# RunhuiWang/DeltaPQ

Hardware: AMD Instinct MI355X
Metric: queries/sec, SIFT1M-shaped m=8 k=256 topk=100 (higher is better)
Workload: dtype f64 sum of f32 table entries (u8 code decode; the reference's incremental f64 stack); 1 GPU

## Files before the change

deltapq_amd/api.py:

```python
import ctypes

import numpy as np

from . import _lib
from ._lib import DpqError, Info, OpenOpts, Profile, check


def _np_ptr(a):
    return ctypes.c_void_p(a.ctypes.data)


def device_count():
    return _lib.load().dpq_device_count()


def read_codewords(path):
    lib = _lib.load()
    M, K, Ds = _lib.c_i32(), _lib.c_i32(), _lib.c_i32()
    check(lib.dpq_read_codewords(path.encode(), M, K, Ds, None), "dpq_read_codewords")
    out = np.empty((M.value, K.value, Ds.value), dtype=np.float32)
    check(lib.dpq_read_codewords(path.encode(), M, K, Ds, _np_ptr(out)), "dpq_read_codewords")
    return out


def read_vecs(path, ext="fvecs", top_n=-1):
    lib = _lib.load()
    n, D = _lib.c_i64(), _lib.c_i32()
    check(lib.dpq_read_vecs(path.encode(), int(ext == "bvecs"), n, D, None, 0), "dpq_read_vecs")
    keep = n.value if top_n < 0 else min(n.value, top_n)
    out = np.empty((keep, D.value), dtype=np.float32)
    check(lib.dpq_read_vecs(path.encode(), int(ext == "bvecs"), n, D, _np_ptr(out), keep), "dpq_read_vecs")
    return out


def read_dtc_file(path):
    lib = _lib.load()
    n_codes, n_bytes = _lib.c_i64(), _lib.c_i64()
    check(lib.dpq_read_dtc_header(path.encode(), n_codes, n_bytes), "dpq_read_dtc_header")
    payload = np.fromfile(path, dtype=np.uint8, offset=16, count=n_bytes.value)
    return n_codes.value, payload


def dtc_validate(payload, n_codes, M=8):
    lib = _lib.load()
    pl = np.ascontiguousarray(payload, dtype=np.uint8)
    st = _lib.DtcStats()
    check(lib.dpq_dtc_validate(_np_ptr(pl), pl.size, n_codes, M, st), "dpq_dtc_validate")
    return dict(n_codes=st.n_codes, n_bytes=st.n_bytes, n_diffs=st.n_diffs, max_depth=st.max_depth,
                depth_hist=list(st.depth_hist))


def dtc_encode(root, depths, masks, deltas, M=8):
    lib = _lib.load()
    root = np.ascontiguousarray(root, dtype=np.uint8)
    depths = np.ascontiguousarray(depths, dtype=np.uint8)
    masks = np.ascontiguousarray(masks, dtype=np.uint16)
    deltas = np.ascontiguousarray(deltas, dtype=np.uint8)
    nb = _lib.c_i64()
    check(lib.dpq_dtc_encode(_np_ptr(root), _np_ptr(depths), _np_ptr(masks), _np_ptr(deltas), len(depths), M, None,
                             nb), "dpq_dtc_encode")
    out = np.empty(nb.value, dtype=np.uint8)
    check(lib.dpq_dtc_encode(_np_ptr(root), _np_ptr(depths), _np_ptr(masks), _np_ptr(deltas), len(depths), M,
                             _np_ptr(out), nb), "dpq_dtc_encode")
    return out


def dtc_decode(payload, n_codes, M=8, first=0, count=None):
    lib = _lib.load()
    pl = np.ascontiguousarray(payload, dtype=np.uint8)
    if count is None:
        count = n_codes - first
    out = np.empty((max(int(count), 0), M), dtype=np.uint8)
    check(lib.dpq_dtc_decode(_np_ptr(pl), pl.size, n_codes, M, first, count, _np_ptr(out)), "dpq_dtc_decode")
    return out


class HostSoA:

    def __init__(self, payload, n_codes, M=8, shard_rank=0, shard_count=1, chunks_per_segment=0, num_codes=0,
                 multi_index_stride=0):
        lib = _lib.load()
        pl = np.ascontiguousarray(payload, dtype=np.uint8)
        opts = OpenOpts(0, shard_rank, shard_count, chunks_per_segment, 0, num_codes, multi_index_stride)
        h = ctypes.c_void_p()
        check(lib.dpq_soa_build(_np_ptr(pl), pl.size, n_codes, M, opts, h), "dpq_soa_build")
        self._h = h
        info = Info()
        check(lib.dpq_soa_info(h, info), "dpq_soa_info")
        self.info = info.as_dict()
        names = ["nib", "mask", "delta", "seg_delta_off", "seg_ckpt", "mi_cell_start", "mi_code", "mi_id", "par", "carry",
                 "st_ckpt", "st_mask", "st_poff", "st_pbase", "st_delta", "st_depth"]
        views = {"seg_delta_off": np.uint64, "st_ckpt": np.uint64, "st_mask": np.uint32, "st_poff": np.uint16, "st_pbase": np.uint32,
                 "st_depth": np.uint16}
        for which, name in enumerate(names):
            ptr, nb = ctypes.c_void_p(), _lib.c_i64()
            check(lib.dpq_soa_array(h, which, ptr, nb), "dpq_soa_array")
            buf = (ctypes.c_ubyte * nb.value).from_address(ptr.value) if nb.value else b""
            arr = np.frombuffer(buf, dtype=np.uint8).copy()
            if name in views:
                arr = arr.view(views[name])
            if name.startswith("mi_"):
                arr = arr.view(np.uint32)
            setattr(self, name, arr)
        lib.dpq_soa_free(h)
        self._h = None


class DeltaTree:

    _ARRAYS = [("vec_id", np.uint32), ("parent_pos", np.uint32), ("depth", np.uint8), ("mask", np.uint16),
               ("deltas", np.uint8), ("root", np.uint8), ("edges", np.uint32)]

    def __init__(self, codes, K=256, max_height_folds=1, codebook=None, device=None):
        lib = _lib.load()
        self._lib = lib
        c = np.ascontiguousarray(codes, dtype=np.uint8)
        assert c.ndim == 2
        n, M = c.shape
        cb = None if codebook is None else np.ascontiguousarray(codebook, dtype=np.float32)
        h = ctypes.c_void_p()
        cbp, ds = (None, 0) if cb is None else (_np_ptr(cb), cb.shape[2])
        if device is None:
            check(lib.dpq_tree_build(_np_ptr(c), n, M, K, max_height_folds, cbp, ds, h), "dpq_tree_build")
        else:
            check(lib.dpq_tree_build_gpu(_np_ptr(c), n, M, K, max_height_folds, cbp, ds, device, h),
                  "dpq_tree_build_gpu")
        self._h = h
        self.M, self.K, self.n = M, K, n
        st = _lib.DtcStats()
        check(lib.dpq_tree_stats(h, st), "dpq_tree_stats")
        self.stats = dict(n_codes=st.n_codes, n_bytes=st.n_bytes, n_diffs=st.n_diffs, max_depth=st.max_depth,
                          depth_hist=list(st.depth_hist))
        for which, (name, dt) in enumerate(self._ARRAYS):
            ptr, nb = ctypes.c_void_p(), _lib.c_i64()
            check(lib.dpq_tree_array(h, which, ptr, nb), "dpq_tree_array")
            buf = (ctypes.c_ubyte * nb.value).from_address(ptr.value) if nb.value else b""
            setattr(self, name, np.frombuffer(buf, dtype=np.uint8).copy().view(dt))
        self.edges = self.edges.reshape(-1, 2)

    def payload(self):
        nb = _lib.c_i64()
        check(self._lib.dpq_tree_encode(self._h, None, nb), "dpq_tree_encode")
        out = np.empty(nb.value, dtype=np.uint8)
        check(self._lib.dpq_tree_encode(self._h, _np_ptr(out), nb), "dpq_tree_encode")
        return out

    def write_files(self, dataset_dir):
        check(self._lib.dpq_tree_write_files(self._h, dataset_dir.encode()), "dpq_tree_write_files")

    def close(self):
        if self._h is not None:
            self._lib.dpq_tree_free(self._h)
            self._h = None

    def __del__(self):
        try:
            self.close()
        except Exception:
            pass


def encode_pq(vectors, codebook, device=0):
    lib = _lib.load()
    v = np.ascontiguousarray(vectors, dtype=np.float32)
    cb = np.ascontiguousarray(codebook, dtype=np.float32)
    M, K, Ds = cb.shape
    out = np.empty((v.shape[0], M), dtype=np.uint8)
    check(lib.dpq_encode_pq(_np_ptr(v), v.shape[0], v.shape[1], _np_ptr(cb), M, K, Ds, device, _np_ptr(out)),
          "dpq_encode_pq")
    return out


def train_codebook(vectors, M=8, K=256, max_iters=25, seed=0, init=None, device=0):
    lib = _lib.load()
    v = np.ascontiguousarray(vectors, dtype=np.float32)
    assert v.ndim == 2
    n, D = v.shape
    Ds = -(-D // M) if M >= 1 else 1
    opts = _lib.TrainOpts(device=device, max_iters=max_iters, seed=seed, use_initial=int(init is not None))
    if init is None:
        cb = np.zeros((max(M, 1), max(K, 1), Ds), dtype=np.float32)
    else:
        cb = np.array(init, dtype=np.float32, order="C")
        assert cb.shape == (M, K, Ds), "init must be [M][K][ceil(D / M)]"
    st = _lib.TrainStats()
    check(lib.dpq_train_codebook(_np_ptr(v), n, D, M, K, opts, _np_ptr(cb), st), "dpq_train_codebook")
    stats = {k: getattr(st, k) for k, _ in st._fields_ if k != "distortion"}
    stats["distortion"] = [st.distortion[i] for i in range(st.iters_run)]
    return cb, stats


def write_codewords(path, codebook):
    cb = np.ascontiguousarray(codebook, dtype=np.float32)
    M, K, Ds = cb.shape
    check(_lib.load().dpq_write_codewords(path.encode(), _np_ptr(cb), M, K, Ds), "dpq_write_codewords")


def read_codes_plain(path, M):
    lib = _lib.load()
    n = _lib.c_i64()
    check(lib.dpq_read_codes_plain(path.encode(), M, n, None), "dpq_read_codes_plain")
    out = np.empty((n.value, M), dtype=np.uint8)
    check(lib.dpq_read_codes_plain(path.encode(), M, n, _np_ptr(out)), "dpq_read_codes_plain")
    return out


def read_codes_plain_ex(path, M, K=256, with_id=False):
    lib = _lib.load()
    n = _lib.c_i64()
    check(lib.dpq_read_codes_plain_ex(path.encode(), M, K, int(with_id), n, None, None), "dpq_read_codes_plain_ex")
    codes = np.empty((n.value, M), dtype=np.uint16 if K > 256 else np.uint8)
    ids = np.empty(n.value, dtype=np.int32) if with_id else None
    check(lib.dpq_read_codes_plain_ex(path.encode(), M, K, int(with_id), n, _np_ptr(codes), None if ids is None else _np_ptr(ids)),
          "dpq_read_codes_plain_ex")
    return codes, ids


def write_codes_plain(path, codes):
    c = np.ascontiguousarray(codes, dtype=np.uint8)
    check(_lib.load().dpq_write_codes_plain(path.encode(), _np_ptr(c), c.shape[0], c.shape[1]), "dpq_write_codes_plain")


def read_qnode_ids(path, n_codes):
    out = np.empty(n_codes, dtype=np.uint32)
    check(_lib.load().dpq_read_qnode_ids(path.encode(), n_codes, _np_ptr(out)), "dpq_read_qnode_ids")
    return out


def _apply_tuning(opts, tune):
    for name, value in tune.items():
        if name == "plan_ratios":
            vals = list(value) + [0, 0, 0]
            for i in range(3):
                opts.plan_ratios[i] = int(vals[i])
        elif name in ("stream_max_queries", "coarse_below", "boot_cap", "boot_target", "flags", "batch_tile_nodes"):
            v = int(value)
            if name == "stream_max_queries" and v > MAX_STREAM_QUERIES:
                raise ValueError("stream_max_queries above %d: the stream pass answers at most four queries per pass" % MAX_STREAM_QUERIES)
            if name == "boot_cap" and v != 0 and not 2048 <= v <= 16384:
                raise ValueError("boot_cap outside 2048..16384")
            setattr(opts, name, v)
        else:
            raise TypeError("unknown dpq_open_opts field %r" % name)
    return opts


OPT_NO_RELABEL, OPT_NO_FUSE_QUANTISE, OPT_NO_ASYNC_OVERLAP, OPT_BOOT_FULLSORT = 1, 2, 4, 8
OPT_NO_TIGHTEN, OPT_NO_STRANDS, OPT_FORCE_STRANDS, OPT_NO_STRAND1 = 16, 32, 64, 128
MAX_STREAM_QUERIES = 16


class DeltaPQIndex:

    def __init__(self, handle):
        self._h = handle
        self._lib = _lib.load()

    @classmethod
    def open_file(cls, path, M=8, K=256, device=0, shard_rank=0, shard_count=1, chunks_per_segment=0,
                  cand_capacity=0, num_codes=0, bootstrap=0, batch_decode=0, **tune):
        lib = _lib.load()
        opts = _apply_tuning(OpenOpts(device, shard_rank, shard_count, chunks_per_segment, cand_capacity, num_codes, bootstrap,
                                      batch_decode), tune)
        h = ctypes.c_void_p()
        check(lib.dpq_open_file(path.encode(), M, K, opts, h), "dpq_open_file")
        return cls(h)

    @classmethod
    def open_memory(cls, payload, n_codes, M=8, K=256, device=0, shard_rank=0, shard_count=1, chunks_per_segment=0,
                    cand_capacity=0, num_codes=0, bootstrap=0, global_offset=0, global_n_codes=0, batch_decode=0, **tune):
        lib = _lib.load()
        pl = np.ascontiguousarray(payload, dtype=np.uint8)
        opts = _apply_tuning(OpenOpts(device, shard_rank, shard_count, chunks_per_segment, cand_capacity, num_codes, bootstrap,
                                      batch_decode, global_offset, global_n_codes), tune)
        h = ctypes.c_void_p()
        check(lib.dpq_open_memory(_np_ptr(pl), pl.size, n_codes, M, K, opts, h), "dpq_open_memory")
        return cls(h)

    @classmethod
    def open_plain(cls, codes, K=256, device=0, shard_rank=0, shard_count=1, chunks_per_segment=0, cand_capacity=0,
                   num_codes=0, bootstrap=0, **tune):
        lib = _lib.load()
        c = np.ascontiguousarray(codes, dtype=np.uint8)
        opts = _apply_tuning(OpenOpts(device, shard_rank, shard_count, chunks_per_segment, cand_capacity, num_codes, bootstrap), tune)
        h = ctypes.c_void_p()
        check(lib.dpq_open_plain_memory(_np_ptr(c), c.shape[0], c.shape[1], K, opts, h), "dpq_open_plain_memory")
        return cls(h)

    def set_codebook(self, codebook):
        cb = np.ascontiguousarray(codebook, dtype=np.float32)
        assert cb.ndim == 3
        check(self._lib.dpq_set_codebook(self._h, _np_ptr(cb), cb.shape[2]), "dpq_set_codebook")
        return self

    def info(self):
        i = Info()
        check(self._lib.dpq_get_info(self._h, i), "dpq_get_info")
        return i.as_dict()

    def query_batch(self, queries, top_k):
        q = np.ascontiguousarray(queries, dtype=np.float32)
        if q.ndim == 1:
            q = q[None, :]
        nq = q.shape[0]
        ids = np.empty((nq, top_k), dtype=np.int32)
        dists = np.empty((nq, top_k), dtype=np.float32)
        check(self._lib.dpq_query_batch(self._h, _np_ptr(q), nq, top_k, _np_ptr(ids), _np_ptr(dists)),
              "dpq_query_batch")
        return ids, dists

    def range_search(self, queries, radius):
        q = np.ascontiguousarray(queries, dtype=np.float32)
        if q.ndim == 1:
            q = q[None, :]
        nq = q.shape[0]
        r = np.ascontiguousarray(np.broadcast_to(np.asarray(radius, dtype=np.float32), (nq,)))
        res = ctypes.c_void_p()
        check(self._lib.dpq_range_search(self._h, _np_ptr(q), nq, _np_ptr(r), res), "dpq_range_search")
        try:
            n = _lib.c_i32()
            pl, pi, pd = ctypes.c_void_p(), ctypes.c_void_p(), ctypes.c_void_p()
            check(self._lib.dpq_range_result_get(res, n, pl, pi, pd), "dpq_range_result_get")
            lims = np.ctypeslib.as_array(ctypes.cast(pl, ctypes.POINTER(_lib.c_i64)), (n.value + 1,)).copy()
            total = int(lims[-1])
            ids = np.empty(total, dtype=np.int32)
            dists = np.empty(total, dtype=np.float32)
            if total:
                ctypes.memmove(ids.ctypes.data, pi.value, total * 4)
                ctypes.memmove(dists.ctypes.data, pd.value, total * 4)
            return lims, ids, dists
        finally:
# ... 398 lines not shown
```

deltapq_amd/csrc/dpq_capi.cpp:

```cpp
#include <hip/hip_runtime.h>

#include <algorithm>
#include <atomic>
#include <cmath>
#include <cstdio>
#include <cstdlib>
#include <cstring>
#include <memory>
#include <new>
#include <numeric>
#include <stdexcept>
#include <string>
#include <type_traits>
#include <vector>

#include "../../include/deltapq_amd.h"
#include "dpq_build.h"
#include "dpq_flat.h"
#include "dpq_format.h"
#include "dpq_kernels.h"
#include "dpq_lookup.h"
#include "dpq_train.h"

namespace {
// ... 54 lines not shown
        return *this;
    }
    ~DevBuf() { reset(); }
    int alloc(size_t count) {
        reset();
        return dev_alloc(&p_, count);
    }
    void reset() {
        if (p_) hipFree(p_);
        p_ = nullptr;
    }
    T* get() const { return p_; }
    operator T*() const { return p_; }

  private:
    T* p_ = nullptr;
};

struct EventPair {
    int kind;
    hipEvent_t a, b;
};

constexpr int kMaxBatchQueries = 2048;

}

struct dpq_soa {
    dpq::SoA soa;
};

struct dpq_tree {
    dpq::Tree tree;
};

struct dpq_range_result {
    int32_t nq = 0;
    std::vector<int64_t> lims;
    std::vector<int32_t> ids;
    std::vector<float> dists;
};

struct dpq_filter {
    uint64_t owner = 0;
    DevBuf<uint32_t> bits;
    int64_t n_allowed = 0;
    mutable DevBuf<uint32_t> l0_id;
    mutable int l0_n = -1;
};

struct dpq_flat {
    int device = 0;
    int64_t n = 0, id_offset = 0;
    int D = 0, Dp = 0;
    DevBuf<float> base;
    DevBuf<uint32_t> map;
    std::vector<uint32_t> h_map;
    DevBuf<uint64_t> keys;
    DevBuf<dpq::FlatQueryState> state;
    DevBuf<float> d_q, d_dists;
    DevBuf<int32_t> d_ids, d_cand;
    DevBuf<uint32_t> flag;
    size_t keys_n = 0, state_n = 0, q_n = 0, out_n = 0, cand_n = 0;
};

namespace {
uint64_t next_index_serial() {
    static std::atomic<uint64_t> next{1};
    return next++;
}
}

struct Tuning {
    int stream_max = 4;
    int coarse_below = 128;
    int plan_ratios[3] = {0, 0, 0};
    int boot_cap = 0, boot_target = 0;
    int boot_variant = 1;
    int select_threads = 0;
    int select_fast = 1;
    int64_t batch_tile_nodes = (int64_t)16 << 20;
    bool relabel = true, fuse_quantise = true, async_overlap = true, boot_fullsort = false, tighten = true, strands = true,
         force_strands = false;
    bool strand1 = true;
    int s1_debug = 0;
};

struct RangeWs {
    DevBuf<int32_t> slot_query;
    DevBuf<uint64_t> thr_key;
    DevBuf<int64_t> out_off;
    DevBuf<uint32_t> max_count;
    DevBuf<int64_t> lims;
    DevBuf<uint32_t> cand_count;
    DevBuf<uint64_t> cand_key;
    DevBuf<int32_t> out_ids;
    DevBuf<float> out_dists;
    DevBuf<uint64_t> scratch;
    size_t key_n = 0, out_n = 0, scratch_n = 0;
    int64_t last_max_keys = 0;
};

struct LookupWs {
    DevBuf<uint32_t> flag;
    DevBuf<int32_t> ids;
    DevBuf<uint8_t> codes;
    DevBuf<float> vecs;
    DevBuf<uint8_t> tile;
    DevBuf<uint32_t> tile_segs;
    size_t ids_n = 0, codes_n = 0, vecs_n = 0, tile_n = 0, tile_segs_n = 0;
};

struct Workspace {
    int slots = 0, cap = 0;
    DevBuf<float> d_lut32;
    DevBuf<float> d_lut32r;
    DevBuf<float> d_lut_min;
    DevBuf<uint4> d_qtab;
    DevBuf<uint32_t> d_cand_count;
    DevBuf<uint32_t> d_overflow;
    DevBuf<uint32_t> d_tight;
    DevBuf<uint64_t> d_cand_key, d_thr_key;
    DevBuf<uint64_t> d_scratch;
    DevBuf<uint8_t> d_batch_raw;
};

struct dpq_index {
    Tuning tune;
    const uint64_t serial = next_index_serial();
    int device = 0;
    int M = 8, K = 256, Ds = 0;
    int cap = 0;
    bool cap_auto = true;
    dpq_info info{};
    dpq::DeviceImage img;
    DevBuf<uint64_t> d_st_ckpt;
    DevBuf<uint32_t> d_st_mask;
    DevBuf<uint16_t> d_st_depth;
    DevBuf<uint32_t> d_st_pbase, d_strip_order;
    DevBuf<uint32_t> d_strip_segs;
    std::vector<int64_t> strip_seg_off;
    DevBuf<uint8_t> d_st_delta;
    int64_t strand_bytes = 0;
    DevBuf<uint8_t> d_nib, d_par, d_carry, d_mask, d_delta, d_ckpt, d_raw;
    bool plain = false;
    DevBuf<uint64_t> d_seg_off;
    DevBuf<uint32_t> d_mi_cell, d_mi_code, d_mi_id;
    bool boot = false;
    int boot_classes = 0;
    DevBuf<unsigned long long> d_boot_stamps;
    DevBuf<unsigned long long> d_s1_stamps;
    int batch_decode = 0;
    DevBuf<uint8_t> d_relabel;
    DevBuf<uint8_t> d_nbr;
    DevBuf<float> d_codebook;
    DevBuf<unsigned long long> d_counters;
    uint32_t* h_overflow = nullptr;
    static constexpr int kFlagSlots = 64;
    uint32_t* h_any = nullptr;
    uint32_t* d_any = nullptr;
    struct Pending {
        const float* d_queries;
        int nq, top_k;
        int32_t* d_ids;
        float* d_dists;
        hipStream_t stream;
        hipStream_t user_stream;
        int flag_slot;
        int host_slot = -1;
    };
    static constexpr int kHostSlots = 16;
    struct HostSlot {
        DevBuf<float> d_q;
        DevBuf<int32_t> d_ids;
        DevBuf<float> d_d;
        size_t qf = 0, oe = 0;
        int32_t* h_ids = nullptr;
        float* h_d = nullptr;
        size_t n_out = 0;
        bool busy = false, redo = false;
        bool direct = false;
        hipEvent_t kernels_done = nullptr;
    };
    HostSlot host_slots[kHostSlots];
    hipStream_t copy_in = nullptr, copy_out = nullptr;
    uint64_t host_seq = 0;
    Workspace lane[2];
    int active_lane = 0;
    Workspace& ws() { return lane[active_lane]; }
    const Workspace& ws() const { return lane[active_lane]; }
    hipStream_t lane_stream[2] = {nullptr, nullptr};
    hipEvent_t lane_ready[2] = {nullptr, nullptr};
    uint64_t async_seq = 0;
    hipStream_t ordered_stream[2] = {nullptr, nullptr};
    bool ordered_stream_set[2] = {false, false};
    int64_t finish_reruns = 0;
    std::vector<Pending> pending;
    DevBuf<float> d_q_stage;
    DevBuf<int32_t> d_ids_stage;
    DevBuf<float> d_dists_stage;
    size_t q_stage_floats = 0, out_stage_elems = 0;
    int plan_top_k = -1, plan_cap = -1, plan_coarse = -1;
    std::vector<int> level_off, level_cnt;
    RangeWs range;
    LookupWs lookup;
    DevBuf<uint32_t> d_order;
    DevBuf<uint32_t> d_l0_id, d_l0_code;
    int l0_segments = 0;
    bool prof = false;
    bool prof_scan_only = false;
    std::vector<EventPair> events;
    std::vector<hipEvent_t> ev_pool;
    dpq_profile prof_acc{};
    hipEvent_t get_event() {
        if (!ev_pool.empty()) {
            hipEvent_t e = ev_pool.back();
            ev_pool.pop_back();
            return e;
        }
        hipEvent_t e = nullptr;
        if (hipEventCreateWithFlags(&e, hipEventDisableSystemFence) != hipSuccess) {
            prof_failed = true;
            return nullptr;
        }
        return e;
    }
    bool prof_failed = false;
    dpq::BootArgs dbg_ba{};
    dpq::ScanArgs dbg_sa{};
    int dbg_boot_slots = 0, dbg_groups = 0, dbg_splits = 0;
};

namespace {

bool dev_mode() {
    const char* dev = getenv("DPQ_DEV");
    return dev && atoi(dev) != 0;
}
#define DPQ_DEV_ONLY() \
    if (!dev_mode()) return fail(DPQ_ERR_STATE, "developer diagnostics: start the process with DPQ_DEV=1")

Tuning resolve_tuning(const dpq_open_opts& o) {
    Tuning t;
    if (o.stream_max_queries != 0) t.stream_max = std::min(16, std::max(0, o.stream_max_queries));
    if (o.coarse_below > 0) t.coarse_below = o.coarse_below;
    for (int i = 0; i < 3; ++i) t.plan_ratios[i] = o.plan_ratios[i];
    t.boot_cap = std::max(0, o.boot_cap);
    t.boot_target = std::max(0, o.boot_target);
    if (o.batch_tile_nodes > 0) t.batch_tile_nodes = o.batch_tile_nodes;
    t.relabel = !(o.flags & DPQ_OPT_NO_RELABEL);
    t.fuse_quantise = !(o.flags & DPQ_OPT_NO_FUSE_QUANTISE);
    t.async_overlap = !(o.flags & DPQ_OPT_NO_ASYNC_OVERLAP);
    t.boot_fullsort = (o.flags & DPQ_OPT_BOOT_FULLSORT) != 0;
    t.tighten = !(o.flags & DPQ_OPT_NO_TIGHTEN);
    t.strands = !(o.flags & DPQ_OPT_NO_STRANDS);
    t.force_strands = (o.flags & DPQ_OPT_FORCE_STRANDS) != 0;
    t.strand1 = !(o.flags & DPQ_OPT_NO_STRAND1);
    if (dev_mode()) {
        auto geti = [](const char* name, int* v) { if (const char* e = getenv(name)) *v = atoi(e); };
        geti("DPQ_STREAM_MAX_QUERIES", &t.stream_max);
        geti("DPQ_COARSE_BELOW", &t.coarse_below);
        if (const char* e = getenv("DPQ_PLAN_RATIOS")) sscanf(e, "%d,%d,%d", &t.plan_ratios[0], &t.plan_ratios[1], &t.plan_ratios[2]);
        geti("DPQ_BOOT_CAP", &t.boot_cap);
        geti("DPQ_BOOT_TARGET", &t.boot_target);
        geti("DPQ_BOOT_VARIANT", &t.boot_variant);
        if (const char* e = getenv("DPQ_BATCH_TILE_NODES")) t.batch_tile_nodes = std::max<int64_t>(1, atoll(e));
        int v = 1;
        geti("DPQ_RELABEL", &v); t.relabel = t.relabel && v != 0;
        v = 1; geti("DPQ_FUSE_QUANTISE", &v); t.fuse_quantise = t.fuse_quantise && v != 0;
        v = 1; geti("DPQ_ASYNC_OVERLAP", &v); t.async_overlap = t.async_overlap && v != 0;
        v = 0; geti("DPQ_BOOT_FULLSORT", &v); t.boot_fullsort = t.boot_fullsort || v != 0;
        v = 1; geti("DPQ_TIGHTEN", &v); t.tighten = t.tighten && v != 0;
        geti("DPQ_SELECT_THREADS", &t.select_threads);
        geti("DPQ_SELECT_FAST", &t.select_fast);
        v = 1; geti("DPQ_STRANDS", &v); t.strands = t.strands && v != 0;
        t.force_strands = t.force_strands || v == 2;
        v = 1; geti("DPQ_STRAND1", &v); t.strand1 = t.strand1 && v != 0;
        geti("DPQ_S1_DEBUG", &t.s1_debug);
    }
    return t;
}

void use_lane(dpq_index* x, int lane) {
    if (lane == x->active_lane) return;
    x->dbg_groups = x->dbg_boot_slots = 0;
    x->active_lane = lane;
}

int ensure_workspace(dpq_index* x, int slots, int cap) {
    Workspace& w = x->ws();
    if (slots <= w.slots && cap <= w.cap) return DPQ_OK;
    slots = std::max(slots, w.slots);
    cap = std::max(cap, w.cap);
    x->dbg_groups = x->dbg_boot_slots = 0;
    DevBuf<uint8_t> batch_raw = std::move(w.d_batch_raw);
    w = Workspace();
    w.d_batch_raw = std::move(batch_raw);
    int rc;
    if ((rc = w.d_lut32.alloc((size_t)slots * x->M * 256))) return rc;
    if (x->d_relabel && (rc = w.d_lut32r.alloc((size_t)slots * x->M * 256))) return rc;
    if ((rc = w.d_lut_min.alloc((size_t)slots * x->M * 4))) return rc;
    if ((rc = w.d_qtab.alloc((size_t)(slots / dpq::queries_per_group(x->M) + 1) *
                             (dpq::qtab_bytes_per_group(x->M) / sizeof(uint4)))))
        return rc;
    if ((rc = w.d_cand_count.alloc((size_t)slots * dpq::kRegionStride))) return rc;
    if ((rc = w.d_cand_key.alloc((size_t)slots * cap))) return rc;
    if ((rc = w.d_scratch.alloc((size_t)slots * cap))) return rc;
    if ((rc = w.d_overflow.alloc((size_t)slots))) return rc;
    if ((rc = w.d_tight.alloc((size_t)slots * dpq::kTightWords))) return rc;
    if ((rc = w.d_thr_key.alloc((size_t)slots))) return rc;
    if (!x->h_overflow) DPQ_HIP(hipHostMalloc(reinterpret_cast<void**>(&x->h_overflow), sizeof(uint32_t) * 4096));
    if (!x->d_counters) {
        if ((rc = x->d_counters.alloc(2))) return rc;
        DPQ_HIP(hipMemset(x->d_counters, 0, 16));
    }
    if (!x->h_any) {
        DPQ_HIP(hipHostMalloc(reinterpret_cast<void**>(&x->h_any), sizeof(uint32_t) * dpq_index::kFlagSlots,
                              hipHostMallocMapped));
        DPQ_HIP(hipHostGetDevicePointer(reinterpret_cast<void**>(&x->d_any), x->h_any, 0));
    }
    w.slots = slots;
    w.cap = cap;
    return DPQ_OK;
}

std::vector<uint32_t> golden_order(int64_t n) {
    std::vector<uint32_t> order((size_t)n);
    int64_t P = std::max<int64_t>(1, (int64_t)((double)n * 0.6180339887498949));
    auto gcd = [](int64_t a, int64_t b) { while (b) { int64_t t = a % b; a = b; b = t; } return a; };
    while (gcd(P, n) != 1) ++P;
    for (int64_t j = 0; j < n; ++j) order[(size_t)j] = (uint32_t)((j * P) % n);
    return order;
}

int ensure_order(dpq_index* x) {
    const int64_t nseg = x->img.n_segments;
    if (x->d_order || nseg <= 0) return DPQ_OK;
    const std::vector<uint32_t> order = golden_order(nseg);
    int rc = x->d_order.alloc((size_t)nseg);
    if (rc) return rc;
    DPQ_HIP(hipMemcpy(x->d_order, order.data(), (size_t)nseg * sizeof(uint32_t), hipMemcpyHostToDevice));
    return DPQ_OK;
}

int auto_cap(int top_k) { return std::max(4096, 32 * top_k); }

int ensure_plan(dpq_index* x, int top_k, int cap, int shape) {
    if (x->plan_top_k == top_k && x->plan_cap == cap && x->plan_coarse == shape) return DPQ_OK;
    const int coarse = shape & 1;
    const bool tight = (shape & 2) != 0;
    const bool one_level = (shape & 4) != 0;
    const int64_t S = (int64_t)dpq::kChunk * x->img.chunks_per_segment;
    const int64_t nseg = x->img.n_segments;
    const int64_t s0 = std::min<int64_t>(nseg, std::max<int64_t>(1, dpq::kLevel0Nodes / S));
    std::vector<int64_t> bounds;
    if (x->boot) {
        bounds.push_back(nseg);
        std::vector<int> ratios;
        const int* forced = x->tune.plan_ratios;
        if (forced[0] >= 2) {
// ... 102 lines not shown
    return x->ws().d_batch_raw.alloc((size_t)batch_raw_bytes(x));
}

int splits_for(int n_seg_pass, int n_groups) {
    const int want = std::max(1, dpq::kMaxSplits / std::max(1, n_groups));
    return std::max(1, std::min(n_seg_pass, want));
}

struct Regions {
    int splits;
    int region_cap;
    int64_t stride;
};

Regions regions_for(const dpq_index* x, int n_seg_pass, int n_groups, int top_k, int cap) {
    Regions r;
    r.splits = splits_for(n_seg_pass, n_groups);
    r.region_cap = (cap - top_k) / r.splits;
    if (x->cap_auto)
        r.region_cap = std::max(r.region_cap, std::max(std::max(256, 16384 / r.splits), 64 * top_k / r.splits));
    r.region_cap = std::max(r.region_cap, 1);
    r.stride = (int64_t)top_k + (int64_t)r.splits * r.region_cap;
    return r;
}

struct Batch {
    int nq, top_k;
    int nqp, ngroups;
    int cap;
    bool tight_plan;
    bool direct;
    bool strands, strand1, strand1_tight;
    bool scratch;
    int64_t tile_segs;
    bool one_tile;
    bool labelled;
    bool boot_tables;
    int plan_shape;
    int64_t stride;
};

Batch batch_mode(const dpq_index* x, int nq, int top_k, bool filtered = false) {
    Batch b{};
    const int QG = dpq::queries_per_group(x->M);
    b.nq = nq;
    b.top_k = top_k;
    b.nqp = (nq + QG - 1) / QG * QG;
    b.ngroups = b.nqp / QG;
    b.cap = x->cap_auto ? auto_cap(top_k) : std::max(x->cap, top_k);
    b.tight_plan = x->tune.tighten && nq > x->tune.stream_max && b.ngroups * dpq::kTightSplits >= dpq::kMaxSplits &&
                   (x->plain || use_batch_decode(x, b.ngroups));
    b.direct = !x->plain && nq <= x->tune.stream_max && !filtered;
    b.strands = b.direct && x->img.st_ckpt != nullptr && (x->tune.force_strands || x->img.n_local >= dpq::kStrandMinNodes);
    b.strand1 = b.strands && x->tune.strand1 && dpq::stream_queries_per_pass(x->M, nq) == 1;
    b.strand1_tight = b.strand1 && x->tune.tighten && x->tune.plan_ratios[0] == 0;
    b.scratch = !b.direct && use_batch_decode(x, b.ngroups);
    b.tile_segs = b.scratch ? batch_tile_segments(x) : 0;
    b.one_tile = b.scratch && b.tile_segs >= x->img.n_segments;
    b.labelled = b.scratch && x->d_relabel.get() != nullptr;
    b.boot_tables = x->boot && x->tune.fuse_quantise && !b.direct;
    b.plan_shape = (nq <= x->tune.coarse_below ? 1 : 0) | (b.tight_plan ? 2 : 0) | (b.strand1_tight ? 4 : 0);
    return b;
}

int prepare_batch(dpq_index* x, Batch* b) {
    int rc;
    if ((rc = ensure_plan(x, b->top_k, b->cap, b->plan_shape))) return rc;
    int64_t stride = b->top_k;
    for (size_t l = 1; l < x->level_cnt.size(); ++l)
        stride = std::max(stride, regions_for(x, x->level_cnt[l], b->ngroups, b->top_k, b->cap).stride);
    const int s1_region_cap = std::min(std::max(64, b->top_k), 256);
    if (b->strand1) stride = std::max<int64_t>(stride, (int64_t)b->top_k + (int64_t)dpq::kStrand1Regions * s1_region_cap);
    if (stride > INT32_MAX) return fail(DPQ_ERR_NOMEM, "candidate buffer too large");
    if ((rc = ensure_workspace(x, b->nqp, (int)stride))) return rc;
    b->stride = x->ws().cap;
    if (b->scratch && (rc = ensure_batch_raw(x))) return rc;
    return DPQ_OK;
}

int build_tables(dpq_index* x, const Batch& b, const float* d_queries, hipStream_t stream) {
    Workspace& w = x->ws();
    if (b.one_tile) {
        Timer t(x, stream, 4);
        DPQ_HIP(dpq::launch_decode_list(x->img, nullptr, x->img.n_segments, x->d_relabel,
                                        reinterpret_cast<uint32_t*>(w.d_batch_raw.get()), stream));
    }
    {
        Timer t(x, stream, 0);
        DPQ_HIP(dpq::launch_lut_build(x->d_codebook, d_queries, b.nq, b.nqp, x->M, x->K, x->Ds, w.d_lut32, w.d_lut_min,
                                      nullptr, w.d_overflow, b.scratch ? x->d_relabel.get() : nullptr, w.d_lut32r,
                                      x->tune.tighten ? w.d_tight.get() : nullptr, stream));
    }
    if (x->prof) x->prof_acc.lut_launches++;
    return DPQ_OK;
}

dpq::ScanArgs batch_scan_args(const dpq_index* x, const Batch& b) {
    const Workspace& w = x->ws();
    dpq::ScanArgs sa{};
    sa.img = x->img;
    if (b.one_tile) sa.img.raw = w.d_batch_raw;
    sa.fp32_accum = x->plain ? 1 : 0;
    sa.lut32 = b.labelled ? w.d_lut32r.get() : w.d_lut32.get();
    sa.lut_min = w.d_lut_min;
    sa.thr_key = w.d_thr_key;
    sa.slot_query = nullptr;
    sa.n_queries = b.nq;
    sa.cand_count = w.d_cand_count;
    sa.cand_key = w.d_cand_key;
    sa.cand_stride = b.stride;
    sa.region_off = b.top_k;
    sa.counters = x->prof && !x->prof_scan_only ? x->d_counters.get() : nullptr;
    sa.qtab = w.d_qtab;
    sa.tight_hist = x->tune.tighten && (b.top_k <= 512 || x->level_cnt.size() <= 2) ? w.d_tight.get() : nullptr;
    sa.tight_k = b.top_k;
    return sa;
}

dpq::SelectArgs batch_select_args(const dpq_index* x, const Batch& b, int32_t* d_ids, float* d_dists, int flag_slot) {
    const Workspace& w = x->ws();
    dpq::SelectArgs se{};
    se.threads = x->tune.select_threads;
    se.fast_final = x->tune.select_fast;
    se.cand_count = w.d_cand_count;
    se.cand_key = w.d_cand_key;
    se.cand_stride = b.stride;
    se.region_off = b.top_k;
    se.scratch = w.d_scratch;
    se.lut32 = w.d_lut32;
    se.slot_query = nullptr;
    se.top_k = b.top_k;
    se.thr_key = w.d_thr_key;
    se.overflow = w.d_overflow;
    se.any_overflow = x->d_any + flag_slot;
    se.out_ids = d_ids;
    se.out_dists = d_dists;
    se.n_codes_total = x->plain ? -1 : x->img.n_codes_total;
    se.fp32_accum = x->plain ? 1 : 0;
    se.keep_thr = x->boot ? 1 : 0;
    se.stamps = x->d_boot_stamps ? x->d_boot_stamps + (size_t)kMaxBatchQueries * 8 : nullptr;
    return se;
}

int boot_level(dpq_index* x, const Batch& b, const dpq_filter* filt, hipStream_t stream) {
    const Workspace& w = x->ws();
    const int top_k = b.top_k;
    const int cap_env = x->tune.boot_cap;
    dpq::BootArgs ba{};
    ba.cell_start = x->d_mi_cell;
    const bool full_sort = x->tune.boot_fullsort;
    ba.nbr = full_sort ? nullptr : x->d_nbr.get();
    ba.n_classes = x->boot_classes;
    ba.mi_code = x->d_mi_code;
    ba.mi_id = x->d_mi_id;
    ba.lut32 = w.d_lut32;
    ba.slot_query = nullptr;
    ba.top_k = top_k;
    const int cap_auto = top_k <= 256 ? (x->M <= 8 ? 3072 : 6144) : (top_k <= 640 && x->M <= 8) ? 5888 : 12288;
    ba.cap = std::max(std::min(cap_env > 0 ? cap_env : cap_auto, 16384), std::max(top_k, 2048));
    ba.cap = (ba.cap + 63) / 64 * 64;
    const int target_env = x->tune.boot_target;
    const int target_auto = top_k <= 256 ? std::max(top_k, ba.cap * 2 / 3) : ba.cap;
    ba.target = target_env > 0 ? std::min(ba.cap, std::max(target_env, top_k)) : target_auto;
    ba.thr_key = w.d_thr_key;
    ba.cand_count = w.d_cand_count;
    ba.fp32_accum = x->plain ? 1 : 0;
    ba.stamps = x->d_boot_stamps;
    ba.variant = x->tune.boot_variant;
    ba.n_queries = b.nq;
    ba.qtab = b.boot_tables ? w.d_qtab.get() : nullptr;
    ba.relabel = b.scratch ? x->d_relabel.get() : nullptr;
    ba.lut_min = w.d_lut_min;
    if (filt) {
        ba.filter = filt->bits;
        ba.id_base = x->img.id_base;
        ba.eval_cap = 8 * ba.cap;
    }
    const int slots = b.boot_tables ? b.nqp : b.nq;
    {
        Timer t(x, stream, 5);
        DPQ_HIP(dpq::launch_bootstrap(ba, x->M, slots, stream));
    }
    if (x->prof) x->prof_acc.bootstrap_launches++;
    if (filt) return DPQ_OK;
    x->dbg_ba = ba;
    x->dbg_boot_slots = slots;
    return DPQ_OK;
}

int stream_level(dpq_index* x, const Batch& b, size_t l, const dpq::ScanArgs& sa, dpq::SelectArgs& se,
                 hipStream_t stream) {
    const Workspace& w = x->ws();
    const int nq = b.nq, top_k = b.top_k;
    dpq::ScanArgs st = sa;
    st.tight_hist = nullptr;
    st.region_cap = se.region_cap = (int32_t)std::min<int64_t>(b.stride - top_k, INT32_MAX);
    se.n_regions = 2;
    DPQ_HIP(hipMemset2DAsync(w.d_cand_count + 1, sizeof(uint32_t) * dpq::kRegionStride, 0, sizeof(uint32_t), (size_t)nq,
                             stream));
    if (!b.strands) {
        Timer t(x, stream, 1);
        DPQ_HIP(dpq::launch_stream(st, nq, stream));
        if (x->prof) x->prof_acc.stream_launches++;
    } else {
        const bool one_level = x->level_cnt.size() == 2;
        const int64_t nseg = x->img.n_segments, ns = x->img.n_strips;
        const int64_t lo = (int64_t)x->level_off[l] * ns / nseg;
        const int64_t hi = l + 1 == x->level_cnt.size() ? ns : ((int64_t)x->level_off[l] + x->level_cnt[l]) * ns / nseg;
        Timer t(x, stream, 1);
        if (b.strand1) {
            st.seg_list = one_level ? nullptr : x->d_strip_order + lo;
            st.n_seg_pass = (int32_t)(hi - lo);
            st.tight_hist = b.strand1_tight && one_level && nq == 1 ? w.d_tight.get() : nullptr;
            st.debug_pass = x->tune.s1_debug ? 16 + x->tune.s1_debug : 0;
            st.stamps = x->d_s1_stamps;
            st.region_cap = se.region_cap = (int32_t)((b.stride - top_k) / dpq::kStrand1Regions);
            se.n_regions = 1 + dpq::strand1_workgroups(st.n_seg_pass);
            DPQ_HIP(dpq::launch_strand1(st, nq, stream));
            if (x->prof) x->prof_acc.strand1_launches++;
        } else if (hi - lo < 1536 && x->d_strip_segs && !x->tune.force_strands) {
            st.seg_list = x->d_strip_segs + x->strip_seg_off[(size_t)lo];
            st.n_seg_pass = (int32_t)(x->strip_seg_off[(size_t)hi] - x->strip_seg_off[(size_t)lo]);
            DPQ_HIP(dpq::launch_stream(st, nq, stream));
            if (x->prof) x->prof_acc.stream_launches++;
        } else {
            st.seg_list = x->d_strip_order + lo;
            st.n_seg_pass = (int32_t)(hi - lo);
            DPQ_HIP(dpq::launch_strand(st, nq, stream));
            if (x->prof) x->prof_acc.strand_launches++;
        }
    }
    if (x->prof) {
        x->prof_acc.scan_launches++;
        x->prof_acc.scan_stream_bytes +=
            (int64_t)nq * (int64_t)((double)x->info.device_bytes * sa.n_seg_pass / std::max(1, x->img.n_segments));
    }
    return DPQ_OK;
}

int filter_level(dpq_index* x, const Batch& b, size_t l, dpq::ScanArgs sa, dpq::SelectArgs& se, hipStream_t stream) {
    const Workspace& w = x->ws();
    const Regions rg = regions_for(x, sa.n_seg_pass, b.ngroups, b.top_k, b.cap);
    sa.region_cap = se.region_cap = rg.region_cap;
    se.n_regions = 1 + rg.splits;
    if (!(b.boot_tables && l == 1)) {
        Timer t(x, stream, 3);
        DPQ_HIP(dpq::launch_quantise(sa, b.ngroups, stream));
    }
    if (b.scratch && !b.one_tile) {
        for (int t0 = 0; t0 < sa.n_seg_pass; t0 += (int)b.tile_segs) {
            const int cnt = std::min<int>((int)b.tile_segs, sa.n_seg_pass - t0);
            {
                Timer t(x, stream, 4);
                DPQ_HIP(dpq::launch_decode_list(x->img, sa.seg_list + t0, cnt, x->d_relabel,
                                                reinterpret_cast<uint32_t*>(w.d_batch_raw.get()), stream));
            }
            dpq::ScanArgs tile = sa;
            tile.img.raw = w.d_batch_raw;
            tile.raw_by_pos = 1;
            tile.append = t0 > 0 ? 1 : 0;
            tile.seg_list = sa.seg_list + t0;
            tile.n_seg_pass = cnt;
            {
                Timer t(x, stream, 1);
                DPQ_HIP(dpq::launch_scan(tile, b.ngroups, rg.splits, stream));
            }
            if (x->prof && t0 > 0) x->prof_acc.scan_launches++;
        }
    } else {
        Timer t(x, stream, 1);
        DPQ_HIP(dpq::launch_scan(sa, b.ngroups, rg.splits, stream));
        if (l == 1 && !sa.filter) {
            x->dbg_sa = sa;
            x->dbg_groups = b.ngroups;
            x->dbg_splits = rg.splits;
        }
    }
    if (x->prof) {
        x->prof_acc.scan_launches++;
        x->prof_acc.scan_stream_bytes +=
            (int64_t)((double)x->info.device_bytes * sa.n_seg_pass / std::max(1, x->img.n_segments));
    }
    return DPQ_OK;
}

int rerun_overflowed(dpq_index* x, const Batch& b, dpq::ScanArgs sa, dpq::SelectArgs se, hipStream_t stream) {
    const Workspace& w = x->ws();
    const int nq = b.nq, top_k = b.top_k;
    DPQ_HIP(hipStreamSynchronize(stream));
    if (*reinterpret_cast<volatile uint32_t*>(x->h_any) == 0) return DPQ_OK;
    std::vector<int> over;
    for (int base = 0; base < nq; base += 4096) {
        const int n = std::min(4096, nq - base);
        DPQ_HIP(hipMemcpyAsync(x->h_overflow, w.d_overflow.get() + base, sizeof(uint32_t) * n, hipMemcpyDeviceToHost,
                               stream));
        DPQ_HIP(hipStreamSynchronize(stream));
        for (int i = 0; i < n; ++i)
            if (x->h_overflow[i]) over.push_back(base + i);
    }
    if (over.empty()) return DPQ_OK;

    const int QG = dpq::queries_per_group(x->M);
    const int slots2 = ((int)over.size() + QG - 1) / QG * QG;
    const int ng2 = slots2 / QG;
    std::vector<int32_t> slot_query((size_t)slots2, -1);
    std::vector<uint64_t> h_key((size_t)b.nqp), k2((size_t)slots2, ~0ull);
    DPQ_HIP(hipMemcpy(h_key.data(), w.d_thr_key, sizeof(uint64_t) * b.nqp, hipMemcpyDeviceToHost));
    for (size_t i = 0; i < over.size(); ++i) {
        slot_query[i] = over[i];
        k2[i] = h_key[(size_t)over[i]];
    }
    const int splits2 = std::min(16, splits_for(x->img.n_segments, ng2));
    int64_t rcap2 = std::max<int64_t>(2 * (int64_t)top_k, 1024);
    for (int attempt = 0;; ++attempt) {
        const int64_t stride2 = (int64_t)top_k + (int64_t)splits2 * rcap2;
        if (stride2 > INT32_MAX) return fail(DPQ_ERR_NOMEM, "candidate buffer too large");
        DevBuf<int32_t> d_slot_query;
        DevBuf<uint32_t> c_count, c_over;
        DevBuf<uint64_t> c_keys, c_scratch, c_tk;
        DevBuf<uint4> c_qtab;
        int rc = d_slot_query.alloc((size_t)slots2);
        if (!rc) rc = c_count.alloc((size_t)slots2 * dpq::kRegionStride);
        if (!rc) rc = c_over.alloc((size_t)slots2);
        if (!rc) rc = c_keys.alloc((size_t)slots2 * stride2);
        if (!rc) rc = c_scratch.alloc((size_t)slots2 * stride2);
        if (!rc) rc = c_tk.alloc((size_t)slots2);
        if (!rc) rc = c_qtab.alloc((size_t)ng2 * (dpq::qtab_bytes_per_group(x->M) / sizeof(uint4)));
        if (rc) return rc;
        hipError_t e = hipSuccess;
        auto chk = [&](hipError_t r) { if (e == hipSuccess) e = r; };
        chk(hipMemcpy(d_slot_query, slot_query.data(), sizeof(int32_t) * slots2, hipMemcpyHostToDevice));
        chk(hipMemcpy(c_tk, k2.data(), sizeof(uint64_t) * slots2, hipMemcpyHostToDevice));
        chk(hipMemsetAsync(c_count, 0, sizeof(uint32_t) * slots2 * dpq::kRegionStride, stream));
        chk(hipMemsetAsync(c_over, 0, sizeof(uint32_t) * slots2, stream));
        sa.seg_list = nullptr;
        sa.n_seg_pass = x->img.n_segments;
        sa.tight_hist = nullptr;
// ... 57 lines not shown
            DPQ_HIP(dpq::launch_filter_ids(x->d_l0_id, n0, filt->bits, x->img.id_base, filt->l0_id, stream));
            filt->l0_n = n0;
        }
    }
    if ((rc = build_tables(x, b, d_queries, stream))) return rc;
    x->h_any[flag_slot] = 0;
    dpq::ScanArgs sa = batch_scan_args(x, b);
    sa.filter = filt ? filt->bits.get() : nullptr;
    dpq::SelectArgs se = batch_select_args(x, b, d_ids, d_dists, flag_slot);

    const int64_t S = (int64_t)dpq::kChunk * x->img.chunks_per_segment;
    const size_t n_levels = x->img.n_segments > 0 ? x->level_cnt.size() : 0;
    if (n_levels == 0) {
        se.final_pass = 1;
        DPQ_HIP(dpq::launch_select(se, x->M, nq, stream));
        return DPQ_OK;
    }
    for (size_t l = 0; l < n_levels; ++l) {
        if (l == 0 && x->boot) {
            if ((rc = boot_level(x, b, filt, stream))) return rc;
            continue;
        }
        if (l == 0) {
            se.shared_id = filt ? filt->l0_id.get() : x->d_l0_id.get();
            se.shared_code = x->d_l0_code;
            se.shared_n = (int)(x->level_cnt[0] * S);
        } else {
            se.shared_id = nullptr;
            se.shared_code = nullptr;
            se.shared_n = 0;
            sa.seg_list = x->d_order + x->level_off[l];
            sa.n_seg_pass = x->level_cnt[l];
            if ((rc = b.direct ? stream_level(x, b, l, sa, se, stream) : filter_level(x, b, l, sa, se, stream))) return rc;
        }
        if (x->prof) x->prof_acc.scan_node_query_pairs += (int64_t)x->level_cnt[l] * S * nq;
        se.final_pass = l + 1 == n_levels ? 1 : 0;
        {
            Timer t(x, stream, 2);
            DPQ_HIP(dpq::launch_select(se, x->M, nq, stream));
        }
        if (x->prof) x->prof_acc.select_launches++;
    }
    if (flag_slot > 0) return DPQ_OK;
    return rerun_overflowed(x, b, sa, se, stream);
}

constexpr int64_t kRangeChunkKeys = (int64_t)1 << 26;

bool range_thr_key(float r, uint64_t* key) {
    if (!(r > 0.0f)) return false;
    if (std::isinf(r)) {
        *key = ~0ull;
        return true;
    }
    uint32_t bits;
    std::memcpy(&bits, &r, sizeof bits);
    *key = ((uint64_t)bits << 32) - 1ull;
    return true;
}

template <class T>
int grow(DevBuf<T>& buf, size_t* have, size_t want) {
    if (want <= *have && buf) return DPQ_OK;
    *have = 0;
    int rc = buf.alloc(want);
    if (!rc) *have = want;
    return rc;
}

int range_scan(dpq_index* x, const Batch& b, dpq::ScanArgs sa, int n_groups, int splits, hipStream_t stream) {
    const Workspace& w = x->ws();
    DPQ_HIP(hipMemsetAsync(sa.cand_count, 0, sizeof(uint32_t) * (size_t)n_groups * dpq::queries_per_group(x->M) *
                                                 dpq::kRegionStride, stream));
    if (sa.n_seg_pass <= 0) return DPQ_OK;
    {
        Timer t(x, stream, 3);
        DPQ_HIP(dpq::launch_quantise(sa, n_groups, stream));
    }
    if (b.scratch && !b.one_tile) {
        for (int t0 = 0; t0 < sa.n_seg_pass; t0 += (int)b.tile_segs) {
            const int cnt = std::min<int>((int)b.tile_segs, sa.n_seg_pass - t0);
            {
                Timer t(x, stream, 4);
                DPQ_HIP(dpq::launch_decode_list(x->img, sa.seg_list + t0, cnt, x->d_relabel,
                                                reinterpret_cast<uint32_t*>(w.d_batch_raw.get()), stream));
            }
            dpq::ScanArgs tile = sa;
            tile.img.raw = w.d_batch_raw;
            tile.raw_by_pos = 1;
            tile.append = t0 > 0 ? 1 : 0;
            tile.seg_list = sa.seg_list + t0;
            tile.n_seg_pass = cnt;
            Timer t(x, stream, 1);
            DPQ_HIP(dpq::launch_scan(tile, n_groups, splits, stream));
            if (x->prof) x->prof_acc.scan_launches++;
        }
    } else {
        Timer t(x, stream, 1);
        DPQ_HIP(dpq::launch_scan(sa, n_groups, splits, stream));
        if (x->prof) x->prof_acc.scan_launches++;
    }
    return DPQ_OK;
}

int range_emit(dpq_index* x, dpq::RangeEmitArgs ea, int n_slots, const std::vector<int>& emit,
               const std::vector<int32_t>& slot_query, const std::vector<int64_t>& lims, int64_t res_base,
               dpq_range_result* res, hipStream_t stream) {
    RangeWs& R = x->range;
    std::vector<int64_t> off((size_t)n_slots);
    for (size_t i = 0; i < emit.size();) {
        std::fill(off.begin(), off.end(), -1);
        int64_t span = 0, max_n = 0;
        bool contiguous = true;
        size_t j = i;
        for (; j < emit.size(); ++j) {
            const int q = slot_query[(size_t)emit[j]];
            const int64_t n = lims[(size_t)q + 1] - lims[(size_t)q];
            if (j > i && span + n > kRangeChunkKeys) break;
            if (j > i && lims[(size_t)slot_query[(size_t)emit[j - 1]] + 1] != lims[(size_t)q]) contiguous = false;
            off[(size_t)emit[j]] = span;
            span += n;
            max_n = std::max(max_n, n);
        }
        if (span > 0) {
            int rc;
            if ((size_t)span > R.out_n) {
                R.out_n = 0;
                if ((rc = R.out_ids.alloc((size_t)span)) || (rc = R.out_dists.alloc((size_t)span))) return rc;
                R.out_n = (size_t)span;
            }
            if (max_n > dpq::kRangeLdsKeys && (rc = grow(R.scratch, &R.scratch_n, 2 * (size_t)span))) return rc;
            DPQ_HIP(hipMemcpyAsync(R.out_off, off.data(), sizeof(int64_t) * n_slots, hipMemcpyHostToDevice, stream));
            ea.out_off = R.out_off;
            ea.out_ids = R.out_ids;
            ea.out_dists = R.out_dists;
            ea.out_n = span;
            ea.scratch = max_n > dpq::kRangeLdsKeys ? R.scratch.get() : nullptr;
            int lk = 2;
            while (lk < std::min<int64_t>(max_n, dpq::kRangeLdsKeys)) lk <<= 1;
            ea.lds_keys = lk;
            {
                Timer t(x, stream, 2);
                DPQ_HIP(dpq::launch_range_emit(ea, n_slots, stream));
            }
            const int64_t first = res_base + lims[(size_t)slot_query[(size_t)emit[i]]];
            if (contiguous) {
                DPQ_HIP(hipMemcpyAsync(res->ids.data() + first, R.out_ids, sizeof(int32_t) * span, hipMemcpyDeviceToHost, stream));
                DPQ_HIP(hipMemcpyAsync(res->dists.data() + first, R.out_dists, sizeof(float) * span, hipMemcpyDeviceToHost,
                                       stream));
                DPQ_HIP(hipStreamSynchronize(stream));
            } else {
                std::vector<int32_t> h_ids((size_t)span);
                std::vector<float> h_d((size_t)span);
                DPQ_HIP(hipMemcpyAsync(h_ids.data(), R.out_ids, sizeof(int32_t) * span, hipMemcpyDeviceToHost, stream));
                DPQ_HIP(hipMemcpyAsync(h_d.data(), R.out_dists, sizeof(float) * span, hipMemcpyDeviceToHost, stream));
                DPQ_HIP(hipStreamSynchronize(stream));
                for (size_t k = i; k < j; ++k) {
                    const int q = slot_query[(size_t)emit[k]];
                    const int64_t o = off[(size_t)emit[k]], n = lims[(size_t)q + 1] - lims[(size_t)q];
                    std::copy(h_ids.begin() + o, h_ids.begin() + o + n, res->ids.begin() + res_base + lims[(size_t)q]);
                    std::copy(h_d.begin() + o, h_d.begin() + o + n, res->dists.begin() + res_base + lims[(size_t)q]);
                }
            }
        }
        i = j;
    }
    return DPQ_OK;
}

int range_batch(dpq_index* x, const float* d_queries, int nq, const float* radii, int base, dpq_range_result* res,
                hipStream_t stream) {
    RangeWs& R = x->range;
    const int QG = dpq::queries_per_group(x->M);
    Batch b = batch_mode(x, nq, 1);
    std::vector<int32_t> slot_query;
    std::vector<uint64_t> thr;
    for (int q = 0; q < nq; ++q) {
        uint64_t key;
        if (!range_thr_key(radii[q], &key)) continue;
        slot_query.push_back(q);
        thr.push_back(key);
    }
    const int n_active = (int)slot_query.size();
    const int slots = (n_active + QG - 1) / QG * QG, n_groups = slots / QG;
    slot_query.resize((size_t)slots, -1);
    thr.resize((size_t)slots, 0ull);
    const int64_t res_base = res->lims[(size_t)base];
    std::vector<int64_t> lims((size_t)nq + 1, 0);
    if (n_active == 0) {
        for (int q = 0; q <= nq; ++q) res->lims[(size_t)base + q] = res_base;
        return DPQ_OK;
    }
    int rc;
    if (!R.slot_query) {
        if ((rc = R.slot_query.alloc(kMaxBatchQueries))) return rc;
        if ((rc = R.thr_key.alloc(kMaxBatchQueries))) return rc;
        if ((rc = R.out_off.alloc(kMaxBatchQueries))) return rc;
        if ((rc = R.max_count.alloc(kMaxBatchQueries))) return rc;
        if ((rc = R.lims.alloc(kMaxBatchQueries + 1))) return rc;
        if ((rc = R.cand_count.alloc((size_t)kMaxBatchQueries * dpq::kRegionStride))) return rc;
    }
    if ((rc = ensure_workspace(x, b.nqp, std::max(1, x->ws().cap)))) return rc;
    if (b.scratch && (rc = ensure_batch_raw(x))) return rc;
    const bool tiled = b.scratch && !b.one_tile;
    if (tiled && (rc = ensure_order(x))) return rc;
    if ((rc = build_tables(x, b, d_queries, stream))) return rc;

    const int nseg = x->img.n_segments;
    const int splits = splits_for(nseg, n_groups);
    const int region_cap = x->cap_auto ? std::max(256, 16384 / splits) : std::max(1, x->cap / splits);
    const Workspace& w = x->ws();
    dpq::ScanArgs sa{};
    sa.img = x->img;
    if (b.one_tile) sa.img.raw = w.d_batch_raw;
    sa.fp32_accum = x->plain ? 1 : 0;
    sa.lut32 = b.labelled ? w.d_lut32r.get() : w.d_lut32.get();
    sa.lut_min = w.d_lut_min;
    sa.thr_key = R.thr_key;
    sa.slot_query = R.slot_query;
    sa.n_queries = slots;
    sa.seg_list = tiled ? x->d_order.get() : nullptr;
    sa.n_seg_pass = nseg;
    sa.cand_count = R.cand_count;
    sa.region_off = 0;
    sa.counters = x->prof && !x->prof_scan_only ? x->d_counters.get() : nullptr;
    sa.qtab = w.d_qtab;
    sa.tight_hist = nullptr;

    auto scan_and_count = [&](int n_live, int rcap, int64_t* lims_out, std::vector<uint32_t>* max_count) -> int {
        const int n_slots = (n_live + QG - 1) / QG * QG, ng = n_slots / QG;
        const int64_t stride = (int64_t)splits * rcap;
        int rc2 = grow(R.cand_key, &R.key_n, (size_t)n_live * stride);
        if (rc2) return rc2;
        R.last_max_keys = std::max(R.last_max_keys, (int64_t)n_live * stride);
        DPQ_HIP(hipMemcpyAsync(R.slot_query, slot_query.data(), sizeof(int32_t) * n_slots, hipMemcpyHostToDevice, stream));
        DPQ_HIP(hipMemcpyAsync(R.thr_key, thr.data(), sizeof(uint64_t) * n_slots, hipMemcpyHostToDevice, stream));
        sa.cand_key = R.cand_key;
        sa.cand_stride = stride;
        sa.region_cap = rcap;
        if ((rc2 = range_scan(x, b, sa, ng, splits, stream))) return rc2;
        dpq::RangeCountArgs ca{};
        ca.slot_query = R.slot_query;
        ca.cand_count = R.cand_count;
        ca.n_slots = n_slots;
        ca.n_regions = splits;
        ca.n_queries = nq;
        ca.max_count = R.max_count;
        ca.lims = R.lims;
        {
            Timer t(x, stream, 2);
            DPQ_HIP(dpq::launch_range_count(ca, stream));
        }
        max_count->resize((size_t)n_slots);
        DPQ_HIP(hipMemcpyAsync(lims_out, R.lims, sizeof(int64_t) * (nq + 1), hipMemcpyDeviceToHost, stream));
        DPQ_HIP(hipMemcpyAsync(max_count->data(), R.max_count, sizeof(uint32_t) * n_slots, hipMemcpyDeviceToHost, stream));
        DPQ_HIP(hipStreamSynchronize(stream));
        return DPQ_OK;
    };
    std::vector<uint32_t> max_count;
    if ((rc = scan_and_count(n_active, region_cap, lims.data(), &max_count))) return rc;
    for (int q = 0; q <= nq; ++q) res->lims[(size_t)base + q] = res_base + lims[(size_t)q];
    const int64_t total = res_base + lims[(size_t)nq];
    res->ids.resize((size_t)total);
    res->dists.resize((size_t)total);

    dpq::RangeEmitArgs ea{};
    ea.cand_count = R.cand_count;
    ea.cand_key = R.cand_key;
    ea.cand_stride = (int64_t)splits * region_cap;
    ea.region_off = 0;
    ea.region_cap = region_cap;
    ea.n_regions = splits;
    ea.n_codes_total = x->plain ? -1 : x->img.n_codes_total;
    std::vector<int> emit, over;
    for (int s = 0; s < n_active; ++s) (max_count[(size_t)s] > (uint32_t)region_cap ? over : emit).push_back(s);
    if ((rc = range_emit(x, ea, slots, emit, slot_query, lims, res_base, res, stream))) return rc;
    if (over.empty()) return DPQ_OK;

    const std::vector<int32_t> q_of(slot_query.begin(), slot_query.begin() + n_active);
    const std::vector<uint64_t> k_of(thr.begin(), thr.begin() + n_active);
    const std::vector<uint32_t> need(max_count.begin(), max_count.begin() + n_active);
    for (size_t i = 0; i < over.size();) {
        size_t j = i;
        uint32_t rcap = 0;
        for (; j < over.size(); ++j) {
            const uint32_t r2 = std::max(rcap, need[(size_t)over[j]]);
            if (j > i && (int64_t)(j - i + 1) * splits * (int64_t)r2 > kRangeChunkKeys) break;
            rcap = r2;
        }
        if ((int64_t)rcap * splits > INT32_MAX) return fail(DPQ_ERR_NOMEM, "range search: candidate regions too large");
        const int n2 = (int)(j - i), slots2 = (n2 + QG - 1) / QG * QG;
        std::fill(slot_query.begin(), slot_query.end(), -1);
        for (int k = 0; k < n2; ++k) {
            slot_query[(size_t)k] = q_of[(size_t)over[i + k]];
            thr[(size_t)k] = k_of[(size_t)over[i + k]];
        }
        std::vector<int64_t> lims2((size_t)nq + 1);
        if ((rc = scan_and_count(n2, (int)rcap, lims2.data(), &max_count))) return rc;
        for (int k = 0; k < n2; ++k) {
            const int q = slot_query[(size_t)k];
            if (max_count[(size_t)k] > rcap || lims2[(size_t)q + 1] - lims2[(size_t)q] != lims[(size_t)q + 1] - lims[(size_t)q])
                return fail(DPQ_ERR_STATE, "range search: the rerun of an overflowed query found a different count");
        }
        ea.cand_key = R.cand_key;
        ea.cand_stride = (int64_t)splits * rcap;
        ea.region_cap = (int)rcap;
        std::vector<int> emit2((size_t)n2);
        std::iota(emit2.begin(), emit2.end(), 0);
        if ((rc = range_emit(x, ea, slots2, emit2, slot_query, lims, res_base, res, stream))) return rc;
        if (x->prof) x->prof_acc.overflow_reruns += n2;
        i = j;
    }
    return DPQ_OK;
}

void range_trim(dpq_index* x) {
    RangeWs& R = x->range;
    if (R.key_n > ((size_t)40 << 20)) R.cand_key.reset(), R.key_n = 0;
    if (R.out_n > ((size_t)16 << 20)) R.out_ids.reset(), R.out_dists.reset(), R.out_n = 0;
    R.scratch.reset();
    R.scratch_n = 0;
}

dpq::ScanArgs debug_scan_args(const dpq_index* x, int nq, int* splits) {
    const Workspace& w = x->ws();
    const int QG = dpq::queries_per_group(x->M);
    dpq::ScanArgs sa{};
    sa.img = x->img;
    sa.fp32_accum = x->plain ? 1 : 0;
    sa.lut32 = w.d_lut32;
    sa.lut_min = w.d_lut_min;
    sa.thr_key = w.d_thr_key;
    sa.slot_query = nullptr;
    sa.n_queries = nq;
    sa.seg_list = nullptr;
    sa.n_seg_pass = x->img.n_segments;
    if (const char* e = getenv("DPQ_DEBUG_NSEG")) sa.n_seg_pass = std::min(x->img.n_segments, atoi(e));
    if (*splits <= 0) *splits = splits_for(sa.n_seg_pass, (nq + QG - 1) / QG);
    sa.cand_count = w.d_cand_count;
    sa.cand_key = w.d_cand_key;
    sa.cand_stride = w.cap;
    sa.region_off = 0;
    sa.region_cap = std::max(1, w.cap / *splits);
    sa.qtab = w.d_qtab;
    return sa;
}

int open_from_payload(const uint8_t* payload, int64_t n_bytes, int64_t n_codes, int M, int K,
                      const dpq_open_opts* opts, dpq_index** out) {
    if (!out) return fail(DPQ_ERR_ARG, "out is NULL");
    *out = nullptr;
    dpq_open_opts o{};
    if (opts) o = *opts;
    if (M != 8 && M != 16)
        return fail(DPQ_ERR_ARG, "this build has scan kernels for M = 8 (reference format) and M = 16 (own extension)");
    if (K < 1 || K > 256) return fail(DPQ_ERR_ARG, "K must be in 1..256 (one byte per sub-code)");
    if (o.global_offset < 0 || o.global_n_codes < 0 || (o.global_offset != 0 && o.global_n_codes == 0) ||
        (o.global_n_codes > 0 && o.global_offset + n_codes > o.global_n_codes))
        return fail(DPQ_ERR_ARG, "global_offset / global_n_codes do not enclose this payload (a part of a larger index "
                                 "needs global_n_codes > 0)");
    if (n_codes >= (int64_t)INT32_MAX || o.global_n_codes >= (int64_t)INT32_MAX || o.global_offset + n_codes >= (int64_t)INT32_MAX)
        return fail(DPQ_ERR_ARG, "ids beyond 2^31 - 1: results carry int32 DFS positions (h:2979)");
    if (o.chunks_per_segment > dpq::kSortMax / dpq::kChunk)
        return fail(DPQ_ERR_ARG, "chunks_per_segment must be <= 64 (a segment is the cascade's level-0 unit)");
    int ndev = 0;
    if (hipGetDeviceCount(&ndev) != hipSuccess || ndev <= 0)
        return fail(DPQ_ERR_NO_DEVICE, "no HIP device visible; this library has no CPU fallback");
    if (o.device < 0 || o.device >= ndev) return fail(DPQ_ERR_NO_DEVICE, "device ordinal out of range");

    dpq::SoA soa;
    std::string err;
    const int64_t n_scan = o.num_codes > 0 ? std::min<int64_t>(o.num_codes, n_codes) : n_codes;
    const int64_t per_shard = n_scan / std::max(1, o.shard_count);
    int mi_stride = o.bootstrap < 0 ? 0 : dpq::bootstrap_stride_for(per_shard);
    if (o.bootstrap > 0 && mi_stride == 0 && per_shard >= 16384) mi_stride = 1;
    const Tuning tune0 = resolve_tuning(o);
    const bool want_strands = tune0.strands && (tune0.force_strands || per_shard >= dpq::kStrandMinNodes / 4 * 3);
    int rc = dpq::transcode(payload, n_bytes, n_codes, M, o.shard_rank, o.shard_count, o.chunks_per_segment, &soa,
                            &err, o.num_codes, mi_stride, 0, want_strands ? 1 : 0);
    if (rc) return fail(rc, err);

    DPQ_HIP(hipSetDevice(o.device));
    dpq_index* x = new dpq_index();
    x->device = o.device;
    x->M = M;
    x->K = K;
    x->cap_auto = o.cand_capacity <= 0;
    x->cap = o.cand_capacity;
    x->batch_decode = o.batch_decode;
    x->tune = tune0;
    auto up = [&](auto& buf, const void* src, size_t bytes) -> int {
        using T = typename std::remove_reference_t<decltype(buf)>::value_type;
        int r = buf.alloc((bytes + sizeof(T) - 1) / sizeof(T) + 64 / sizeof(T));
        if (r) return r;
        if (bytes) {
            hipError_t e = hipMemcpy(buf, src, bytes, hipMemcpyHostToDevice);
            if (e != hipSuccess) return fail(DPQ_ERR_HIP, std::string("upload: ") + hipGetErrorString(e));
        }
        return DPQ_OK;
    };
    rc = up(x->d_nib, soa.nib.data(), soa.nib.size());
    if (!rc) rc = up(x->d_par, soa.par.data(), soa.par.size());
    if (!rc) rc = up(x->d_carry, soa.carry.data(), soa.carry.size());
    if (!rc) rc = up(x->d_mask, soa.mask.data(), soa.mask.size());
    if (!rc) rc = up(x->d_delta, soa.delta.data(), soa.delta.size());
    if (!rc) rc = up(x->d_seg_off, soa.seg_delta_off.data(), soa.seg_delta_off.size() * 8);
    if (!rc) rc = up(x->d_ckpt, soa.seg_ckpt.data(), soa.seg_ckpt.size());
    if (o.global_offset != 0)
        for (uint32_t& id : soa.mi_id) id += (uint32_t)o.global_offset;
    if (!rc && soa.mi_stride > 0 && (int64_t)soa.mi_id.size() >= 16384) {
        rc = up(x->d_mi_cell, soa.mi_cell_start.data(), soa.mi_cell_start.size() * 4);
        if (!rc) rc = up(x->d_mi_code, soa.mi_code.data(), soa.mi_code.size() * 4);
        if (!rc) rc = up(x->d_mi_id, soa.mi_id.data(), soa.mi_id.size() * 4);
        x->boot = !rc;
        x->boot_classes = soa.mi_classes;
    }
    if (!rc && x->tune.relabel && soa.relabel.size() == (size_t)M * 256) {
        rc = up(x->d_relabel, soa.relabel.data(), soa.relabel.size());
    }
    if (!rc && x->boot && x->tune.strands && soa.n_strips > 0 && soa.n_strips < INT32_MAX) {
        rc = up(x->d_st_ckpt, soa.st_ckpt.data(), soa.st_ckpt.size() * 8);
        if (!rc) rc = up(x->d_st_mask, soa.st_mask.data(), soa.st_mask.size() * 4);
        if (!rc) rc = up(x->d_st_depth, soa.st_depth.data(), soa.st_depth.size() * 2);
        if (!rc) rc = up(x->d_st_pbase, soa.st_pbase.data(), soa.st_pbase.size() * 4);
        if (!rc) rc = up(x->d_st_delta, soa.st_delta.data(), soa.st_delta.size());
        if (!rc) {
            const int64_t ns = soa.n_strips;
            const std::vector<uint32_t> order = golden_order(ns);
            rc = up(x->d_strip_order, order.data(), order.size() * 4);
            const int64_t S = soa.nodes_per_segment();
            if (!rc && dpq::kStripNodes % S == 0) {
                std::vector<uint32_t> segs;
                x->strip_seg_off.assign((size_t)ns + 1, 0);
                for (int64_t j = 0; j < ns; ++j) {
                    const int64_t s0 = (int64_t)order[(size_t)j] * (dpq::kStripNodes / S);
                    for (int64_t t = s0; t < std::min(s0 + dpq::kStripNodes / S, soa.n_segments); ++t) segs.push_back((uint32_t)t);
                    x->strip_seg_off[(size_t)j + 1] = (int64_t)segs.size();
                }
                rc = up(x->d_strip_segs, segs.data(), segs.size() * 4);
            }
        }
        if (!rc) {
            x->img.st_ckpt = x->d_st_ckpt;
            x->img.st_mask = x->d_st_mask;
            x->img.st_depth = x->d_st_depth;
            x->img.st_pbase = x->d_st_pbase;
            x->img.st_delta = x->d_st_delta;
            x->img.n_strips = (int32_t)soa.n_strips;
            x->strand_bytes = soa.strand_bytes();
        }
    }
    if (rc) {
        dpq_close(x);
        return rc;
    }
    x->img.nib = x->d_nib;
    x->img.par = x->d_par;
    x->img.carry = x->d_carry;
    x->img.mask = x->d_mask;
    x->img.delta = x->d_delta;
    x->img.seg_delta_off = x->d_seg_off;
    x->img.seg_ckpt = x->d_ckpt;
    x->img.n_local = soa.node_hi - soa.node_lo;
    x->img.n_codes_total = o.global_n_codes > 0 ? o.global_n_codes : soa.n_codes_total;
    x->img.id_base = (uint32_t)(o.global_offset + soa.node_lo);
    x->img.n_segments = (int32_t)soa.n_segments;
    x->img.chunks_per_segment = soa.chunks_per_segment;
    x->img.M = M;
    x->img.K = K;

    dpq_info& inf = x->info;
    inf.n_codes_total = x->img.n_codes_total;
    inf.n_bytes_total = soa.n_bytes_total;
    inf.node_lo = o.global_offset + soa.node_lo;
    inf.node_hi = o.global_offset + soa.node_hi;
    inf.algorithmic_bytes = soa.algorithmic_bytes;
    inf.device_bytes = soa.device_bytes();
    inf.bootstrap_bytes = x->boot ? soa.bootstrap_bytes() : 0;
    inf.bootstrap_stride = x->boot ? soa.mi_stride : 0;
    inf.batch_decode_mb = batch_decode_possible(x) ? (int32_t)((batch_raw_bytes(x) + (1 << 20) - 1) >> 20) : 0;
    inf.strand_bytes = x->strand_bytes;
    inf.n_diffs = soa.n_diffs;
    inf.M = M;
    inf.K = K;
    inf.Ds = 0;
    inf.n_segments = (int32_t)soa.n_segments;
    inf.chunks_per_segment = soa.chunks_per_segment;
    inf.max_depth = soa.max_depth;
    inf.device = o.device;
    inf.cand_capacity = x->cap;
    *out = x;
    return DPQ_OK;
}

int open_plain(const uint8_t* codes, int64_t n_codes, int M, int K, const dpq_open_opts* opts, dpq_index** out) {
    if (!out) return fail(DPQ_ERR_ARG, "out is NULL");
    *out = nullptr;
    dpq_open_opts o{};
    if (opts) o = *opts;
    if (!codes || n_codes < 1 || n_codes >= (int64_t)INT32_MAX) return fail(DPQ_ERR_ARG, "bad codes / n_codes");
    if (M != 8 && M != 16) return fail(DPQ_ERR_ARG, "M must be 8 or 16");
    if (K < 1 || K > 256) return fail(DPQ_ERR_ARG, "K must be in 1..256 (one byte per sub-code)");
    int ndev = 0;
    if (hipGetDeviceCount(&ndev) != hipSuccess || ndev <= 0)
        return fail(DPQ_ERR_NO_DEVICE, "no HIP device visible; this library has no CPU fallback");
    if (o.device < 0 || o.device >= ndev) return fail(DPQ_ERR_NO_DEVICE, "device ordinal out of range");
    int cps = o.chunks_per_segment <= 0 ? dpq::kDefaultChunksPerSegment : o.chunks_per_segment;
    if (cps > dpq::kSortMax / dpq::kChunk) return fail(DPQ_ERR_ARG, "chunks_per_segment must be <= 64");
    int count = o.shard_count <= 0 ? 1 : o.shard_count;
    if (o.shard_rank < 0 || o.shard_rank >= count) return fail(DPQ_ERR_ARG, "bad shard_rank / shard_count");
    if (o.num_codes < 0 || (int64_t)o.num_codes > n_codes) return fail(DPQ_ERR_ARG, "num_codes outside 0..n_codes");
    if (o.num_codes > 0) n_codes = o.num_codes;
    const int64_t S = (int64_t)dpq::kChunk * cps;
    const int64_t nseg_total = (n_codes + S - 1) / S;
    const int64_t seg_lo = nseg_total * o.shard_rank / count, seg_hi = nseg_total * (o.shard_rank + 1) / count;
    const int64_t lo = std::min(seg_lo * S, n_codes), hi = std::min(seg_hi * S, n_codes);
    DPQ_HIP(hipSetDevice(o.device));
    dpq_index* x = new dpq_index();
    x->device = o.device;
    x->M = M;
    x->K = K;
    x->plain = true;
    x->tune = resolve_tuning(o);
    x->cap_auto = o.cand_capacity <= 0;
    x->cap = o.cand_capacity;
    const size_t padded = (size_t)(seg_hi - seg_lo) * S * M;
    int rc = x->d_raw.alloc(padded + 64);
    if (!rc) {
        hipError_t e = hipMemset(x->d_raw, 0, padded + 64);
        if (e == hipSuccess && hi > lo)
            e = hipMemcpy(x->d_raw, codes + (size_t)lo * M, (size_t)(hi - lo) * M, hipMemcpyHostToDevice);
        if (e != hipSuccess) rc = fail(DPQ_ERR_HIP, std::string("upload: ") + hipGetErrorString(e));
    }
    if (rc) {
        dpq_close(x);
        return rc;
    }
    {
        int mi_stride = o.bootstrap < 0 ? 0 : dpq::bootstrap_stride_for(hi - lo);
        if (o.bootstrap > 0 && mi_stride == 0 && hi - lo >= 16384) mi_stride = 1;
        if (mi_stride > 0) {
            dpq::SoA mi;
            std::vector<uint32_t> ids;
            std::vector<uint8_t> cds;
            for (int64_t i = lo; i < hi; i += mi_stride) {
                ids.push_back((uint32_t)i);
                cds.insert(cds.end(), codes + (size_t)i * M, codes + (size_t)(i + 1) * M);
            }
            dpq::build_multi_index(ids, cds, M, mi_stride, dpq::bootstrap_classes_for((int64_t)ids.size()), &mi);
            auto upl = [&](DevBuf<uint32_t>& d, const std::vector<uint32_t>& v) -> int {
                int r = d.alloc(v.size() + 16);
                if (r) return r;
                if (!v.empty() && hipMemcpy(d, v.data(), v.size() * 4, hipMemcpyHostToDevice) != hipSuccess)
                    return fail(DPQ_ERR_HIP, "upload of the bootstrap multi-index failed");
                return DPQ_OK;
            };
            rc = upl(x->d_mi_cell, mi.mi_cell_start);
            if (!rc) rc = upl(x->d_mi_code, mi.mi_code);
            if (!rc) rc = upl(x->d_mi_id, mi.mi_id);
            if (rc) {
// ... 65 lines not shown
        case DPQ_ERR_NO_DEVICE: return "no usable GPU";
        case DPQ_ERR_HIP: return "HIP runtime error";
        case DPQ_ERR_NOMEM: return "out of memory";
        case DPQ_ERR_STATE: return "call out of order";
        case DPQ_ERR_TOPK: return "top_k exceeds the number of codes";
        default: return "unknown status";
    }
}

const char* dpq_last_error(void) { return g_last_error.c_str(); }

int dpq_device_count(void) {
    int n = 0;
    if (hipGetDeviceCount(&n) != hipSuccess) return 0;
    return n < 0 ? 0 : n;
}

int dpq_read_dtc_header(const char* path, int64_t* n_codes, int64_t* n_bytes) {
    return guarded([&]() -> int {
    if (!path || !n_codes || !n_bytes) return fail(DPQ_ERR_ARG, "NULL argument");
    std::string err;
    int rc = dpq::read_dtc_header(path, n_codes, n_bytes, &err);
    return rc ? fail(rc, err) : DPQ_OK;
    });
}

int dpq_read_codewords(const char* path, int32_t* M, int32_t* K, int32_t* Ds, float* out) {
    return guarded([&]() -> int {
    if (!path || !M || !K || !Ds) return fail(DPQ_ERR_ARG, "NULL argument");
    std::string err;
    std::vector<float> v;
    int m, k, ds;
    int rc = dpq::read_codewords(path, &m, &k, &ds, out ? &v : nullptr, &err);
    if (rc) return fail(rc, err);
    *M = m;
    *K = k;
    *Ds = ds;
    if (out) memcpy(out, v.data(), v.size() * sizeof(float));
    return DPQ_OK;
    });
}

int dpq_read_vecs(const char* path, int is_bvecs, int64_t* n, int32_t* D, float* out, int64_t cap) {
    return guarded([&]() -> int {
    if (!path || !n || !D) return fail(DPQ_ERR_ARG, "NULL argument");
    std::string err;
    std::vector<float> v;
    int d = 0;
    int rc = dpq::read_vecs(path, is_bvecs != 0, n, &d, out ? &v : nullptr, cap, &err);
    if (rc) return fail(rc, err);
    *D = d;
    if (out) memcpy(out, v.data(), v.size() * sizeof(float));
    return DPQ_OK;
    });
}

int dpq_dtc_file_name(const char* dataset_dir, int M, int K, int64_t N, char* out, int64_t out_len) {
    return guarded([&]() -> int {
    if (!dataset_dir || !out) return fail(DPQ_ERR_ARG, "NULL argument");
    std::string s = dpq::dtc_file_name(dataset_dir, M, K, N);
    if ((int64_t)s.size() + 1 > out_len) return fail(DPQ_ERR_ARG, "output buffer too small");
    memcpy(out, s.c_str(), s.size() + 1);
    return DPQ_OK;
    });
}

int dpq_dtc_validate(const uint8_t* payload, int64_t n_bytes, int64_t n_codes, int M, dpq_dtc_stats* stats) {
    return guarded([&]() -> int {
    std::string err;
    int rc = dpq::validate(payload, n_bytes, n_codes, M, stats, &err);
    return rc ? fail(rc, err) : DPQ_OK;
    });
}

int dpq_soa_build(const uint8_t* payload, int64_t n_bytes, int64_t n_codes, int M, const dpq_open_opts* opts,
                  dpq_soa** out) {
    return guarded([&]() -> int {
    if (!out) return fail(DPQ_ERR_ARG, "out is NULL");
    dpq_open_opts o{};
    if (opts) o = *opts;
    dpq_soa* s = new dpq_soa();
    std::string err;
    int rc = dpq::transcode(payload, n_bytes, n_codes, M, o.shard_rank, o.shard_count, o.chunks_per_segment, &s->soa,
                            &err, o.num_codes, o.bootstrap > 0 && M % 4 == 0 ? o.bootstrap : 0);
    if (rc) {
        delete s;
        *out = nullptr;
        return fail(rc, err);
    }
    *out = s;
    return DPQ_OK;
    });
}

int dpq_soa_info(const dpq_soa* soa, dpq_info* info) {
    return guarded([&]() -> int {
    if (!soa || !info) return fail(DPQ_ERR_ARG, "NULL argument");
    fill_info_from_soa(soa->soa, info);
    return DPQ_OK;
    });
}

int dpq_soa_array(const dpq_soa* soa, int which, const void** ptr, int64_t* n_bytes) {
    return guarded([&]() -> int {
    if (!soa || !ptr || !n_bytes) return fail(DPQ_ERR_ARG, "NULL argument");
    const dpq::SoA& s = soa->soa;
    switch (which) {
        case 0: *ptr = s.nib.data(); *n_bytes = (int64_t)s.nib.size(); break;
        case 1: *ptr = s.mask.data(); *n_bytes = (int64_t)s.mask.size(); break;
        case 2: *ptr = s.delta.data(); *n_bytes = (int64_t)s.delta.size(); break;
        case 3: *ptr = s.seg_delta_off.data(); *n_bytes = (int64_t)s.seg_delta_off.size() * 8; break;
        case 4: *ptr = s.seg_ckpt.data(); *n_bytes = (int64_t)s.seg_ckpt.size(); break;
        case 5: *ptr = s.mi_cell_start.data(); *n_bytes = (int64_t)s.mi_cell_start.size() * 4; break;
        case 6: *ptr = s.mi_code.data(); *n_bytes = (int64_t)s.mi_code.size() * 4; break;
        case 7: *ptr = s.mi_id.data(); *n_bytes = (int64_t)s.mi_id.size() * 4; break;
        case 8: *ptr = s.par.data(); *n_bytes = (int64_t)s.par.size(); break;
        case 9: *ptr = s.carry.data(); *n_bytes = (int64_t)s.carry.size(); break;
        case 10: *ptr = s.st_ckpt.data(); *n_bytes = (int64_t)s.st_ckpt.size() * 8; break;
        case 11: *ptr = s.st_mask.data(); *n_bytes = (int64_t)s.st_mask.size() * 4; break;
        case 12: *ptr = s.st_poff.data(); *n_bytes = (int64_t)s.st_poff.size() * 2; break;
        case 13: *ptr = s.st_pbase.data(); *n_bytes = (int64_t)s.st_pbase.size() * 4; break;
        case 14: *ptr = s.st_delta.data(); *n_bytes = (int64_t)s.st_delta.size(); break;
        case 15: *ptr = s.st_depth.data(); *n_bytes = (int64_t)s.st_depth.size() * 2; break;
        default: return fail(DPQ_ERR_ARG, "which must be 0..15");
    }
    return DPQ_OK;
    });
}

void dpq_soa_free(dpq_soa* soa) { delete soa; }

int dpq_dtc_encode(const uint8_t* root_code, const uint8_t* depths, const uint16_t* masks, const uint8_t* deltas,
                   int64_t n_codes, int M, uint8_t* out, int64_t* n_bytes) {
    return guarded([&]() -> int {
    std::string err;
    int rc = dpq::encode(root_code, depths, masks, deltas, n_codes, M, out, n_bytes, &err);
    return rc ? fail(rc, err) : DPQ_OK;
    });
}

int dpq_tree_build(const uint8_t* codes, int64_t n_codes, int M, int K, int max_height_folds, const float* codewords,
                   int Ds, dpq_tree** out) {
    return guarded([&]() -> int {
    if (!out) return fail(DPQ_ERR_ARG, "out is NULL");
    *out = nullptr;
    dpq_tree* t = new dpq_tree();
    std::string err;
    int rc = dpq::build_tree(codes, n_codes, M, K, max_height_folds, codewords, Ds, &t->tree, &err);
    if (rc) {
        delete t;
        return fail(rc, err);
    }
    *out = t;
    return DPQ_OK;
    });
}

int dpq_tree_build_gpu(const uint8_t* codes, int64_t n_codes, int M, int K, int max_height_folds,
                       const float* codewords, int Ds, int device, dpq_tree** out) {
    return guarded([&]() -> int {
    if (!out) return fail(DPQ_ERR_ARG, "out is NULL");
    *out = nullptr;
    if (!codes || n_codes < 1 || n_codes >= (int64_t)INT32_MAX || M < 1 || M > 16 || K < 1 || K > 256 ||
        max_height_folds < 1)
        return fail(DPQ_ERR_ARG, "bad argument to dpq_tree_build_gpu");
    std::string err;
    std::vector<uint32_t> finalists;
    std::vector<std::pair<uint32_t, uint32_t>> edges;
    const bool prefilter = !(dev_mode() && getenv("DPQ_BUILD_PREFILTER") && atoi(getenv("DPQ_BUILD_PREFILTER")) == 0);
    int rc = dpq::find_edges_gpu(codes, n_codes, M, max_height_folds, device, &finalists, &edges, &err, prefilter);
    if (rc) return fail(rc, err);
    dpq_tree* t = new dpq_tree();
    static const bool host_layout = dev_mode() && getenv("DPQ_BUILD_LAYOUT") &&
                                    std::string(getenv("DPQ_BUILD_LAYOUT")) == "host";
    rc = host_layout ? dpq::layout_tree(codes, n_codes, M, K, max_height_folds, codewords, Ds, finalists, &edges, &t->tree, &err)
                     : dpq::layout_tree_gpu(codes, n_codes, M, K, max_height_folds, codewords, Ds, finalists, &edges, device,
                                            &t->tree, &err);
    if (rc) {
        delete t;
        return fail(rc, err);
    }
    *out = t;
    return DPQ_OK;
    });
}

int dpq_tree_stats(const dpq_tree* t, dpq_dtc_stats* stats) {
    return guarded([&]() -> int {
    if (!t || !stats) return fail(DPQ_ERR_ARG, "NULL argument");
    const dpq::Tree& tr = t->tree;
    memset(stats, 0, sizeof *stats);
    stats->n_codes = tr.n;
    stats->n_diffs = tr.n_diffs;
    stats->n_bytes = tr.M + tr.n_diffs + (tr.n - 1) * dpq::mask_bytes_for(tr.M) + tr.n / 2;
    for (int d = 0; d < 16; ++d) stats->depth_hist[d] = tr.depth_hist[d];
    stats->max_depth = tr.max_depth;
    stats->M = tr.M;
    return DPQ_OK;
    });
}

int dpq_tree_array(const dpq_tree* t, int which, const void** ptr, int64_t* n_bytes) {
    return guarded([&]() -> int {
    if (!t || !ptr || !n_bytes) return fail(DPQ_ERR_ARG, "NULL argument");
    const dpq::Tree& tr = t->tree;
    switch (which) {
        case 0: *ptr = tr.vec_id.data(); *n_bytes = (int64_t)tr.vec_id.size() * 4; break;
// ... 883 lines not shown
    int64_t allowed = 0;
    for (int64_t w = 0; w < n_words && 32 * w < n_local; ++w) {
        const int64_t g0 = base + 32 * w;
        if (g0 >= n_bits) break;
        const int64_t lo = g0 >> 5;
        const int sh = (int)(g0 & 31);
        uint32_t v = words[lo] >> sh;
        if (sh && lo + 1 < user_words) v |= words[lo + 1] << (32 - sh);
        const int64_t valid = std::min<int64_t>(32, std::min(n_bits - g0, n_local - 32 * w));
        if (valid < 32) v &= (1u << valid) - 1u;
        h[(size_t)w] = v;
    }
    const int64_t N = x->img.n_codes_total;
    if (!x->plain && (N & 1) == 0 && N - 1 >= base && N - 1 < base + n_local) {
        const int64_t l = N - 1 - base;
        h[(size_t)(l >> 5)] = (h[(size_t)(l >> 5)] & ~(1u << (l & 31))) | (user_bit(N) << (l & 31));
    }
    for (uint32_t v : h) allowed += __builtin_popcount(v);
    std::unique_ptr<dpq_filter> f(new dpq_filter());
    f->owner = x->serial;
    f->n_allowed = allowed;
    int rc = f->bits.alloc((size_t)n_words);
    if (rc) return rc;
    DPQ_HIP(hipMemcpy(f->bits, h.data(), (size_t)n_words * sizeof(uint32_t), hipMemcpyHostToDevice));
    *out = f.release();
    return DPQ_OK;
    });
}

void dpq_filter_free(dpq_filter* f) { delete f; }

int dpq_filter_count(const dpq_filter* f, int64_t* n_allowed) {
    if (!f || !n_allowed) return fail(DPQ_ERR_ARG, "NULL argument");
    *n_allowed = f->n_allowed;
    return DPQ_OK;
}

int dpq_query_batch_filtered(dpq_index* x, const dpq_filter* f, const float* queries, int nq, int top_k, int32_t* ids,
                             float* dists) {
    return guarded([&]() -> int {
    int rc = check_filter(x, f);
    if (rc) return rc;
    return query_host(x, f, queries, nq, top_k, ids, dists);
    });
}

int dpq_query_batch_device_filtered(dpq_index* x, const dpq_filter* f, const float* d_queries, int nq, int top_k,
                                    int32_t* d_ids, float* d_dists, void* hip_stream) {
    return guarded([&]() -> int {
    int rc = check_filter(x, f);
    if (rc) return rc;
    return query_device(x, f, d_queries, nq, top_k, d_ids, d_dists, hip_stream);
    });
}

namespace {

constexpr size_t kLookupVecBytes = (size_t)64 << 20;
constexpr int64_t kLookupTileNodes = (int64_t)4 << 20;

bool lookup_id_ok(const dpq_index* x, int64_t id) {
    const int64_t N = x->img.n_codes_total;
    int64_t pos = id;
    if (!x->plain && (N & 1) == 0) {
        if (id == N)
            pos = N - 1;
        else if (id == N - 1)
            return false;
    }
    const int64_t l = pos - (int64_t)x->img.id_base;
    return l >= 0 && l < x->img.n_local;
}

int lookup_begin(dpq_index* x, int64_t n, hipStream_t stream, dpq::DeviceImage* img) {
    LookupWs& lw = x->lookup;
    *img = x->img;
    const int64_t image_bytes = (int64_t)x->img.n_segments * dpq::kChunk * x->img.chunks_per_segment * x->M;
    const bool possible = !x->plain && x->img.n_segments > 0 && image_bytes <= dpq::kLookupGroupedMaxBytes;
    bool grouped = possible && n >= dpq::kLookupGroupedPerSegment * (int64_t)x->img.n_segments;
    if (possible && dev_mode())
        if (const char* e = getenv("DPQ_LOOKUP_GROUPED")) grouped = atoi(e) != 0;
    if (!grouped) return DPQ_OK;
    if (int rc = grow(lw.tile, &lw.tile_n, (size_t)image_bytes)) return rc;
    DPQ_HIP(dpq::launch_decode_list(x->img, nullptr, x->img.n_segments, nullptr, reinterpret_cast<uint32_t*>(lw.tile.get()),
                                    stream));
    img->raw = lw.tile;
    return DPQ_OK;
}

void lookup_end(dpq_index* x) {
    LookupWs& lw = x->lookup;
    if (lw.tile_n > (size_t)(kLookupTileNodes + 1024 * dpq::kChunk) * x->M) {
        lw.tile.reset();
        lw.tile_n = 0;
    }
}

int lookup_run(dpq_index* x, const dpq::DeviceImage& img, const int32_t* d_ids, int64_t n, uint8_t* d_codes, float* d_vecs,
               hipStream_t stream, const char* who) {
    LookupWs& lw = x->lookup;
    int rc;
    if (!lw.flag.get() && (rc = lw.flag.alloc(1))) return rc;
    DPQ_HIP(hipMemsetAsync(lw.flag, 0, sizeof(uint32_t), stream));
    const size_t D = (size_t)x->M * x->Ds;
    for (int64_t i0 = 0; i0 < n; i0 += dpq::kLookupSlice) {
        dpq::LookupArgs a{};
        a.img = img;
        a.ids = d_ids + i0;
        a.n = std::min(dpq::kLookupSlice, n - i0);
        a.even_rule = x->plain ? 0 : 1;
        if (d_vecs) {
            a.out_vecs = d_vecs + (size_t)i0 * D;
            a.codebook = x->d_codebook;
            a.Ds = x->Ds;
        } else {
            a.out_codes = d_codes + (size_t)i0 * x->M;
        }
        a.flag = lw.flag;
        DPQ_HIP(dpq::launch_lookup(a, stream));
    }
    uint32_t bad = 0;
    DPQ_HIP(hipMemcpyAsync(&bad, lw.flag, sizeof bad, hipMemcpyDeviceToHost, stream));
    DPQ_HIP(hipStreamSynchronize(stream));
    if (bad) return fail(DPQ_ERR_ARG, std::string(who) + ": an id names no node of this handle");
    return DPQ_OK;
}

int lookup_on_device(dpq_index* x, const int32_t* d_ids, int64_t n, uint8_t* d_codes, float* d_vecs, hipStream_t stream,
                     const char* who) {
    dpq::DeviceImage img;
    int rc = lookup_begin(x, n, stream, &img);
    if (!rc) rc = lookup_run(x, img, d_ids, n, d_codes, d_vecs, stream, who);
    if (rc) hipStreamSynchronize(stream);
    lookup_end(x);
    return rc;
}

int lookup_args(dpq_index* x, const void* ids, int64_t n, const void* out, bool recon, const char* who) {
    if (!x || n < 0 || (n > 0 && (!ids || !out))) return fail(DPQ_ERR_ARG, std::string(who) + ": NULL argument or n < 0");
    if (recon && !x->d_codebook) return fail(DPQ_ERR_STATE, "dpq_set_codebook has not been called");
    if (!x->pending.empty())
        if (int rc = dpq_finish(x)) return rc;
    return DPQ_OK;
}

int lookup_host(dpq_index* x, const int32_t* ids, int64_t n, uint8_t* codes_out, float* vecs_out, const char* who) {
    int rc = lookup_args(x, ids, n, codes_out ? (const void*)codes_out : (const void*)vecs_out, vecs_out != nullptr, who);
    if (rc || n == 0) return rc;
    for (int64_t i = 0; i < n; ++i)
        if (ids[i] >= 0 && !lookup_id_ok(x, ids[i])) {
            char msg[160];
            snprintf(msg, sizeof msg, "%s: ids[%lld] = %d names no node of this handle", who, (long long)i, (int)ids[i]);
            return fail(DPQ_ERR_ARG, msg);
        }
    DPQ_HIP(hipSetDevice(x->device));
    LookupWs& lw = x->lookup;
    const size_t D = (size_t)x->M * x->Ds;
    int64_t slice = dpq::kLookupSlice;
    if (vecs_out) slice = std::max<int64_t>(1, std::min<int64_t>(slice, (int64_t)(kLookupVecBytes / (D * sizeof(float)))));
    slice = std::min(slice, n);
    rc = grow(lw.ids, &lw.ids_n, (size_t)slice);
    if (!rc && vecs_out) rc = grow(lw.vecs, &lw.vecs_n, (size_t)slice * D);
    if (!rc && codes_out) rc = grow(lw.codes, &lw.codes_n, (size_t)slice * x->M);
    if (rc) return rc;
    dpq::DeviceImage img;
    rc = lookup_begin(x, n, nullptr, &img);
    for (int64_t i0 = 0; !rc && i0 < n; i0 += slice) {
        const int64_t m = std::min(slice, n - i0);
        hipError_t e = hipMemcpy(lw.ids, ids + i0, (size_t)m * sizeof(int32_t), hipMemcpyHostToDevice);
        if (e == hipSuccess)
            rc = lookup_run(x, img, lw.ids, m, codes_out ? lw.codes.get() : nullptr, vecs_out ? lw.vecs.get() : nullptr, nullptr,
                            who);
        if (e == hipSuccess && !rc)
            e = vecs_out ? hipMemcpy(vecs_out + (size_t)i0 * D, lw.vecs, (size_t)m * D * sizeof(float), hipMemcpyDeviceToHost)
                         : hipMemcpy(codes_out + (size_t)i0 * x->M, lw.codes, (size_t)m * x->M, hipMemcpyDeviceToHost);
        if (e != hipSuccess) rc = fail(DPQ_ERR_HIP, std::string(who) + ": " + hipGetErrorString(e));
    }
    hipDeviceSynchronize();
    lookup_end(x);
    return rc;
}

}

int dpq_get_codes(dpq_index* x, const int32_t* ids, int64_t n, uint8_t* codes_out) {
    return guarded([&]() -> int { return lookup_host(x, ids, n, codes_out, nullptr, "dpq_get_codes"); });
}

int dpq_reconstruct(dpq_index* x, const int32_t* ids, int64_t n, float* vectors_out) {
    return guarded([&]() -> int {
    if (!vectors_out && n != 0) return fail(DPQ_ERR_ARG, "dpq_reconstruct: NULL argument or n < 0");
    return lookup_host(x, ids, n, nullptr, vectors_out, "dpq_reconstruct");
    });
}

int dpq_get_codes_device(dpq_index* x, const int32_t* d_ids, int64_t n, uint8_t* d_codes, void* hip_stream) {
    return guarded([&]() -> int {
    int rc = lookup_args(x, d_ids, n, d_codes, false, "dpq_get_codes_device");
    if (rc || n == 0) return rc;
    DPQ_HIP(hipSetDevice(x->device));
    return lookup_on_device(x, d_ids, n, d_codes, nullptr, (hipStream_t)hip_stream, "dpq_get_codes_device");
    });
}

int dpq_reconstruct_device(dpq_index* x, const int32_t* d_ids, int64_t n, float* d_vectors, void* hip_stream) {
    return guarded([&]() -> int {
    int rc = lookup_args(x, d_ids, n, d_vectors, true, "dpq_reconstruct_device");
    if (rc || n == 0) return rc;
    DPQ_HIP(hipSetDevice(x->device));
    return lookup_on_device(x, d_ids, n, nullptr, d_vectors, (hipStream_t)hip_stream, "dpq_reconstruct_device");
    });
}

int dpq_decode_range(dpq_index* x, int64_t first, int64_t count, uint8_t* codes_out) {
    return guarded([&]() -> int {
    if (!x || !codes_out) return fail(DPQ_ERR_ARG, "dpq_decode_range: NULL argument");
    if (first < 0 || count < 0 || first < x->info.node_lo || first > x->info.node_hi || count > x->info.node_hi - first)
        return fail(DPQ_ERR_ARG, "dpq_decode_range: [first, first + count) is not inside the handle's [node_lo, node_hi)");
    if (!x->pending.empty())
        if (int rc = dpq_finish(x)) return rc;
    if (count == 0) return DPQ_OK;
    DPQ_HIP(hipSetDevice(x->device));
    const int M = x->M;
    const int64_t l0 = first - x->info.node_lo, l1 = l0 + count;
    if (x->plain) {
        DPQ_HIP(hipMemcpy(codes_out, x->d_raw.get() + (size_t)l0 * M, (size_t)count * M, hipMemcpyDeviceToHost));
        return DPQ_OK;
    }
    LookupWs& lw = x->lookup;
    const int64_t S = (int64_t)dpq::kChunk * x->img.chunks_per_segment;
    const int64_t seg0 = l0 / S, seg1 = (l1 + S - 1) / S;
    const int64_t tile = std::min(std::max<int64_t>(1, kLookupTileNodes / S), seg1 - seg0);
    int rc = grow(lw.tile, &lw.tile_n, (size_t)(tile * S * M));
    if (!rc) rc = grow(lw.tile_segs, &lw.tile_segs_n, (size_t)tile);
    if (rc) return rc;
    std::vector<uint32_t> segs((size_t)tile);
    for (int64_t t0 = seg0; t0 < seg1; t0 += tile) {
        const int64_t nt = std::min(tile, seg1 - t0);
        for (int64_t j = 0; j < nt; ++j) segs[(size_t)j] = (uint32_t)(t0 + j);
        DPQ_HIP(hipMemcpy(lw.tile_segs, segs.data(), (size_t)nt * sizeof(uint32_t), hipMemcpyHostToDevice));
        DPQ_HIP(dpq::launch_decode_list(x->img, lw.tile_segs, (int)nt, nullptr, reinterpret_cast<uint32_t*>(lw.tile.get()),
                                        nullptr));
        const int64_t a = std::max(l0, t0 * S), b = std::min(l1, (t0 + nt) * S);
        DPQ_HIP(hipMemcpy(codes_out + (size_t)(a - l0) * M, lw.tile.get() + (size_t)(a - t0 * S) * M, (size_t)(b - a) * M,
                          hipMemcpyDeviceToHost));
    }
    return DPQ_OK;
    });
}

int dpq_dtc_decode(const uint8_t* payload, int64_t n_bytes, int64_t n_codes, int M, int64_t first, int64_t count,
                   uint8_t* codes_out) {
    return guarded([&]() -> int {
    std::string err;
    int rc = dpq::decode_codes(payload, n_bytes, n_codes, M, first, count, codes_out, &err);
    return rc ? fail(rc, err) : DPQ_OK;
    });
}

int dpq_range_search(dpq_index* x, const float* queries, int nq, const float* radii, dpq_range_result** out) {
    return guarded([&]() -> int {
    if (!out) return fail(DPQ_ERR_ARG, "out is NULL");
    *out = nullptr;
    if (!x || nq < 0 || (nq > 0 && (!queries || !radii))) return fail(DPQ_ERR_ARG, "NULL argument or nq < 0");
    if (!x->d_codebook) return fail(DPQ_ERR_STATE, "dpq_set_codebook has not been called");
    for (int q = 0; q < nq; ++q)
        if (std::isnan(radii[q])) return fail(DPQ_ERR_ARG, "radius of query " + std::to_string(q) + " is NaN");
    if (!x->pending.empty()) {
        int rc = dpq_finish(x);
        if (rc) return rc;
    }
    x->range.last_max_keys = 0;
    std::unique_ptr<dpq_range_result> res(new dpq_range_result());
    res->nq = nq;
    res->lims.assign((size_t)nq + 1, 0);
    if (nq > 0) {
        DPQ_HIP(hipSetDevice(x->device));
        const size_t qf = (size_t)nq * x->M * x->Ds;
        if (qf > x->q_stage_floats) {
            x->q_stage_floats = 0;
            int rc = x->d_q_stage.alloc(qf);
            if (rc) return rc;
            x->q_stage_floats = qf;
        }
        DPQ_HIP(hipMemcpy(x->d_q_stage, queries, qf * sizeof(float), hipMemcpyHostToDevice));
        const int D = x->M * x->Ds;
        int rc = DPQ_OK;
        for (int base = 0; base < nq && !rc; base += kMaxBatchQueries) {
            const int n = std::min(kMaxBatchQueries, nq - base);
            rc = range_batch(x, x->d_q_stage + (size_t)base * D, n, radii + base, base, res.get(), nullptr);
        }
        range_trim(x);
        if (rc) return rc;
        if (x->prof) x->prof_acc.queries += nq;
    }
    *out = res.release();
    return DPQ_OK;
    });
}

int dpq_range_result_get(const dpq_range_result* r, int32_t* nq, const int64_t** lims, const int32_t** ids,
                         const float** dists) {
    if (!r || !nq || !lims || !ids || !dists) return fail(DPQ_ERR_ARG, "NULL argument");
    *nq = r->nq;
    *lims = r->lims.data();
    *ids = r->ids.data();
    *dists = r->dists.data();
    return DPQ_OK;
}

void dpq_range_result_free(dpq_range_result* r) { delete r; }

int dpq_query_batch_host_async(dpq_index* x, const float* queries, int nq, int top_k, int32_t* ids, float* dists) {
    return guarded([&]() -> int {
    int rc = check_batch_args(x, queries, nq, top_k, ids, dists);
    if (rc || nq == 0) return rc;
    DPQ_HIP(hipSetDevice(x->device));
    if (!x->copy_in) {
        DPQ_HIP(hipStreamCreateWithFlags(&x->copy_in, hipStreamNonBlocking));
        DPQ_HIP(hipStreamCreateWithFlags(&x->copy_out, hipStreamNonBlocking));
    }
    int slot = (int)(x->host_seq % dpq_index::kHostSlots);
    if (x->host_slots[slot].busy) {
        if ((rc = dpq_finish(x))) return rc;
// ... 74 lines not shown
                uint32_t bits;
                memcpy(&bits, &dists[o], 4);
                keys.push_back(((uint64_t)bits << 32) | (uint32_t)ids[o]);
            }
        const size_t kk = std::min((size_t)top_k, keys.size());
        std::partial_sort(keys.begin(), keys.begin() + kk, keys.end());
        for (int r = 0; r < top_k; ++r) {
            const size_t o = (size_t)q * top_k + r;
            if ((size_t)r < kk) {
                out_ids[o] = (int32_t)(keys[r] & 0xffffffffu);
                uint32_t bits = (uint32_t)(keys[r] >> 32);
                memcpy(&out_dists[o], &bits, 4);
            } else {
                out_ids[o] = -1;
                out_dists[o] = INFINITY;
            }
        }
    }
    return DPQ_OK;
    });
}

int dpq_merge_topk_device(const int32_t* d_ids, const float* d_dists, int n_lists, int nq, int top_k,
                          int32_t* d_out_ids, float* d_out_dists, int device, void* hip_stream) {
    return guarded([&]() -> int {
    if (!d_ids || !d_dists || !d_out_ids || !d_out_dists || n_lists < 1 || nq < 0 || top_k < 1)
        return fail(DPQ_ERR_ARG, "bad merge argument");
    if ((int64_t)n_lists * top_k > 16384) return fail(DPQ_ERR_ARG, "n_lists * top_k exceeds 16384");
    DPQ_HIP(hipSetDevice(device));
    DPQ_HIP(dpq::launch_merge(d_ids, d_dists, n_lists, nq, top_k, top_k, d_out_ids, d_out_dists,
                              reinterpret_cast<hipStream_t>(hip_stream)));
    return DPQ_OK;
    });
}

int dpq_merge_topk_device_packed(const int32_t* d_packed, int n_lists, int nq, int top_k, int32_t* d_out_ids,
                                 float* d_out_dists, int device, void* hip_stream) {
    return guarded([&]() -> int {
    if (!d_packed || !d_out_ids || !d_out_dists || n_lists < 1 || nq < 0 || top_k < 1)
        return fail(DPQ_ERR_ARG, "bad merge argument");
    if ((int64_t)n_lists * top_k > 16384) return fail(DPQ_ERR_ARG, "n_lists * top_k exceeds 16384");
    DPQ_HIP(hipSetDevice(device));
    DPQ_HIP(dpq::launch_merge(d_packed, reinterpret_cast<const float*>(d_packed + top_k), n_lists, nq, top_k, 2 * top_k,
                              d_out_ids, d_out_dists, reinterpret_cast<hipStream_t>(hip_stream)));
    return DPQ_OK;
    });
}

int dpq_debug_scan_time(dpq_index* x, int nq, int pass_all, int reps, int splits, float* ms_out) {
    return guarded([&]() -> int {
    DPQ_DEV_ONLY();
    if (!x || !ms_out || !x->ws().d_lut32) return fail(DPQ_ERR_STATE, "run a query batch first");
    DPQ_HIP(hipSetDevice(x->device));
    if (pass_all == 3) {
        if (x->dbg_groups <= 0 || x->dbg_boot_slots <= 0) return fail(DPQ_ERR_STATE, "the last batch ran no bootstrap + scan");
        hipEvent_t a, b;
        DPQ_HIP(hipEventCreate(&a));
        DPQ_HIP(hipEventCreate(&b));
        DPQ_HIP(dpq::launch_bootstrap(x->dbg_ba, x->M, x->dbg_boot_slots, nullptr));
        DPQ_HIP(dpq::launch_scan(x->dbg_sa, x->dbg_groups, x->dbg_splits, nullptr));
        DPQ_HIP(hipEventRecord(a, nullptr));
        for (int r = 0; r < reps; ++r) {
            if (x->dbg_sa.tight_hist)
                DPQ_HIP(hipMemsetAsync(x->dbg_sa.tight_hist, 0, sizeof(uint32_t) * dpq::kTightWords * (size_t)x->dbg_boot_slots, nullptr));
            DPQ_HIP(dpq::launch_scan(x->dbg_sa, x->dbg_groups, x->dbg_splits, nullptr));
        }
        DPQ_HIP(hipEventRecord(b, nullptr));
        DPQ_HIP(hipEventSynchronize(b));
        float ms = 0;
        DPQ_HIP(hipEventElapsedTime(&ms, a, b));
        *ms_out = ms / reps;
        hipEventDestroy(a);
        hipEventDestroy(b);
        return DPQ_OK;
    }
    const int QG = dpq::queries_per_group(x->M);
    const int nqp = (nq + QG - 1) / QG * QG;
    const Workspace& w = x->ws();
    if (nqp > w.slots) return fail(DPQ_ERR_ARG, "nq exceeds the workspace");
    dpq::ScanArgs sa = debug_scan_args(x, nq, &splits);
    sa.debug_pass = pass_all == 2 ? 0 : (pass_all ? 2 : 1);
    if (!x->plain && w.d_batch_raw && batch_tile_segments(x) >= x->img.n_segments && !getenv("DPQ_DEBUG_FUSED")) {
        sa.img.raw = w.d_batch_raw;
        if (x->d_relabel) sa.lut32 = w.d_lut32r;
    }
    hipEvent_t a, b;
    DPQ_HIP(hipEventCreate(&a));
    DPQ_HIP(hipEventCreate(&b));
    DPQ_HIP(dpq::launch_quantise(sa, nqp / QG, nullptr));
    DPQ_HIP(dpq::launch_scan(sa, nqp / QG, splits, nullptr));
    DPQ_HIP(hipEventRecord(a, nullptr));
    for (int r = 0; r < reps; ++r) DPQ_HIP(dpq::launch_scan(sa, nqp / QG, splits, nullptr));
    DPQ_HIP(hipEventRecord(b, nullptr));
    DPQ_HIP(hipEventSynchronize(b));
    float ms = 0;
    DPQ_HIP(hipEventElapsedTime(&ms, a, b));
    *ms_out = ms / reps;
    hipEventDestroy(a);
    hipEventDestroy(b);
    if (getenv("DPQ_DEBUG_WG_TIMES")) {
        const int nwg = splits * (nqp / QG);
        DevBuf<unsigned long long> d_t;
        int rc = d_t.alloc((size_t)nwg * 2);
        if (rc) return rc;
        sa.wg_times = d_t;
        DPQ_HIP(dpq::launch_scan(sa, nqp / QG, splits, nullptr));
        DPQ_HIP(hipDeviceSynchronize());
        std::vector<unsigned long long> h((size_t)nwg * 2);
        DPQ_HIP(hipMemcpy(h.data(), d_t, h.size() * 8, hipMemcpyDeviceToHost));
        unsigned long long t0 = ~0ull, t1 = 0;
        for (int i = 0; i < nwg; ++i) t0 = std::min(t0, h[2 * (size_t)i]), t1 = std::max(t1, h[2 * (size_t)i + 1]);
        std::vector<double> st, en, life;
        for (int i = 0; i < nwg; ++i) {
            st.push_back((double)(h[2 * (size_t)i] - t0) / 100.0);
            en.push_back((double)(h[2 * (size_t)i + 1] - t0) / 100.0);
            life.push_back(en.back() - st.back());
        }
        std::sort(st.begin(), st.end()); std::sort(en.begin(), en.end()); std::sort(life.begin(), life.end());
        auto pct = [&](const std::vector<double>& v, double p) { return v[(size_t)(p * (v.size() - 1))]; };
        fprintf(stderr, "scan workgroups (%d, %s codes): span %.1f us; start p50 %.1f max %.1f; end min %.1f p10 %.1f p50 %.1f p90 %.1f max %.1f; "
                        "lifetime min %.1f p50 %.1f max %.1f us; busy %.1f %%\n", nwg, sa.img.raw ? "plain" : "compressed",
                (double)(t1 - t0) / 100.0, pct(st, 0.5), st.back(), en.front(), pct(en, 0.1), pct(en, 0.5), pct(en, 0.9), en.back(),
                life.front(), pct(life, 0.5), life.back(),
                100.0 * std::accumulate(life.begin(), life.end(), 0.0) / (nwg * (double)(t1 - t0) / 100.0));
    }
    return DPQ_OK;
    });
}

int dpq_debug_scan_stamps(dpq_index* x, int nq, int splits, unsigned long long* out, int n_out, float* ms_out) {
    return guarded([&]() -> int {
    DPQ_DEV_ONLY();
    if (!x || !out || !x->ws().d_lut32) return fail(DPQ_ERR_STATE, "run a query batch first");
    if (x->M != 8) return fail(DPQ_ERR_ARG, "the STAMPS build exists for M = 8");
    DPQ_HIP(hipSetDevice(x->device));
    const int QG = dpq::queries_per_group(x->M);
    const int nqp = (nq + QG - 1) / QG * QG;
    if (nqp > x->ws().slots) return fail(DPQ_ERR_ARG, "nq exceeds the workspace");
    const int n = std::min(n_out, dpq::scan_stamp_count());
    DevBuf<unsigned long long> d_st;
    int rc = d_st.alloc((size_t)dpq::scan_stamp_count());
    if (rc) return rc;
    DPQ_HIP(hipMemset(d_st, 0, sizeof(unsigned long long) * dpq::scan_stamp_count()));
    dpq::ScanArgs sa = debug_scan_args(x, nq, &splits);
    sa.stamps = d_st;
    hipEvent_t a, b;
    DPQ_HIP(hipEventCreate(&a));
    DPQ_HIP(hipEventCreate(&b));
    DPQ_HIP(dpq::launch_quantise(sa, nqp / QG, nullptr));
    DPQ_HIP(hipEventRecord(a, nullptr));
    DPQ_HIP(dpq::launch_scan(sa, nqp / QG, splits, nullptr));
    DPQ_HIP(hipEventRecord(b, nullptr));
    DPQ_HIP(hipEventSynchronize(b));
    float ms = 0;
    DPQ_HIP(hipEventElapsedTime(&ms, a, b));
    if (ms_out) *ms_out = ms;
    DPQ_HIP(hipMemcpy(out, d_st, sizeof(unsigned long long) * n, hipMemcpyDeviceToHost));
    hipEventDestroy(a);
    hipEventDestroy(b);
    return DPQ_OK;
    });
}

int dpq_debug_strand1_stamps(dpq_index* x, unsigned long long* out, int n_words) {
    return guarded([&]() -> int {
    DPQ_DEV_ONLY();
// ... 179 lines not shown
```

deltapq_amd/csrc/dpq_format.cpp:

```cpp
#include "dpq_format.h"

#include <algorithm>
#include <cstdio>
#include <cstring>
#include <fstream>

namespace dpq {

static inline int popcnt(unsigned x) { return __builtin_popcount(x); }

DtcWalker::DtcWalker(const uint8_t* payload, int64_t n_bytes, int64_t n_codes, int M)
    : p_(payload), nb_(n_bytes), n_(n_codes), M_(M), mb_(mask_bytes_for(M)), dmask_(depth_field_mask(M)) {}

int DtcWalker::next(NodeRec* rec) {
    char msg[160];
    if (i_ >= n_) {
        err_ = "walk past the last node";
        return DPQ_ERR_FORMAT;
    }
    if (i_ == 0) {
        if (nb_ < M_) {
            err_ = "payload shorter than the root code";
            return DPQ_ERR_FORMAT;
        }
        rec->depth = 0;
        rec->mask = (1u << M_) - 1u;
        rec->deltas = p_;
        rec->n_diff = M_;
        rec->payload_begin = 0;
        rec->payload_end = M_;
        off_ = M_;
        i_ = 1;
        return DPQ_OK;
    }
    int64_t begin = off_;
    int depth;
    if (pending_depth_ >= 0) {
        depth = pending_depth_;
        pending_depth_ = -1;
    } else {
        if (off_ >= nb_) {
            snprintf(msg, sizeof msg, "payload ends before the depth byte of node %lld", (long long)i_);
            err_ = msg;
            return DPQ_ERR_FORMAT;
        }
        int b = p_[off_++];
        if (i_ + 1 < n_) {
            depth = b & dmask_;
            pending_depth_ = (b >> 4) & dmask_;
        } else {
            depth = b;
        }
    }
    if (depth < 1 || depth >= M_ || depth > max_depth_seen_ + 1) {
        snprintf(msg, sizeof msg, "node %lld: depth %d invalid (deepest so far %d, M %d)", (long long)i_, depth,
                 max_depth_seen_, M_);
        err_ = msg;
        return DPQ_ERR_FORMAT;
    }
    if (depth > max_depth_seen_) max_depth_seen_ = depth;
    if (off_ + mb_ > nb_) {
        snprintf(msg, sizeof msg, "payload ends before the mask of node %lld", (long long)i_);
        err_ = msg;
        return DPQ_ERR_FORMAT;
    }
    unsigned mask = p_[off_];
    if (mb_ == 2) mask |= (unsigned)p_[off_ + 1] << 8;
    off_ += mb_;
    if (M_ < 16 && (mask >> M_) != 0) {
        snprintf(msg, sizeof msg, "node %lld: mask 0x%x has bits beyond M=%d", (long long)i_, mask, M_);
        err_ = msg;
        return DPQ_ERR_FORMAT;
    }
    int nd = popcnt(mask);
    if (off_ + nd > nb_) {
        snprintf(msg, sizeof msg, "payload ends inside the changed bytes of node %lld", (long long)i_);
        err_ = msg;
        return DPQ_ERR_FORMAT;
    }
    rec->depth = depth;
    rec->mask = mask;
    rec->deltas = p_ + off_;
    rec->n_diff = nd;
    rec->payload_begin = begin;
    off_ += nd;
    rec->payload_end = off_;
    i_++;
    return DPQ_OK;
}

static int check_args(const uint8_t* payload, int64_t n_bytes, int64_t n_codes, int M, std::string* err) {
    if (!payload || n_bytes < 0 || n_codes < 1 || M < 1 || M > 16) {
        if (err) *err = "bad argument (payload NULL, n_codes < 1 or M outside 1..16)";
        return DPQ_ERR_ARG;
    }
    if (n_codes >= (int64_t)INT32_MAX) {
        if (err) *err = "number of codes does not fit a 32-bit id";
        return DPQ_ERR_ARG;
    }
    const int64_t least = (int64_t)M + (n_codes - 1) * mask_bytes_for(M) + n_codes / 2;
    if (n_bytes < least) {
        if (err) *err = "n_codes in the header needs more payload bytes than n_bytes";
        return DPQ_ERR_FORMAT;
    }
    return DPQ_OK;
}

int validate(const uint8_t* payload, int64_t n_bytes, int64_t n_codes, int M, dpq_dtc_stats* stats,
             std::string* err) {
    int rc = check_args(payload, n_bytes, n_codes, M, err);
    if (rc) return rc;
    dpq_dtc_stats st;
    memset(&st, 0, sizeof st);
    st.n_codes = n_codes;
    st.n_bytes = n_bytes;
    st.M = M;
    DtcWalker w(payload, n_bytes, n_codes, M);
    NodeRec r;
    while (!w.done()) {
        rc = w.next(&r);
        if (rc) {
            if (err) *err = w.error();
            return rc;
        }
        st.depth_hist[r.depth]++;
        if (r.depth > st.max_depth) st.max_depth = r.depth;
        if (w.pos() > 1) st.n_diffs += r.n_diff;
    }
    if (w.offset() != n_bytes) {
        if (err) {
            char msg[160];
            snprintf(msg, sizeof msg, "stream consumed %lld bytes but n_bytes is %lld", (long long)w.offset(),
                     (long long)n_bytes);
            *err = msg;
        }
        return DPQ_ERR_FORMAT;
    }
    if (stats) *stats = st;
    return DPQ_OK;
}

int transcode(const uint8_t* payload, int64_t n_bytes, int64_t n_codes, int M, int shard_rank, int shard_count,
              int chunks_per_segment, SoA* out, std::string* err, int64_t scan_codes, int multi_index_stride,
              int multi_index_classes, int strands) {
    int rc = check_args(payload, n_bytes, n_codes, M, err);
    if (rc) return rc;
    if (scan_codes < 0 || scan_codes > n_codes) {
        if (err) *err = "num_codes (prefix to scan) outside 0..n_codes";
        return DPQ_ERR_ARG;
    }
    const int64_t n_scan = scan_codes > 0 ? scan_codes : n_codes;
    const bool prefix = n_scan < n_codes;
    if (shard_count <= 0) shard_count = 1;
    if (chunks_per_segment <= 0) chunks_per_segment = kDefaultChunksPerSegment;
    if (shard_rank < 0 || shard_rank >= shard_count || chunks_per_segment > 1024) {
        if (err) *err = "bad shard_rank / shard_count / chunks_per_segment";
        return DPQ_ERR_ARG;
    }
    const int64_t S = (int64_t)kChunk * chunks_per_segment;
    const int64_t nseg_total = (n_scan + S - 1) / S;
    const int levels = levels_for(M);
    const int mb = mask_bytes_for(M);

    int64_t seg_lo = 0, seg_hi = nseg_total;
    if (shard_count > 1) {
        std::vector<int64_t> seg_bytes((size_t)nseg_total, 0);
        DtcWalker w(payload, n_bytes, n_codes, M);
        NodeRec r;
        int64_t bytes_scanned = 0;
        while (!w.done() && w.pos() < n_scan) {
            int64_t i = w.pos();
            rc = w.next(&r);
            if (rc) {
                if (err) *err = w.error();
                return rc;
            }
            seg_bytes[(size_t)(i / S)] += r.payload_end - r.payload_begin;
            bytes_scanned += r.payload_end - r.payload_begin;
        }
        if (!prefix && w.offset() != n_bytes) {
            if (err) *err = "stream length does not match n_bytes";
            return DPQ_ERR_FORMAT;
        }
        auto boundary = [&](int r_) -> int64_t {
            if (r_ <= 0) return 0;
            if (r_ >= shard_count) return nseg_total;
            long double target = (long double)bytes_scanned * r_ / shard_count;
            int64_t acc = 0;
            for (int64_t s = 0; s < nseg_total; s++) {
                if ((long double)acc >= target) return s;
                acc += seg_bytes[(size_t)s];
            }
            return nseg_total;
        };
        seg_lo = boundary(shard_rank);
        seg_hi = boundary(shard_rank + 1);
        if (seg_hi < seg_lo) seg_hi = seg_lo;
    }

    SoA& o = *out;
    o = SoA();
    o.M = M;
    o.levels = levels;
    o.mask_bytes = mb;
    o.chunks_per_segment = chunks_per_segment;
    o.n_codes_total = n_scan;
    o.n_bytes_total = n_bytes;
    o.node_lo = std::min(seg_lo * S, n_scan);
    o.node_hi = std::min(seg_hi * S, n_scan);
    o.n_segments = seg_hi - seg_lo;
    const int64_t n_pad = o.n_segments * S;
    o.nib.assign((size_t)(n_pad / 2), 0x00);
    o.par.assign((size_t)n_pad, 0xFF);
    o.carry.assign((size_t)(n_pad / kChunk) * levels, 0xFF);
    o.mask.assign((size_t)(n_pad * mb), 0);
    o.seg_delta_off.assign((size_t)o.n_segments + 1, 0);
    o.seg_ckpt.assign((size_t)(o.n_segments * levels * M), 0);
    o.delta.reserve((size_t)std::min<int64_t>(n_bytes, (o.node_hi - o.node_lo) * (int64_t)M / 2 + 64));

    std::vector<uint8_t> stack((size_t)levels * M, 0);
    int last_lane[16], top_level[64];
    const bool want_relabel = multi_index_stride > 0 && M % 4 == 0;
    const int64_t group_step = std::max<int64_t>(1, (o.node_hi - o.node_lo) / (16 * 65536));
    std::vector<uint32_t> cooc(want_relabel ? (size_t)M * 65536 : 0, 0);
    uint8_t grp[16][16];
    int grp_n = 0;
    std::vector<uint32_t> mi_ids;
    std::vector<uint8_t> mi_codes;
    if (multi_index_stride > 0) {
        mi_ids.reserve((size_t)((o.node_hi - o.node_lo) / multi_index_stride + 1));
        mi_codes.reserve((size_t)((o.node_hi - o.node_lo) / multi_index_stride + 1) * M);
    }
    const bool want_strands = multi_index_stride > 0 && M == 8 && strands != 0;
    constexpr int kPhases = kRunLen / kPhaseLen;
    std::vector<uint8_t> strip_bytes;
    std::vector<uint8_t> strip_cnt;
    if (want_strands) {
        o.n_strips = (o.node_hi - o.node_lo + kStripNodes - 1) / kStripNodes;
        o.st_ckpt.assign((size_t)o.n_strips * levels * 64, 0);
        o.st_mask.assign((size_t)o.n_strips * (kRunLen / 4) * 64, 0u);
        o.st_depth.assign((size_t)o.n_strips * (kRunLen / 4) * 64, 0x1111u);
        o.st_poff.assign((size_t)o.n_strips * kPhases * 64, 0);
        o.st_pbase.assign((size_t)o.n_strips * kPhases + 1, 0);
        strip_bytes.assign((size_t)kStripNodes * 8, 0);
        strip_cnt.assign((size_t)kStripNodes, 0);
    }
    auto flush_strip = [&](int64_t strip) {
        for (int ph = 0; ph < kPhases; ++ph) {
            o.st_pbase[(size_t)(strip * kPhases + ph)] = (uint32_t)(o.st_delta.size() / 16);
            size_t used = 0;
            for (int lane = 0; lane < 64; ++lane) {
                o.st_poff[(size_t)((strip * kPhases + ph) * 64 + lane)] = (uint16_t)used;
                for (int st = ph * kPhaseLen; st < (ph + 1) * kPhaseLen; ++st) {
                    const size_t node = (size_t)lane * kRunLen + st;
                    o.st_delta.insert(o.st_delta.end(), &strip_bytes[node * 8], &strip_bytes[node * 8] + strip_cnt[node]);
                    used += strip_cnt[node];
                }
            }
            o.st_delta.resize((o.st_delta.size() + 15) / 16 * 16, 0);
        }
        std::fill(strip_cnt.begin(), strip_cnt.end(), 0);
    };
    DtcWalker w(payload, n_bytes, n_codes, M);
    NodeRec r;
    while (!w.done()) {
        const int64_t i = w.pos();
        if ((shard_count > 1 || prefix) && i >= o.node_hi) break;
        if (want_strands && i >= o.node_lo && i < o.node_hi && (i - o.node_lo) % kRunLen == 0) {
            const int64_t l = i - o.node_lo, strip = l / kStripNodes;
            const int lane = (int)((l % kStripNodes) / kRunLen);
            for (int lv = 0; lv < levels; ++lv) memcpy(&o.st_ckpt[(size_t)((strip * levels + lv) * 64 + lane)], &stack[(size_t)lv * M], 8);
        }
        if (i >= o.node_lo && i < o.node_hi && (i - o.node_lo) % S == 0) {
            const int64_t t = (i - o.node_lo) / S;
            memcpy(&o.seg_ckpt[(size_t)(t * levels * M)], stack.data(), (size_t)levels * M);
            o.seg_delta_off[(size_t)t] = o.delta.size();
        }
        rc = w.next(&r);
        if (rc) {
            if (err) *err = w.error();
            return rc;
        }
        uint8_t* cur = &stack[(size_t)r.depth * M];
        if (r.depth > 0) memcpy(cur, &stack[(size_t)(r.depth - 1) * M], (size_t)M);
        int j = 0;
        for (int m = 0; m < M; m++)
            if (r.mask & (1u << m)) cur[m] = r.deltas[j++];
        if (i >= o.node_lo && i < o.node_hi) {
            const int64_t l = i - o.node_lo;
            const int lane = (int)(l % kChunk);
            if (lane == 0)
                for (int d = 0; d < 16; ++d) last_lane[d] = -1;
            const int pl = r.depth > 0 ? last_lane[r.depth - 1] : -1;
            const int level = pl >= 0 ? top_level[pl] : (r.depth > 0 ? r.depth - 1 : 0);
            top_level[lane] = level;
            last_lane[r.depth] = lane;
            o.par[(size_t)l] = pl >= 0 ? (uint8_t)pl : 0xFF;
            o.carry[(size_t)(l / kChunk) * levels + r.depth] = (uint8_t)lane;
            uint8_t& nb = o.nib[(size_t)(l >> 1)];
            if (l & 1)
                nb = (uint8_t)((nb & 0x0F) | (level << 4));
            else
                nb = (uint8_t)((nb & 0xF0) | level);
            o.mask[(size_t)(l * mb)] = (uint8_t)(r.mask & 0xFF);
            if (mb == 2) o.mask[(size_t)(l * mb + 1)] = (uint8_t)(r.mask >> 8);
            o.delta.insert(o.delta.end(), r.deltas, r.deltas + r.n_diff);
            if (want_strands) {
                const int64_t strip = l / kStripNodes, in_strip = l % kStripNodes;
                const int s_lane = (int)(in_strip / kRunLen), step = (int)(in_strip % kRunLen);
                const size_t hw = (size_t)((strip * (kRunLen / 4) + step / 4) * 64 + s_lane);
                o.st_mask[hw] |= (uint32_t)(r.mask & 0xFFu) << (8 * (step % 4));
                o.st_depth[hw] = (uint16_t)((o.st_depth[hw] & ~(0xFu << (4 * (step % 4)))) | ((unsigned)r.depth << (4 * (step % 4))));
                memcpy(&strip_bytes[(size_t)in_strip * 8], r.deltas, (size_t)r.n_diff);
                strip_cnt[(size_t)in_strip] = (uint8_t)r.n_diff;
                if (in_strip + 1 == kStripNodes || i + 1 == o.node_hi) flush_strip(strip);
            }
            o.algorithmic_bytes += r.payload_end - r.payload_begin;
            if (i > 0) o.n_diffs += r.n_diff;
            if (r.depth > o.max_depth) o.max_depth = r.depth;
            if (multi_index_stride > 0 && l % multi_index_stride == 0) {
                mi_ids.push_back((uint32_t)i);
                mi_codes.insert(mi_codes.end(), cur, cur + M);
            }
            if (want_relabel && (l / 16) % group_step == 0) {
                for (int m = 0; m < M; ++m) grp[m][grp_n] = cur[m];
                if (++grp_n == 16 || i + 1 == o.node_hi) {
                    for (int m = 0; m < M; ++m) {
                        uint8_t* v = grp[m];
                        std::sort(v, v + grp_n);
                        const int nd = (int)(std::unique(v, v + grp_n) - v);
                        uint32_t* Wm = &cooc[(size_t)m * 65536];
                        for (int x = 0; x < nd; ++x)
                            for (int y = x + 1; y < nd; ++y) {
                                Wm[(size_t)v[x] * 256 + v[y]]++;
                                Wm[(size_t)v[y] * 256 + v[x]]++;
                            }
                    }
                    grp_n = 0;
                }
            }
        }
    }
    if (want_relabel) {
        o.relabel.assign((size_t)M * 256, 0);
        for (int m = 0; m < M; ++m) {
            const uint32_t* Wm = &cooc[(size_t)m * 65536];
            std::vector<uint64_t> weight(256, 0);
            for (int a = 0; a < 256; ++a)
                for (int b = 0; b < 256; ++b) weight[(size_t)a] += Wm[(size_t)a * 256 + b];
            std::vector<int> order(256);
            for (int a = 0; a < 256; ++a) order[(size_t)a] = a;
            std::stable_sort(order.begin(), order.end(), [&](int a, int b) { return weight[(size_t)a] > weight[(size_t)b]; });
            int load[16] = {0};
            std::vector<uint64_t> cost(256 * 16, 0);
            int colour[256];
            for (int a : order) {
                int best = -1;
                for (int c = 0; c < 16; ++c)
                    if (load[c] < 16 && (best < 0 || cost[(size_t)a * 16 + c] < cost[(size_t)a * 16 + best] ||
                                         (cost[(size_t)a * 16 + c] == cost[(size_t)a * 16 + best] && load[c] < load[best])))
                        best = c;
                colour[a] = best;
                load[best]++;
                for (int b = 0; b < 256; ++b) cost[(size_t)b * 16 + best] += Wm[(size_t)b * 256 + a];
            }
            int seen[16] = {0};
            for (int a = 0; a < 256; ++a) o.relabel[(size_t)m * 256 + a] = (uint8_t)(colour[a] + 16 * seen[colour[a]]++);
        }
    }
    if (multi_index_stride > 0)
        build_multi_index(mi_ids, mi_codes, M, multi_index_stride,
                          multi_index_classes > 0 ? multi_index_classes : bootstrap_classes_for((int64_t)mi_ids.size()), &o);
    if (w.done() && w.offset() != n_bytes) {
        if (err) {
            char msg[160];
            snprintf(msg, sizeof msg, "stream consumed %lld bytes but n_bytes is %lld", (long long)w.offset(),
                     (long long)n_bytes);
            *err = msg;
        }
        return DPQ_ERR_FORMAT;
    }
    o.seg_delta_off[(size_t)o.n_segments] = o.delta.size();
    o.delta.resize(o.delta.size() + 32, 0);
    if (want_strands) {
        o.st_pbase[(size_t)o.n_strips * kPhases] = (uint32_t)(o.st_delta.size() / 16);
        o.st_delta.resize(o.st_delta.size() + 48, 0);
        if (o.st_delta.size() / 16 > 0xffffffffull) {
            if (err) *err = "strand image beyond 64 GB of changed bytes";
            return DPQ_ERR_NOMEM;
        }
    }
    return DPQ_OK;
}

void build_multi_index(const std::vector<uint32_t>& ids, const std::vector<uint8_t>& codes, int M, int stride, int classes,
                       SoA* out) {
    const size_t n = ids.size(), W = (size_t)M / 4;
    const size_t P = (size_t)std::min(std::max(classes, 1), kBootPairs);
    out->mi_stride = stride;
    out->mi_classes = (int)P;
    out->mi_cell_start.assign(P * 65537, 0);
    out->mi_code.assign(n * W, 0);
    out->mi_id.assign(n, 0);
    auto cls = [&](size_t e) { return e % P; };
    auto cell_of = [&](size_t e) {
        const int s = bootstrap_pair_subspace(M, (int)cls(e));
        return (size_t)codes[e * M + s] | ((size_t)codes[e * M + s + 1] << 8);
    };
    for (size_t e = 0; e < n; ++e) out->mi_cell_start[cls(e) * 65537 + cell_of(e) + 1]++;
    uint32_t run = 0;
    for (size_t p = 0; p < P; ++p) {
        uint32_t* cs = &out->mi_cell_start[p * 65537];
        cs[0] = run;
        for (size_t c = 0; c < 65536; ++c) cs[c + 1] += cs[c];
        run = cs[65536];
    }
    std::vector<uint32_t> fill(P * 65536);
    for (size_t p = 0; p < P; ++p)
        for (size_t c = 0; c < 65536; ++c) fill[p * 65536 + c] = out->mi_cell_start[p * 65537 + c];
    for (size_t e = 0; e < n; ++e) {
        const size_t pos = fill[cls(e) * 65536 + cell_of(e)]++;
        out->mi_id[pos] = ids[e];
        memcpy(&out->mi_code[pos * W], &codes[e * M], (size_t)M);
    }
}

int encode(const uint8_t* root_code, const uint8_t* depths, const uint16_t* masks, const uint8_t* deltas,
           int64_t n_codes, int M, uint8_t* out, int64_t* n_bytes, std::string* err) {
    if (!root_code || !depths || !masks || n_codes < 1 || M < 1 || M > 16 || !n_bytes) {
        if (err) *err = "bad argument";
        return DPQ_ERR_ARG;
    }
    const int mb = mask_bytes_for(M);
    int64_t nd = 0;
    for (int64_t i = 1; i < n_codes; i++) nd += popcnt(masks[i]);
    const int64_t total = M + nd + (n_codes - 1) * mb + (n_codes - 1 + 1) / 2;
    *n_bytes = total;
    if (!out) return DPQ_OK;
    int64_t off = 0, doff = 0;
    for (int m = 0; m < M; m++) out[off++] = root_code[m];
    auto put_node = [&](int64_t i) {
        out[off++] = (uint8_t)(masks[i] & 0xFF);
        if (mb == 2) out[off++] = (uint8_t)(masks[i] >> 8);
        int c = popcnt(masks[i]);
        for (int j = 0; j < c; j++) out[off++] = deltas[doff++];
    };
    int64_t i = 1;
    for (; i + 1 < n_codes; i += 2) {
        if (depths[i] < 1 || depths[i] >= M || depths[i + 1] < 1 || depths[i + 1] >= M) {
            if (err) *err = "depth outside 1..M-1";
            return DPQ_ERR_ARG;
        }
        out[off++] = (uint8_t)(depths[i] | (depths[i + 1] << 4));
        put_node(i);
        put_node(i + 1);
    }
    if (i == n_codes - 1) {
        if (depths[i] < 1 || depths[i] >= M) {
            if (err) *err = "depth outside 1..M-1";
            return DPQ_ERR_ARG;
        }
        out[off++] = depths[i];
        put_node(i);
    }
    if (off != total) {
        if (err) *err = "internal: encoded size mismatch";
        return DPQ_ERR_FORMAT;
    }
    return DPQ_OK;
}

int decode_codes(const uint8_t* payload, int64_t n_bytes, int64_t n_codes, int M, int64_t first, int64_t count,
                 uint8_t* codes_out, std::string* err) {
    int rc = validate(payload, n_bytes, n_codes, M, nullptr, err);
    if (rc) return rc;
// ... 150 lines not shown
```

deltapq_amd/csrc/dpq_format.h:

```cpp
#pragma once
#include <cstdint>
#include <string>
#include <vector>

#include "../../include/deltapq_amd.h"

namespace dpq {

constexpr int kChunk = 64;
constexpr int kBootPairs = 4;
constexpr int kRunLen = 64;
constexpr int kStripNodes = 64 * kRunLen;
constexpr int kPhaseLen = 4;
constexpr int kDefaultChunksPerSegment = 2;

inline int mask_bytes_for(int M) { return M > 8 ? 2 : 1; }
inline int depth_field_mask(int M) { return M > 8 ? 15 : 7; }
inline int levels_for(int M) { return M > 8 ? 16 : 8; }

struct NodeRec {
    int depth;
    unsigned mask;
    const uint8_t* deltas;
    int n_diff;
    int64_t payload_begin;
    int64_t payload_end;
};

class DtcWalker {
public:
    DtcWalker(const uint8_t* payload, int64_t n_bytes, int64_t n_codes, int M);
    int next(NodeRec* rec);
    int64_t pos() const { return i_; }
    bool done() const { return i_ >= n_; }
    int64_t offset() const { return off_; }
    const std::string& error() const { return err_; }

private:
    const uint8_t* p_;
    int64_t nb_, n_;
    int M_, mb_, dmask_;
    int64_t i_ = 0, off_ = 0;
    int pending_depth_ = -1;
    int max_depth_seen_ = 0;
    std::string err_;
};

struct SoA {
    int M = 8;
    int levels = 8;
    int mask_bytes = 1;
    int chunks_per_segment = kDefaultChunksPerSegment;
    int64_t n_codes_total = 0, n_bytes_total = 0;
    int64_t node_lo = 0, node_hi = 0;
    int64_t n_segments = 0;
    int64_t algorithmic_bytes = 0;
    int64_t n_diffs = 0;
    int max_depth = 0;
    std::vector<uint8_t> nib;
    std::vector<uint8_t> par;
    std::vector<uint8_t> carry;
    std::vector<uint8_t> mask;
    std::vector<uint8_t> delta;
    std::vector<uint64_t> seg_delta_off;
    std::vector<uint8_t> seg_ckpt;
    int mi_stride = 0;
    int mi_classes = 0;
    std::vector<uint32_t> mi_cell_start;
    std::vector<uint32_t> mi_code;
    std::vector<uint32_t> mi_id;
    std::vector<uint8_t> relabel;
    int64_t n_strips = 0;
    std::vector<uint64_t> st_ckpt;
    std::vector<uint32_t> st_mask;
    std::vector<uint16_t> st_depth;
    std::vector<uint16_t> st_poff;
    std::vector<uint32_t> st_pbase;
    std::vector<uint8_t> st_delta;
    int64_t strand_bytes() const {
        return (int64_t)(st_ckpt.size() * 8 + st_mask.size() * 4 + st_depth.size() * 2 + st_pbase.size() * 4 + st_delta.size());
    }
    int64_t nodes_per_segment() const { return (int64_t)kChunk * chunks_per_segment; }
    int64_t device_bytes() const {
        return (int64_t)(nib.size() + par.size() + carry.size() + mask.size() + delta.size() + seg_delta_off.size() * 8 +
                         seg_ckpt.size());
    }
    int64_t bootstrap_bytes() const { return (int64_t)((mi_cell_start.size() + mi_code.size() + mi_id.size()) * 4); }
};

int validate(const uint8_t* payload, int64_t n_bytes, int64_t n_codes, int M, dpq_dtc_stats* stats, std::string* err);
int transcode(const uint8_t* payload, int64_t n_bytes, int64_t n_codes, int M, int shard_rank, int shard_count,
              int chunks_per_segment, SoA* out, std::string* err, int64_t scan_codes = 0, int multi_index_stride = 0,
              int multi_index_classes = 0, int strands = -1);
constexpr int64_t kStrandMinNodes = (int64_t)8 << 20;
void build_multi_index(const std::vector<uint32_t>& ids, const std::vector<uint8_t>& codes, int M, int stride, int classes,
                       SoA* out);
inline int bootstrap_pair_subspace(int M, int p) { return 2 * p * (M / 8); }
constexpr int64_t kBootstrapMinNodes = 65536;
inline int bootstrap_stride_for(int64_t n_local) {
    if (n_local < kBootstrapMinNodes) return 0;
    return (int)((n_local + (1 << 22) - 1) >> 22);
}
inline int bootstrap_classes_for(int64_t n_sampled) { return n_sampled >= 4 * 65536 ? kBootPairs : 1; }
int encode(const uint8_t* root_code, const uint8_t* depths, const uint16_t* masks, const uint8_t* deltas,
           int64_t n_codes, int M, uint8_t* out, int64_t* n_bytes, std::string* err);
int decode_codes(const uint8_t* payload, int64_t n_bytes, int64_t n_codes, int M, int64_t first, int64_t count,
                 uint8_t* codes_out, std::string* err);

int read_file(const std::string& path, std::vector<uint8_t>* out, std::string* err);
int read_dtc_header(const std::string& path, int64_t* n_codes, int64_t* n_bytes, std::string* err);
int read_codewords(const std::string& path, int* M, int* K, int* Ds, std::vector<float>* out, std::string* err);
int read_vecs(const std::string& path, bool is_bvecs, int64_t* n, int* D, std::vector<float>* out, int64_t cap,
              std::string* err);
std::string dtc_file_name(const std::string& dir, int M, int K, int64_t N);

}
```

deltapq_amd/csrc/dpq_kernels.h:

```cpp
#pragma once
#include <hip/hip_runtime.h>

#include <cstdint>

#include "dpq_format.h"

namespace dpq {

constexpr int kScanThreads = 1024;
constexpr int kScanWaves = kScanThreads / 64;
constexpr int kMaxTopK = 2048;
constexpr int kSelectThreads = 512;
constexpr int kMaxSplits = 256;
constexpr int kRegionStride = 1 + kMaxSplits;
constexpr int kLevel0Nodes = 3840;
constexpr int kSortMax = 4096;
constexpr int queries_per_group(int M) { return M <= 8 ? 64 : 32; }
constexpr int kTightBuckets = 8;
constexpr int kTightSplits = 32;
constexpr int kTightWords = kTightSplits * kTightBuckets / 4;
constexpr int kS1Replicas = 8, kS1ReplicaWords = 512;
constexpr int kS1HistWords = kS1Replicas * kS1ReplicaWords;
static_assert(queries_per_group(8) * kTightWords >= kS1HistWords, "strand1's histogram exceeds what one query group clears");

struct DeviceImage {
    const uint8_t* nib = nullptr;
    const uint8_t* par = nullptr;
    const uint8_t* carry = nullptr;
    const uint8_t* mask = nullptr;
    const uint8_t* delta = nullptr;
    const uint64_t* seg_delta_off = nullptr;
    const uint8_t* seg_ckpt = nullptr;
    const uint8_t* raw = nullptr;
    const uint64_t* st_ckpt = nullptr;
    const uint32_t* st_mask = nullptr;
    const uint16_t* st_depth = nullptr;
    const uint32_t* st_pbase = nullptr;
    const uint8_t* st_delta = nullptr;
    int32_t n_strips = 0;
    int64_t n_local = 0;
    int64_t n_codes_total = 0;
    uint32_t id_base = 0;
    int32_t n_segments = 0;
    int32_t chunks_per_segment = 4;
    int32_t M = 8, K = 256;
};

struct ScanArgs {
    DeviceImage img;
    const uint32_t* seg_list;
    int32_t n_seg_pass;
    const float* lut32;
    const float* lut_min;
    const uint64_t* thr_key;
    const int32_t* slot_query;
    int32_t n_queries;
    int32_t debug_pass;
    unsigned long long* wg_times;
    int32_t raw_by_pos;
    int32_t append;
    int32_t fp32_accum;
    uint32_t* cand_count;
    uint64_t* cand_key;
    int64_t cand_stride;
    int32_t region_off, region_cap;
    unsigned long long* counters;
    uint4* qtab;
    unsigned long long* stamps;
    uint32_t* tight_hist;
    int32_t tight_k;
    const uint32_t* filter;
};

struct SelectArgs {
    const uint32_t* shared_id;
    const uint32_t* shared_code;
    int32_t shared_n;
    uint32_t* cand_count;
    uint64_t* cand_key;
    int64_t cand_stride;
    int32_t region_off, region_cap;
    int32_t n_regions;
    uint64_t* scratch;
    const float* lut32;
    const int32_t* slot_query;
    int32_t top_k;
    int32_t final_pass;
    uint64_t* thr_key;
    uint32_t* overflow;
    uint32_t* any_overflow;
    int32_t* out_ids;
    float* out_dists;
    int64_t n_codes_total;
    int32_t fp32_accum;
    int32_t keep_thr;
    unsigned long long* stamps;
    int32_t threads;
    int32_t fast_final;
};

struct BootArgs {
    const uint8_t* relabel;
    const uint8_t* nbr;
    const uint32_t* cell_start;
    int32_t n_classes;
    const uint32_t* mi_code;
    const uint32_t* mi_id;
    const float* lut32;
    const int32_t* slot_query;
    int32_t top_k;
    int32_t target;
    int32_t cap;
    uint64_t* thr_key;
    uint32_t* cand_count;
    int32_t fp32_accum;
    int32_t n_queries;
    uint4* qtab;
    const float* lut_min;
    unsigned long long* stamps;
    int32_t variant;
    const uint32_t* filter;
    uint32_t id_base;
    int32_t eval_cap;
};

hipError_t launch_filter_ids(const uint32_t* ids, int n, const uint32_t* filter, uint32_t id_base, uint32_t* out,
                             hipStream_t stream);

constexpr int kRangeMaxQueries = 2048;
constexpr int kRangeCountThreads = 1024;
constexpr int kRangeEmitThreads = 256;
constexpr int kRangeLdsKeys = 8192;

struct RangeCountArgs {
    const int32_t* slot_query;
    const uint32_t* cand_count;
    int32_t n_slots, n_regions, n_queries;
    uint32_t* max_count;
    int64_t* lims;
};

struct RangeEmitArgs {
    const int64_t* out_off;
    const uint32_t* cand_count;
    const uint64_t* cand_key;
    int64_t cand_stride;
    int32_t region_off, region_cap, n_regions;
    int32_t lds_keys;
    int32_t* out_ids;
    float* out_dists;
    int64_t out_n;
    uint64_t* scratch;
    int64_t n_codes_total;
};

hipError_t launch_lut_build(const float* d_codebook, const float* d_queries, int nq, int n_slots, int M, int K, int Ds,
                            float* d_lut32, float* d_lut_min, uint32_t* d_cand_count, uint32_t* d_overflow,
                            const uint8_t* d_relabel, float* d_lut_labels, uint32_t* d_tight_hist,
                            hipStream_t stream);
hipError_t launch_decode_list(const DeviceImage& img, const uint32_t* seg_list, int n_seg, const uint8_t* relabel,
                              uint32_t* out_code, hipStream_t stream);
hipError_t launch_decode_segments(const DeviceImage& img, const uint32_t* seg_list, int n_seg, uint32_t* out_id,
                                  uint32_t* out_code, hipStream_t stream);
hipError_t launch_stream(const ScanArgs& a, int n_slots, hipStream_t stream);
hipError_t launch_strand(const ScanArgs& a, int n_slots, hipStream_t stream);
int stream_queries_per_pass(int M, int n_slots);
hipError_t launch_strand1(const ScanArgs& a, int n_slots, hipStream_t stream);
int strand1_workgroups(int n_strips);
constexpr int kStrand1Regions = 256;
hipError_t launch_quantise(const ScanArgs& a, int n_slot_groups, hipStream_t stream);
hipError_t launch_scan(const ScanArgs& a, int n_slot_groups, int splits, hipStream_t stream);
size_t qtab_bytes_per_group(int M);
int scan_stamp_count();
hipError_t launch_select(const SelectArgs& a, int M, int n_slots, hipStream_t stream);
hipError_t launch_bootstrap(const BootArgs& a, int M, int n_slots, hipStream_t stream);
hipError_t launch_range_count(const RangeCountArgs& a, hipStream_t stream);
hipError_t launch_range_emit(const RangeEmitArgs& a, int n_slots, hipStream_t stream);
hipError_t launch_merge(const int32_t* d_ids, const float* d_dists, int n_lists, int nq, int top_k, int row_stride,
                        int32_t* d_out_ids, float* d_out_dists, hipStream_t stream);
hipError_t launch_encode_pq(const float* d_vectors, int64_t n, int D, const float* d_codebook, int M, int K, int Ds,
                            uint8_t* d_codes, hipStream_t stream);
size_t scan_lds_bytes(int M);
size_t select_lds_bytes(int M, int top_k, int n_shared);

}
```

deltapq_amd/csrc/dpq_kernels.hip:

```cpp
#include "dpq_kernels.h"
#include "dpq_wave_decoder.h"

#include <atomic>
#include <type_traits>
#include <cfloat>
#include <cmath>

namespace dpq {

static hipError_t ensure_dynamic_lds(const void* fn, size_t bytes, std::atomic<bool>* done);


__device__ __forceinline__ uint32_t and_or(uint32_t a, uint32_t mask, uint32_t c) {
    uint32_t r;
    asm("v_and_or_b32 %0, %1, %2, %3" : "=v"(r) : "v"(a), "s"(mask), "v"(c));
    return r;
}

__device__ __forceinline__ uint64_t make_key(float d, uint32_t id) {
    return ((uint64_t)__float_as_uint(d) << 32) | (uint64_t)id;
}

constexpr int kLutQueries = 8;
constexpr int kLutMinParts = 4;
// ... 19 lines not shown
        if (overflow) overflow[q0 + k] = 0;
    }
    if (m == 0 && tight_hist)
        for (int i = k; i < kLutQueries * kTightWords; i += 256)
            if (q0 * kTightWords + i < n_slots * kTightWords) tight_hist[(size_t)q0 * kTightWords + i] = 0;
    if (q0 >= nq) return;
    float acc[kLutQueries];
#pragma unroll
    for (int j = 0; j < kLutQueries; ++j) acc[j] = 0.0f;
    if (k < K) {
        const float* c = codebook + ((size_t)m * K + k) * Ds;
        const float* qv = queries + (size_t)q0 * M * Ds + (size_t)m * Ds;
        const size_t qstride = (size_t)M * Ds;
        auto step = [&](float& a, float cv, float qd) {
            const float diff = __fsub_rn(cv, qd);
            const double sq = __dmul_rn((double)diff, (double)diff);
            a = (float)__dadd_rn((double)a, sq);
        };
        if ((Ds & 3) == 0) {
            const float4* c4 = reinterpret_cast<const float4*>(c);
            for (int d = 0; d < Ds; d += 4) {
                const float4 v = c4[d >> 2];
#pragma unroll
                for (int j = 0; j < kLutQueries; ++j) {
                    const float* qj = qv + (size_t)min(j, nq - 1 - q0) * qstride + d;
                    step(acc[j], v.x, qj[0]);
                    step(acc[j], v.y, qj[1]);
                    step(acc[j], v.z, qj[2]);
                    step(acc[j], v.w, qj[3]);
                }
            }
        } else {
            for (int d = 0; d < Ds; ++d) {
                const float cv = c[d];
#pragma unroll
                for (int j = 0; j < kLutQueries; ++j) step(acc[j], cv, qv[(size_t)min(j, nq - 1 - q0) * qstride + d]);
            }
        }
    } else {
#pragma unroll
        for (int j = 0; j < kLutQueries; ++j) acc[j] = INFINITY;
    }
#pragma unroll
    for (int j = 0; j < kLutQueries; ++j) {
        if (q0 + j < nq) lut[((size_t)(q0 + j) * M + m) * 256 + k] = acc[j];
        if (lut_labels && q0 + j < nq) lut_labels[((size_t)(q0 + j) * M + m) * 256 + relabel[m * 256 + k]] = acc[j];
        uint32_t v = __float_as_uint(acc[j]);
#pragma unroll
        for (int o = 32; o > 0; o >>= 1) v = min(v, (uint32_t)__shfl_xor((int)v, o));
        if ((k & 63) == 0 && q0 + j < nq) lut_min[((size_t)(q0 + j) * M + m) * kLutMinParts + (k >> 6)] = __uint_as_float(v);
    }
}

template <int M>
__global__ __launch_bounds__(64) void decode_segments_kernel(const DeviceImage img,
                                                              const uint32_t* __restrict__ seg_list,
                                                              uint32_t* __restrict__ out_id,
                                                              uint32_t* __restrict__ out_code) {
    constexpr int W = Cfg<M>::W;
    const int lane = threadIdx.x;
    const uint32_t seg = seg_list ? seg_list[blockIdx.x] : blockIdx.x;
    const int cps = img.chunks_per_segment;
    WaveDecoder<M> dec;
    if (!img.raw) dec.begin_segment(img, seg, lane);
    for (int c = 0; c < cps; ++c) {
        const int64_t node = ((int64_t)seg * cps + c) * 64 + lane;
        uint32_t code[W];
        if (img.raw) {
#pragma unroll
            for (int w = 0; w < W; ++w) code[w] = reinterpret_cast<const uint32_t*>(img.raw)[(size_t)node * W + w];
        } else {
            dec.step(img, node, lane, c + 1 < cps, code);
        }
        const size_t o = ((size_t)blockIdx.x * cps + c) * 64 + lane;
        out_id[o] = node < img.n_local ? img.id_base + (uint32_t)node : 0xffffffffu;
#pragma unroll
        for (int w = 0; w < W; ++w) out_code[W * o + w] = code[w];
    }
}

template <int M>
__global__ __launch_bounds__(256) void decode_list_kernel(const DeviceImage img, const uint32_t* __restrict__ seg_list,
                                                           int n_seg, const uint8_t* __restrict__ relabel,
                                                           uint32_t* __restrict__ out_code) {
    constexpr int W = Cfg<M>::W;
    __builtin_amdgcn_s_setprio(DPQ_UNDER_SCAN_PRIO);
    const int lane = threadIdx.x & 63;
    const int64_t j = (int64_t)blockIdx.x * 4 + (threadIdx.x >> 6);
    if (j >= n_seg) return;
    const int64_t seg = seg_list ? (int64_t)seg_list[j] : j;
    const int cps = img.chunks_per_segment;
    WaveDecoder<M> dec;
    dec.begin_segment(img, (uint32_t)seg, lane);
    for (int c = 0; c < cps; ++c) {
        const int64_t node = (seg * cps + c) * 64 + lane;
        const int64_t out = (j * cps + c) * 64 + lane;
        uint32_t code[W];
        dec.step(img, node, lane, c + 1 < cps, code);
        if (relabel) {
#pragma unroll
            for (int w = 0; w < W; ++w) {
                uint32_t r = 0;
#pragma unroll
                for (int b = 0; b < 4; ++b) r |= (uint32_t)relabel[(4 * w + b) * 256 + ((code[w] >> (8 * b)) & 0xffu)] << (8 * b);
                code[w] = r;
            }
        }
        if constexpr (W == 2)
            reinterpret_cast<uint2*>(out_code)[out] = make_uint2(code[0], code[1]);
        else
            reinterpret_cast<uint4*>(out_code)[out] = make_uint4(code[0], code[1], code[2], code[3]);
    }
}

template <int M>
__device__ __forceinline__ float exact_dist(const float* __restrict__ T, const uint32_t* __restrict__ c, bool fp32_accum) {
    if (fp32_accum) {
        float fsum = 0.0f;
#pragma unroll
        for (int m = 0; m < M; ++m) fsum = __fadd_rn(fsum, T[m * 256 + ((c[m >> 2] >> (8 * (m & 3))) & 0xffu)]);
        return fsum;
    }
    double dsum = 0.0;
#pragma unroll
    for (int m = 0; m < M; ++m) {
        const uint32_t byte = (c[m >> 2] >> (8 * (m & 3))) & 0xffu;
        dsum = __dadd_rn(dsum, (double)T[m * 256 + byte]);
    }
    return (float)dsum;
}

struct FilterScale {
    float s32;
    uint32_t bias;
    double B;
};

template <int M>
__device__ __forceinline__ FilterScale filter_scale(uint64_t key, const float* __restrict__ lut_min, size_t q) {
    using C = Cfg<M>;
    FilterScale r{0.0f, 0u, 0.0};
    double B = 0.0;
#pragma unroll
    for (int mm = 0; mm < M; ++mm) B += (double)lut_min_of(lut_min, q, M, mm);
    const double taup = (double)__uint_as_float((uint32_t)(key >> 32)) * (1.0 + 0x1p-20);
    const double R = taup - B;
    r.B = B;
    if (key != ~0ull && R > 0.0 && R < 1e300) {
        r.s32 = (float)((double)C::QT / R * (1.0 - 0x1p-20));
        r.bias = C::R == 1 ? (uint32_t)C::BIAS : 0u;
    }
    return r;
}

template <int M>
__device__ __forceinline__ float filter_offset(const FilterScale& fs, float min_m, int m) {
    const float mn = fs.s32 != 0.0f ? min_m : 0.0f;
    const double od = (double)mn * (double)fs.s32;
    float of = (float)od;
    if ((double)of < od) of = __uint_as_float(__float_as_uint(of) + 1u);
    const double sd = (m == 0 ? (double)fs.bias : 0.0) - 0.5 - (double)of;
    float sf = (float)sd;
    if ((double)sf > sd) sf = __uint_as_float(__float_as_uint(sf) + (sf > 0.0f ? -1 : 1));
    return sf;
}

template <int M>
__device__ __forceinline__ uint32_t filter_field(float tv, float sc, float of, uint32_t bias_m) {
    using C = Cfg<M>;
    const float fv = fminf(__fmaf_rn(tv, sc, of), (float)C::SAT + (float)bias_m);
    return __builtin_amdgcn_cvt_pk_u8_f32(fv, 0u, 0u);
}

template <int M>
__device__ __forceinline__ void write_filter_fields(uint4* qtab, int slot, const float* T, float sc, const float* of_m,
                                                    uint32_t bias, const uint8_t* __restrict__ relabel, int tid, int nthreads) {
    using C = Cfg<M>;
    constexpr int F = C::F, AB = C::AB, R = C::R, QG = C::QG, NG = C::NG, J = C::J;
    const int group = slot / QG, ls = slot % QG;
    const int f = (ls % (J * F)) / J, acc = (ls / (J * F)) * AB + ls % J;
    const int d = acc / R, tb = f * R + acc % R;
    const int g = d >> 2, c = d & 3;
    unsigned char* base = reinterpret_cast<unsigned char*>(qtab + ((size_t)group * NG + g) * M * 256) + c * 4 + tb;
    for (int e = tid; e < M * 256; e += nthreads) {
        const int m = e >> 8;
        const uint32_t v = T ? filter_field<M>(T[e], sc, of_m[m], m == 0 ? bias : 0u) : C::reject_entry(m);
        const int row = relabel ? (m << 8) + relabel[e] : e;
        base[(size_t)row * 16] = (unsigned char)v;
    }
// ... 266 lines not shown
            if (!frozen) h[(size_t)split * QG] = mine;
            uint32_t cnt[kTightBuckets];
#pragma unroll
            for (int e = 0; e < kTightBuckets; ++e) cnt[e] = 0;
            const int n_rows = (int)gridDim.x;
            for (int r0 = 0; r0 < n_rows; r0 += 4) {
                uint32_t w[8];
#pragma unroll
                for (int j = 0; j < 4; ++j) {
                    const uint64_t g = r0 + j < n_rows ? __hip_atomic_load(reinterpret_cast<const uint64_t*>(h + (size_t)(r0 + j) * QG),
                                                                            __ATOMIC_RELAXED, __HIP_MEMORY_SCOPE_WORKGROUP) : 0ull;
                    w[2 * j] = (uint32_t)g, w[2 * j + 1] = (uint32_t)(g >> 32);
                }
#pragma unroll
                for (int j = 0; j < 4; ++j) {
                    const uint32_t lo = r0 + j == split ? mine.x : w[2 * j], hi = r0 + j == split ? mine.y : w[2 * j + 1];
#pragma unroll
                    for (int e = 0; e < 4; ++e) cnt[e] += (lo >> (8 * e)) & 0xffu, cnt[4 + e] += (hi >> (8 * e)) & 0xffu;
                }
            }
            uint32_t c = 0;
            int best = 0;
#pragma unroll
            for (int e = C::XMAX; e >= 1; --e) {
                c += cnt[e];
                if (best == 0 && c >= (uint32_t)a.tight_k) best = e;
            }
            if (best > my_steps) {
                raise = (uint32_t)((best - my_steps) * C::XU);
                my_steps = best;
                const double t2 = ((double)s_bdn[ls] + (double)(C::QT - best * C::XU) / (double)s_scale[ls]) / (1.0 + 0x1p-20);
                const uint64_t key = ((uint64_t)__float_as_uint(__double2float_ru(t2)) << 32) | 0xffffffffull;
                if (key < s_thr[ls]) s_thr[ls] = key;
                const int f = (ls % (C::J * F)) / C::J, acc = (ls / (C::J * F)) * EB + ls % C::J;
                field = C::R == 1 ? acc * 4 + f : acc * 2 + f;
            }
        }
        if constexpr (C::R == 1) {
            if (__ballot(raise != 0)) {
                if (raise != 0) reinterpret_cast<volatile uint8_t*>(s_extra)[field] = (uint8_t)raise;
                __builtin_amdgcn_wave_barrier();
                asm volatile("" ::: "memory");
#pragma unroll
                for (int g = 0; g < NG; ++g) {
                    const uint4 d = reinterpret_cast<const uint4*>(s_extra)[g];
                    if ((d.x | d.y | d.z | d.w) == 0) continue;
#pragma unroll
                    for (int i = 0; i < 4; ++i) {
                        uint4 v = lut[(g * M) * 256 + lane + 64 * i];
                        v.x += d.x, v.y += d.y, v.z += d.z, v.w += d.w;
                        lut[(g * M) * 256 + lane + 64 * i] = v;
                    }
                }
                __builtin_amdgcn_wave_barrier();
                if (lane < NA) s_extra[lane] = 0;
                __builtin_amdgcn_wave_barrier();
            }
        } else {
            if (raise != 0) reinterpret_cast<volatile uint16_t*>(s_extra)[field] = (uint16_t)(C::BIAS + my_steps * C::XU);
        }
    };
    const bool helper = TIGHT && __builtin_amdgcn_readfirstlane(tid) >= kScanThreads - 64;
    uint32_t* wg_done = wg_checks + 2;

    int entry_pos = 0;
    auto next_entry = [&]() -> int {
        int j = 0;
        if (lane == 0) j = (int)atomicAdd(wg_next, 1u);
        j = __builtin_amdgcn_readfirstlane(j);
        const int s = split + (int)gridDim.x * j;
        if (s >= a.n_seg_pass) return -1;
        entry_pos = s;
        return __builtin_amdgcn_readfirstlane(a.seg_list ? (int)a.seg_list[s] : s);
    };
    struct Chunk {
        int seg, c;
        int pos;
        typename WaveDecoder<M>::In in;
        uint32_t carry_lane;
        uint64_t h_doff;
        uint32_t h_stk[W];
        typename WaveDecoder<M>::Ld ld;
        uint32_t raw[W];
    };
    int nlane = lane;
    if constexpr (PLAIN) {
        const int h = lane & 31;
        const int g = (h >= 4 && h < 12) || (h >= 16 && h < 20) || h >= 28;
        const int pos = h < 4 ? h : h < 12 ? h - 4 : h < 16 ? h - 8 : h < 20 ? h - 8 : h < 28 ? h - 12 : h - 16;
        nlane = (lane & 32) + 16 * g + pos;
    }
    auto node_of = [&](const Chunk& k) { return ((int64_t)k.seg * cps + k.c) * 64 + nlane; };
    auto stage1 = [&](Chunk& k) {
        if (k.seg < 0) return;
        const int64_t node = node_of(k);
        if (PLAIN) {
#pragma unroll
            for (int w = 0; w < W; ++w) {
                const int64_t at = a.raw_by_pos ? ((int64_t)k.pos * cps + k.c) * 64 + nlane : node;
                k.raw[w] = reinterpret_cast<const uint32_t*>(a.img.raw)[(size_t)at * W + w];
            }
        } else {
            k.in = WaveDecoder<M>::load_in(a.img, node);
            k.carry_lane = 0xffu;
            if (k.c + 1 < cps && lane < C::LEVELS) k.carry_lane = a.img.carry[(size_t)(node >> 6) * C::LEVELS + lane];
            if (k.c == 0) {
                k.h_doff = a.img.seg_delta_off[k.seg];
#pragma unroll
                for (int w = 0; w < W; ++w) k.h_stk[w] = 0;
                if (lane < C::LEVELS) {
                    const uint32_t* ck = reinterpret_cast<const uint32_t*>(a.img.seg_ckpt) + ((size_t)k.seg * C::LEVELS + lane) * W;
#pragma unroll
                    for (int w = 0; w < W; ++w) k.h_stk[w] = ck[w];
                }
            }
        }
    };
    uint64_t at = 0;
    auto stage2 = [&](Chunk& k) {
        if (k.seg < 0 || PLAIN) return;
        if (k.c == 0) at = k.h_doff;
        k.ld = WaveDecoder<M>::load_delta(a.img, k.in, node_of(k), at);
    };
    auto successor = [&](const Chunk& k) {
        Chunk n;
        n.seg = k.seg;
        n.pos = k.pos;
        n.c = k.c + 1;
        if (k.seg >= 0 && n.c == cps) {
            n.seg = next_entry();
            n.pos = entry_pos;
            n.c = 0;
        }
        return n;
    };
    Chunk A, B, Cn;
    uint32_t fwA = 0, fwB = 0, fwC = 0;
    auto filter_word = [&](const Chunk& k) -> uint32_t { return k.seg < 0 ? 0u : a.filter[(size_t)node_of(k) >> 5]; };
    A.seg = helper ? -1 : next_entry();
    A.pos = entry_pos;
    A.c = 0;
    stage1(A);
    if constexpr (FILT) fwA = filter_word(A);
    B = successor(A);
    stage1(B);
    if constexpr (FILT) fwB = filter_word(B);
    stage2(A);
    stamp(kStSegment);
    while (A.seg >= 0) {
        if constexpr (PLAIN) {
#pragma unroll
            for (int w = 0; w < W; ++w) asm volatile("" ::"v"(A.raw[w]), "v"(B.raw[w]));
        } else {
            asm volatile("" ::"v"(A.ld.level), "v"(A.ld.mk), "v"(A.ld.par), "v"(A.carry_lane), "v"(B.in.nb), "v"(B.in.mk),
                         "v"(B.in.par), "v"(B.carry_lane));
#pragma unroll
            for (int h = 0; h < W / 2; ++h)
                asm volatile("" ::"v"(A.ld.w[h][0]), "v"(A.ld.w[h][1]), "v"(A.ld.w[h][2]), "v"(A.ld.t[h].x), "v"(A.ld.t[h].y));
#pragma unroll
            for (int w = 0; w < W; ++w) asm volatile("" ::"v"(A.h_stk[w]), "v"(B.h_stk[w]));
        }
        if constexpr (FILT) asm volatile("" ::"v"(fwA), "v"(fwB));
        Cn = successor(B);
        stage2(B);
        stage1(Cn);
        if constexpr (FILT) fwC = filter_word(Cn);
        {
            const int64_t node = node_of(A);
            uint32_t code[W];
            if (PLAIN) {
#pragma unroll
                for (int w = 0; w < W; ++w) code[w] = A.raw[w];
            } else {
                if (A.c == 0) {
#pragma unroll
                    for (int w = 0; w < W; ++w) dec.stk[w] = A.h_stk[w];
                }
                dec.finish(A.ld, lane, A.carry_lane, code);
            }
            if constexpr (STAMPS) {
                st[kStSteps] += 1;
                asm volatile("" ::"v"(code[0]), "v"(code[W - 1]));
            }
            stamp(kStDecode);

            uint32_t acc[NA];
            uint32_t fold_h[MD] = {};
            if constexpr (C::R == 1 && DPQ_GATHER_PIPE > 0) {
                static_assert(NG * 8 == 32 && (DPQ_GATHER_PIPE % 2) == 0 && DPQ_GATHER_PIPE >= 2 && DPQ_GATHER_PIPE <= 14, "window of read pairs");
                uint32_t off[8];
#pragma unroll
                for (int m = 0; m < 8; ++m) off[m] = (code[m >> 2] >> (8 * (m & 3))) & 0xffu;
                uint4 gv[32];
#define DPQ_RD(r) gv[r] = lut[(((r) >> 3) * M + ((r) & 7)) * 256 + off[(r) & 7]]
#pragma unroll
                for (int r = 0; r < DPQ_GATHER_PIPE; r += 2) {
                    DPQ_RD(r);
                    DPQ_RD(r + 1);
                    __builtin_amdgcn_sched_barrier(0);
                }
#pragma unroll
                for (int p = 0; p < 16; ++p) {
                    if (2 * p + DPQ_GATHER_PIPE < 32) {
                        DPQ_RD(2 * p + DPQ_GATHER_PIPE);
                        DPQ_RD(2 * p + DPQ_GATHER_PIPE + 1);
                    }
                    __builtin_amdgcn_sched_barrier(0);
                    const int g = p >> 2;
                    const uint4 x = gv[2 * p], y = gv[2 * p + 1];
                    if ((p & 3) == 0) {
                        acc[4 * g + 0] = x.x + y.x;
                        acc[4 * g + 1] = x.y + y.y;
                        acc[4 * g + 2] = x.z + y.z;
                        acc[4 * g + 3] = x.w + y.w;
                    } else {
                        acc[4 * g + 0] += x.x + y.x;
                        acc[4 * g + 1] += x.y + y.y;
                        acc[4 * g + 2] += x.z + y.z;
                        acc[4 * g + 3] += x.w + y.w;
                    }
                    if ((p & 3) == 3) {
#pragma unroll
                        for (int j = 4 * g; j < 4 * g + 4; ++j)
                            fold_h[j / EB] = and_or(acc[j], C::LOW << (EB - 1), fold_h[j / EB] >> 1);
                    }
                    __builtin_amdgcn_sched_barrier(0);
                }
#undef DPQ_RD
            } else
#pragma unroll
            for (int g = 0; g < NG; ++g) {
                if constexpr (C::R == 1) {
                    uint4 v[8];
#pragma unroll
                    for (int m = 0; m < 8; ++m) {
                        const uint32_t byte = (code[m >> 2] >> (8 * (m & 3))) & 0xffu;
                        v[m] = lut[(g * M + m) * 256 + byte];
                    }
                    acc[4 * g + 0] = ((v[0].x + v[1].x + v[2].x) + v[3].x + v[4].x) + (v[5].x + v[6].x + v[7].x);
                    acc[4 * g + 1] = ((v[0].y + v[1].y + v[2].y) + v[3].y + v[4].y) + (v[5].y + v[6].y + v[7].y);
                    acc[4 * g + 2] = ((v[0].z + v[1].z + v[2].z) + v[3].z + v[4].z) + (v[5].z + v[6].z + v[7].z);
                    acc[4 * g + 3] = ((v[0].w + v[1].w + v[2].w) + v[3].w + v[4].w) + (v[5].w + v[6].w + v[7].w);
                } else {
                    uint32_t lo[4], hi[4];
                    if constexpr (TIGHT) {
                        asm volatile("" ::: "memory");
                        const uint4 e0 = reinterpret_cast<const uint4*>(s_extra)[2 * g], e1 = reinterpret_cast<const uint4*>(s_extra)[2 * g + 1];
                        lo[0] = e0.x, hi[0] = e0.y, lo[1] = e0.z, hi[1] = e0.w, lo[2] = e1.x, hi[2] = e1.y, lo[3] = e1.z, hi[3] = e1.w;
                    } else {
#pragma unroll
                        for (int c = 0; c < 4; ++c) lo[c] = hi[c] = (uint32_t)C::BIAS * C::LOW;
                    }
#pragma unroll
                    for (int m0 = 0; m0 < M; m0 += C::PRE) {
                        uint32_t p[4] = {0, 0, 0, 0};
#pragma unroll
                        for (int mm = 0; mm < C::PRE; ++mm) {
                            const int m = m0 + mm;
                            const uint32_t byte = (code[m >> 2] >> (8 * (m & 3))) & 0xffu;
                            const uint4 v = lut[(g * M + m) * 256 + byte];
                            p[0] += v.x, p[1] += v.y, p[2] += v.z, p[3] += v.w;
                        }
#pragma unroll
                        for (int c = 0; c < 4; ++c) {
                            lo[c] += __builtin_amdgcn_perm(0u, p[c], 0x0c020c00u);
                            hi[c] += __builtin_amdgcn_perm(0u, p[c], 0x0c030c01u);
                        }
                    }
#pragma unroll
                    for (int c = 0; c < 4; ++c) {
                        acc[(4 * g + c) * 2 + 0] = lo[c];
                        acc[(4 * g + c) * 2 + 1] = hi[c];
                    }
                }
            }
            if constexpr (STAMPS) {
#pragma unroll
                for (int i = 0; i < NA; ++i) asm volatile("" ::"v"(acc[i]));
            }
            stamp(kStGather);
            bool valid = node < a.img.n_local;
            if constexpr (FILT) valid = valid && ((fwA >> ((uint32_t)node & 31u)) & 1u) != 0u;
            uint64_t pend = 0;
#pragma unroll
            for (int h = 0; h < MD; ++h) {
                uint32_t fail = 0;
                if constexpr (C::R == 1 && DPQ_GATHER_PIPE > 0) {
                    fail = fold_h[h];
                } else {
#pragma unroll
                    for (int j = 0; j < C::J; ++j) fail = and_or(acc[EB * h + j], C::LOW << (EB - 1), fail >> 1);
                }
                fail >>= EB - C::J;
                pend |= (uint64_t)(valid ? (~fail & live) : 0u) << (32 * h);
            }
            const uint64_t pushing = __ballot(pend != 0);
            stamp(kStFold);
            if (pushing) {
                const int cnt = (int)__popcll(pushing);
                while (rq_n + cnt > QCAP) {
                    refine(min(rq_n, 64));
                    stamp(kStRefine);
                }
                if (pend != 0) {
                    int pos = rq_head + rq_n + (int)mbcnt64(pushing, 0);
                    pos = pos >= QCAP ? pos - QCAP : pos;
#pragma unroll
                    for (int w = 0; w < W; ++w) rq_code[pos * W + w] = code[w];
                    rq_id[pos] = a.img.id_base + (uint32_t)node;
                    rq_mask[pos * MD] = (uint32_t)pend;
                    if constexpr (MD == 2) rq_mask[pos * MD + 1] = (uint32_t)(pend >> 32);
                }
                rq_n += cnt;
                stamp(kStPush);
            }
        }
        A = B;
        B = Cn;
        if constexpr (FILT) fwA = fwB, fwB = fwC;
    }
    while (rq_n > 0) refine(min(rq_n, 64));
    stamp(kStRefine);
    if constexpr (TIGHT) {
        if (helper) {
            for (;;) {
                tighten();
                if (__builtin_amdgcn_readfirstlane((int)*reinterpret_cast<volatile uint32_t*>(wg_done)) >= kScanWaves - 1) break;
                __builtin_amdgcn_s_sleep(DPQ_TIGHT_SLEEP);
            }
        } else if (lane == 0) {
            atomicAdd(wg_done, 1u);
        }
    }
    if (a.counters || STAMPS) {
#pragma unroll
        for (int off = 32; off > 0; off >>= 1) my_pairs += (uint32_t)__shfl_xor((int)my_pairs, off, 64);
        if (a.counters && lane == 0) atomicAdd(wg_checks, my_pairs);
        if constexpr (STAMPS) st[kStEntries] += my_pairs;
    }

    __syncthreads();
    if (a.counters && tid < 64) {
        uint32_t c = 0;
        for (int q = tid; q < QG; q += 64)
            c += wg_count[q] - (a.append ? a.cand_count[(size_t)(slot0 + q) * kRegionStride + 1 + split] : 0u);
#pragma unroll
        for (int off = 32; off > 0; off >>= 1) c += (uint32_t)__shfl_xor((int)c, off, 64);
        if (tid == 0) {
            atomicAdd(&a.counters[0], (unsigned long long)*wg_checks);
            atomicAdd(&a.counters[1], (unsigned long long)c);
        }
    }
    __syncthreads();
    if (tid < QG) a.cand_count[(size_t)(slot0 + tid) * kRegionStride + 1 + split] = wg_count[tid];
    if (a.wg_times && tid == 0) a.wg_times[2 * (blockIdx.y * gridDim.x + blockIdx.x) + 1] = __builtin_amdgcn_s_memrealtime();
    if constexpr (STAMPS) {
        st[kStTotal] = __builtin_amdgcn_s_memtime() - t_start;
        st[kStWaves] = 1;
        if (a.stamps && lane == 0)
            for (int i = 0; i < kStCount; ++i) atomicAdd(&a.stamps[i], (unsigned long long)st[i]);
    }
}

template <int Q>
constexpr int stream_threads() { return Q >= 4 ? 512 : 256; }
// ... 1851 lines not shown
        sv[d * 256 + tid] = (v < n && col < D) ? vectors[(size_t)v * D + col] : 0.0f;
    }
    __syncthreads();
    if (v >= n) return;
    float best = FLT_MAX;
    int best_k = 0;
    for (int k = 0; k < K; ++k) {
        float dist = 0.0f;
        for (int d = 0; d < Ds; ++d) {
            const float diff = __fsub_rn(sv[d * 256 + tid], cw[k * Ds + d]);
            dist = __fadd_rn(dist, __fmul_rn(diff, diff));
        }
        if (dist < best) {
            best = dist;
            best_k = k;
        }
    }
    codes[(size_t)v * M + m] = (uint8_t)best_k;
}


static hipError_t ensure_dynamic_lds(const void* fn, size_t bytes, std::atomic<bool>* done) {
    int dev = 0;
    hipError_t e = hipGetDevice(&dev);
    if (e != hipSuccess) return e;
    if (dev < 0 || dev >= 64 || !done[dev].load(std::memory_order_acquire)) {
        e = hipFuncSetAttribute(fn, hipFuncAttributeMaxDynamicSharedMemorySize, (int)bytes);
        if (e != hipSuccess) return e;
        if (dev >= 0 && dev < 64) done[dev].store(true, std::memory_order_release);
    }
    return hipSuccess;
}

hipError_t launch_encode_pq(const float* d_vectors, int64_t n, int D, const float* d_codebook, int M, int K, int Ds,
                            uint8_t* d_codes, hipStream_t stream) {
    if (n <= 0) return hipSuccess;
    const size_t lds = ((size_t)K * Ds + (size_t)Ds * 256) * sizeof(float);
    if (lds > 160 * 1024) return hipErrorInvalidValue;
    static std::atomic<bool> done[64] = {};
    hipError_t e = ensure_dynamic_lds(reinterpret_cast<const void*>(&encode_pq_kernel), 160 * 1024, done);
    if (e != hipSuccess) return e;
    hipLaunchKernelGGL(encode_pq_kernel, dim3((unsigned)((n + 255) / 256), (unsigned)M), dim3(256), lds, stream,
                       d_vectors, n, D, d_codebook, M, K, Ds, d_codes);
    return hipGetLastError();
}

size_t scan_lds_bytes(int M) { return M <= 8 ? ScanLds<8>::kBytes : ScanLds<16>::kBytes; }

size_t select_lds_bytes(int M, int top_k, int n_shared) {
    size_t kp = 1;
    while (kp < (size_t)top_k) kp <<= 1;
    const size_t n_keys = n_shared > 0 ? (size_t)std::min(n_shared, kSortMax) : (size_t)select_list_keys(top_k);
    const size_t area = n_shared > 0 ? kp : (size_t)select_area_keys(top_k);
    const size_t select_bytes = area * 8 + 266 * 4, table_bytes = n_shared > 0 ? (size_t)M * 256 * 4 : 0;
    return n_keys * 8 + std::max(select_bytes, table_bytes) + 16;
}

hipError_t launch_lut_build(const float* d_codebook, const float* d_queries, int nq, int n_slots, int M, int K, int Ds,
                            float* d_lut32, float* d_lut_min, uint32_t* d_cand_count, uint32_t* d_overflow,
                            const uint8_t* d_relabel, float* d_lut_labels, uint32_t* d_tight_hist, hipStream_t stream) {
    if (nq <= 0) return hipSuccess;
    n_slots = std::max(n_slots, nq);
    hipLaunchKernelGGL(lut_build_kernel, dim3((unsigned)((n_slots + kLutQueries - 1) / kLutQueries), (unsigned)M),
                       dim3(256), 0, stream, d_codebook, d_queries, nq, n_slots, M, K, Ds, d_lut32, d_lut_min,
                       d_cand_count, d_overflow, d_relabel, d_relabel ? d_lut_labels : nullptr, d_tight_hist);
    return hipGetLastError();
}

hipError_t launch_decode_segments(const DeviceImage& img, const uint32_t* seg_list, int n_seg, uint32_t* out_id,
                                  uint32_t* out_code, hipStream_t stream) {
    if (n_seg <= 0) return hipSuccess;
    if (img.M == 8)
        hipLaunchKernelGGL(decode_segments_kernel<8>, dim3((unsigned)n_seg), dim3(64), 0, stream, img, seg_list,
                           out_id, out_code);
    else if (img.M == 16)
        hipLaunchKernelGGL(decode_segments_kernel<16>, dim3((unsigned)n_seg), dim3(64), 0, stream, img, seg_list,
                           out_id, out_code);
    else
        return hipErrorInvalidValue;
    return hipGetLastError();
}

hipError_t launch_decode_list(const DeviceImage& img, const uint32_t* seg_list, int n_seg, const uint8_t* relabel,
                              uint32_t* out_code, hipStream_t stream) {
    if (n_seg <= 0) return hipSuccess;
    const unsigned grid = (unsigned)((n_seg + 3) / 4);
    if (img.M == 8)
        hipLaunchKernelGGL(decode_list_kernel<8>, dim3(grid), dim3(256), 0, stream, img, seg_list, n_seg, relabel, out_code);
    else if (img.M == 16)
        hipLaunchKernelGGL(decode_list_kernel<16>, dim3(grid), dim3(256), 0, stream, img, seg_list, n_seg, relabel, out_code);
    else
        return hipErrorInvalidValue;
    return hipGetLastError();
}

template <int M, bool PLAIN, bool STAMPS, bool TIGHT = false>
static hipError_t launch_scan_m(const ScanArgs& a, int n_slot_groups, int splits, hipStream_t stream) {
    static std::atomic<bool> done[64] = {};
    hipError_t e = ensure_dynamic_lds(reinterpret_cast<const void*>(&scan_kernel<M, PLAIN, STAMPS, TIGHT>), scan_lds_bytes(M), done);
    if (e != hipSuccess) return e;
    hipLaunchKernelGGL((scan_kernel<M, PLAIN, STAMPS, TIGHT>), dim3((unsigned)splits, (unsigned)n_slot_groups),
                       dim3(kScanThreads), scan_lds_bytes(M), stream, a);
    return hipGetLastError();
}

template <int M, bool PLAIN, bool TIGHT>
static hipError_t launch_scan_filtered_m(const ScanArgs& a, int n_slot_groups, int splits, hipStream_t stream) {
    static std::atomic<bool> done[64] = {};
    hipError_t e = ensure_dynamic_lds(reinterpret_cast<const void*>(&scan_kernel<M | kFiltered, PLAIN, false, TIGHT>),
                                      scan_lds_bytes(M), done);
    if (e != hipSuccess) return e;
    hipLaunchKernelGGL((scan_kernel<M | kFiltered, PLAIN, false, TIGHT>), dim3((unsigned)splits, (unsigned)n_slot_groups),
                       dim3(kScanThreads), scan_lds_bytes(M), stream, a);
    return hipGetLastError();
}

template <int M, int Q>
static hipError_t launch_stream_mq(const ScanArgs& a, int n_slots, hipStream_t stream) {
    const size_t lds = (size_t)Q * M * 256 * sizeof(float);
    static std::atomic<bool> done[64] = {};
    hipError_t e = ensure_dynamic_lds(reinterpret_cast<const void*>(&stream_kernel<M, Q>), lds, done);
    if (e != hipSuccess) return e;
    const int passes = (n_slots + Q - 1) / Q;
    constexpr int threads = stream_threads<Q>(), waves = threads / 64;
    const int per_cu = std::max(1, std::min(32 / waves, (int)(160 * 1024 / lds)));
    const int wgs = std::max(1, std::min(256 * per_cu / std::max(1, std::min(passes, 8)), (a.n_seg_pass + waves - 1) / waves));
    hipLaunchKernelGGL((stream_kernel<M, Q>), dim3((unsigned)wgs, (unsigned)passes), dim3(threads), lds, stream, a);
    return hipGetLastError();
}

int stream_queries_per_pass(int M, int n_slots) {
    (void)M;
    return n_slots <= 1 ? 1 : n_slots <= 2 ? 2 : 4;
}

hipError_t launch_stream(const ScanArgs& a, int n_slots, hipStream_t stream) {
    if (a.n_seg_pass <= 0 || n_slots <= 0) return hipSuccess;
    const int q = stream_queries_per_pass(a.img.M, n_slots);
    if (a.img.M == 8) {
        switch (q) {
            case 1: return launch_stream_mq<8, 1>(a, n_slots, stream);
            case 2: return launch_stream_mq<8, 2>(a, n_slots, stream);
            default: return launch_stream_mq<8, 4>(a, n_slots, stream);
        }
    }
    if (a.img.M == 16) {
        switch (q) {
            case 1: return launch_stream_mq<16, 1>(a, n_slots, stream);
            case 2: return launch_stream_mq<16, 2>(a, n_slots, stream);
            default: return launch_stream_mq<16, 4>(a, n_slots, stream);
        }
    }
    return hipErrorInvalidValue;
}

template <int Q>
static hipError_t launch_strand_q(const ScanArgs& a, int n_slots, hipStream_t stream) {
    const size_t lds = StrandLds<Q>::kBytes;
    static std::atomic<bool> done[64] = {};
    hipError_t e = ensure_dynamic_lds(reinterpret_cast<const void*>(&strand_kernel<Q>), lds, done);
    if (e != hipSuccess) return e;
    const int passes = (n_slots + Q - 1) / Q;
    const int per_cu = std::max(1, std::min(8, (int)(160 * 1024 / lds)));
    const int wgs = std::max(1, std::min(256 * per_cu / std::max(1, std::min(passes, 8)), (a.n_seg_pass + 3) / 4));
    hipLaunchKernelGGL((strand_kernel<Q>), dim3((unsigned)wgs, (unsigned)passes), dim3(kStrandThreads), lds, stream, a);
    return hipGetLastError();
}

#ifndef DPQ_S1_MAX_WGS
#define DPQ_S1_MAX_WGS 256
#endif
int strand1_workgroups(int n_strips) { return std::max(1, std::min(DPQ_S1_MAX_WGS, n_strips)); }

// ... 121 lines not shown
```

include/deltapq_amd.h:

```cpp
#ifndef DELTAPQ_AMD_H
#define DELTAPQ_AMD_H

#include <stdint.h>

#ifdef __cplusplus
extern "C" {
#endif

#define DPQ_VERSION 100

typedef enum dpq_status {
    DPQ_OK = 0,
    DPQ_ERR_ARG = -1,
    DPQ_ERR_IO = -2,
    DPQ_ERR_FORMAT = -3,
    DPQ_ERR_NO_DEVICE = -4,
    DPQ_ERR_HIP = -5,
    DPQ_ERR_NOMEM = -6,
    DPQ_ERR_STATE = -7,
    DPQ_ERR_TOPK = -8
} dpq_status;

typedef struct dpq_index dpq_index;
typedef struct dpq_soa dpq_soa;
typedef struct dpq_tree dpq_tree;

typedef struct dpq_open_opts {
    int32_t device;
    int32_t shard_rank;
    int32_t shard_count;
    int32_t chunks_per_segment;
    int32_t cand_capacity;
    int32_t num_codes;
    int32_t bootstrap;
    int32_t batch_decode;
    int64_t global_offset;
    int64_t global_n_codes;
    int32_t stream_max_queries;
    int32_t coarse_below;
    int32_t plan_ratios[3];
    int32_t boot_cap;
    int32_t boot_target;
    int32_t flags;
    int64_t batch_tile_nodes;
} dpq_open_opts;

#define DPQ_OPT_NO_RELABEL 1u
#define DPQ_OPT_NO_FUSE_QUANTISE 2u
#define DPQ_OPT_NO_ASYNC_OVERLAP 4u
#define DPQ_OPT_BOOT_FULLSORT 8u
#define DPQ_OPT_NO_TIGHTEN 16u
#define DPQ_OPT_NO_STRANDS 32u
#define DPQ_OPT_FORCE_STRANDS 64u
#define DPQ_OPT_NO_STRAND1 128u

typedef struct dpq_info {
    int64_t n_codes_total;
    int64_t n_bytes_total;
    int64_t node_lo, node_hi;
    int64_t algorithmic_bytes;
    int64_t device_bytes;
    int64_t n_diffs;
    int32_t M, K, Ds;
    int32_t n_segments;
    int32_t chunks_per_segment;
    int32_t max_depth;
    int32_t device;
    int32_t cand_capacity;
    int64_t bootstrap_bytes;
    int32_t bootstrap_stride;
    int32_t batch_decode_mb;
    int64_t strand_bytes;
} dpq_info;

typedef struct dpq_profile {
    double lut_ms, scan_ms, select_ms;
    int64_t lut_launches, scan_launches, select_launches;
    int64_t scan_node_query_pairs;
    int64_t scan_stream_bytes;
    int64_t query_batches, queries;
    int64_t overflow_reruns;
    int64_t exact_checks;
    int64_t candidates;
    double quantise_ms;
    double decode_ms;
    double bootstrap_ms;
    int64_t bootstrap_launches;
    int64_t stream_launches, strand_launches, strand1_launches;
} dpq_profile;

typedef struct dpq_dtc_stats {
    int64_t n_codes, n_bytes, n_diffs;
    int64_t depth_hist[16];
    int32_t max_depth;
    int32_t M;
} dpq_dtc_stats;

int dpq_version(void);
const char* dpq_strerror(int status);
const char* dpq_last_error(void);
int dpq_device_count(void);

int dpq_read_dtc_header(const char* path, int64_t* n_codes, int64_t* n_bytes);
int dpq_read_codewords(const char* path, int32_t* M, int32_t* K, int32_t* Ds, float* out);
int dpq_read_vecs(const char* path, int is_bvecs, int64_t* n, int32_t* D, float* out, int64_t cap);
int dpq_dtc_file_name(const char* dataset_dir, int M, int K, int64_t N, char* out, int64_t out_len);

int dpq_dtc_validate(const uint8_t* payload, int64_t n_bytes, int64_t n_codes, int M, dpq_dtc_stats* stats);
int dpq_soa_build(const uint8_t* payload, int64_t n_bytes, int64_t n_codes, int M, const dpq_open_opts* opts,
                  dpq_soa** out);
int dpq_soa_info(const dpq_soa* soa, dpq_info* info);
int dpq_soa_array(const dpq_soa* soa, int which, const void** ptr, int64_t* n_bytes);
void dpq_soa_free(dpq_soa* soa);
int dpq_dtc_encode(const uint8_t* root_code, const uint8_t* depths, const uint16_t* masks, const uint8_t* deltas,
                   int64_t n_codes, int M, uint8_t* out, int64_t* n_bytes);
int dpq_dtc_decode(const uint8_t* payload, int64_t n_bytes, int64_t n_codes, int M, int64_t first, int64_t count,
                   uint8_t* codes_out);

int dpq_tree_build(const uint8_t* codes, int64_t n_codes, int M, int K, int max_height_folds, const float* codewords,
                   int Ds, dpq_tree** out);
int dpq_tree_build_gpu(const uint8_t* codes, int64_t n_codes, int M, int K, int max_height_folds,
                       const float* codewords, int Ds, int device, dpq_tree** out);
int dpq_tree_stats(const dpq_tree* t, dpq_dtc_stats* stats);
int dpq_tree_array(const dpq_tree* t, int which, const void** ptr, int64_t* n_bytes);
int dpq_tree_encode(const dpq_tree* t, uint8_t* out, int64_t* n_bytes);
int dpq_tree_write_files(const dpq_tree* t, const char* dataset_dir);
void dpq_tree_free(dpq_tree* t);
int dpq_read_qnode_ids(const char* path, int64_t n_codes, uint32_t* vec_ids);
int dpq_read_codes_plain(const char* path, int M, int64_t* n_codes, uint8_t* out);
int dpq_write_codes_plain(const char* path, const uint8_t* codes, int64_t n_codes, int M);
int dpq_read_codes_plain_ex(const char* path, int M, int K, int with_id, int64_t* n_codes, uint8_t* codes_out,
                            int32_t* ids_out);
int dpq_encode_pq(const float* vectors, int64_t n, int D, const float* codewords, int M, int K, int Ds, int device,
                  uint8_t* codes_out);

typedef struct dpq_train_opts {
    int32_t device;
// ... 107 lines not shown
```

Baseline: 6.652 million queries/s.

## Permute codes within each chunk to cut per-group LUT bank conflicts

Adds a host-side placement pass that, per 64-code chunk, greedily swaps codes among four 16-lane groups so that, for each subspace, fewer distinct labels in a group share the same low nibble. The decode kernel applies this permutation with ds_bpermute when writing raw codes, and the plain scan reads the placement byte to recover each lane's true node id. The filter word becomes a 64-bit scalar per chunk. The goal is fewer LDS bank conflicts on LUT lookups during the scan, at the cost of extra build time, a byte of device memory per node and an extra per-lane load in the scan.

```diff
diff --git a/deltapq_amd/api.py b/deltapq_amd/api.py
--- a/deltapq_amd/api.py
+++ b/deltapq_amd/api.py
@@ -78,10 +78,11 @@
 class HostSoA:
 
     def __init__(self, payload, n_codes, M=8, shard_rank=0, shard_count=1, chunks_per_segment=0, num_codes=0,
-                 multi_index_stride=0):
+                 multi_index_stride=0, flags=0):
         lib = _lib.load()
         pl = np.ascontiguousarray(payload, dtype=np.uint8)
         opts = OpenOpts(0, shard_rank, shard_count, chunks_per_segment, 0, num_codes, multi_index_stride)
+        opts.flags = flags
         h = ctypes.c_void_p()
         check(lib.dpq_soa_build(_np_ptr(pl), pl.size, n_codes, M, opts, h), "dpq_soa_build")
         self._h = h
@@ -89,7 +90,7 @@
         check(lib.dpq_soa_info(h, info), "dpq_soa_info")
         self.info = info.as_dict()
         names = ["nib", "mask", "delta", "seg_delta_off", "seg_ckpt", "mi_cell_start", "mi_code", "mi_id", "par", "carry",
-                 "st_ckpt", "st_mask", "st_poff", "st_pbase", "st_delta", "st_depth"]
+                 "st_ckpt", "st_mask", "st_poff", "st_pbase", "st_delta", "st_depth", "relabel", "place"]
         views = {"seg_delta_off": np.uint64, "st_ckpt": np.uint64, "st_mask": np.uint32, "st_poff": np.uint16, "st_pbase": np.uint32,
                  "st_depth": np.uint16}
         for which, name in enumerate(names):
@@ -246,7 +247,7 @@
 
 
 OPT_NO_RELABEL, OPT_NO_FUSE_QUANTISE, OPT_NO_ASYNC_OVERLAP, OPT_BOOT_FULLSORT = 1, 2, 4, 8
-OPT_NO_TIGHTEN, OPT_NO_STRANDS, OPT_FORCE_STRANDS, OPT_NO_STRAND1 = 16, 32, 64, 128
+OPT_NO_TIGHTEN, OPT_NO_STRANDS, OPT_FORCE_STRANDS, OPT_NO_STRAND1, OPT_NO_PLACE = 16, 32, 64, 128, 256
 MAX_STREAM_QUERIES = 16
 
 
diff --git a/deltapq_amd/csrc/dpq_capi.cpp b/deltapq_amd/csrc/dpq_capi.cpp
--- a/deltapq_amd/csrc/dpq_capi.cpp
+++ b/deltapq_amd/csrc/dpq_capi.cpp
@@ -160,6 +160,7 @@
     int64_t batch_tile_nodes = (int64_t)16 << 20;
     bool relabel = true, fuse_quantise = true, async_overlap = true, boot_fullsort = false, tighten = true, strands = true,
          force_strands = false;
+    bool place = true;
     bool strand1 = true;
     int s1_debug = 0;
 };
@@ -230,6 +231,7 @@
     DevBuf<unsigned long long> d_s1_stamps;
     int batch_decode = 0;
     DevBuf<uint8_t> d_relabel;
+    DevBuf<uint8_t> d_place;
     DevBuf<uint8_t> d_nbr;
     DevBuf<float> d_codebook;
     DevBuf<unsigned long long> d_counters;
@@ -334,6 +336,7 @@
     t.strands = !(o.flags & DPQ_OPT_NO_STRANDS);
     t.force_strands = (o.flags & DPQ_OPT_FORCE_STRANDS) != 0;
     t.strand1 = !(o.flags & DPQ_OPT_NO_STRAND1);
+    t.place = !(o.flags & DPQ_OPT_NO_PLACE);
     if (dev_mode()) {
         auto geti = [](const char* name, int* v) { if (const char* e = getenv(name)) *v = atoi(e); };
         geti("DPQ_STREAM_MAX_QUERIES", &t.stream_max);
@@ -354,6 +357,7 @@
         v = 1; geti("DPQ_STRANDS", &v); t.strands = t.strands && v != 0;
         t.force_strands = t.force_strands || v == 2;
         v = 1; geti("DPQ_STRAND1", &v); t.strand1 = t.strand1 && v != 0;
+        v = 1; geti("DPQ_PLACE", &v); t.place = t.place && v != 0;
         geti("DPQ_S1_DEBUG", &t.s1_debug);
     }
     return t;
@@ -622,7 +626,7 @@
     Workspace& w = x->ws();
     if (b.one_tile) {
         Timer t(x, stream, 4);
-        DPQ_HIP(dpq::launch_decode_list(x->img, nullptr, x->img.n_segments, x->d_relabel,
+        DPQ_HIP(dpq::launch_decode_list(x->img, nullptr, x->img.n_segments, x->d_relabel, x->d_place,
                                         reinterpret_cast<uint32_t*>(w.d_batch_raw.get()), stream));
     }
     {
@@ -640,6 +644,7 @@
     dpq::ScanArgs sa{};
     sa.img = x->img;
     if (b.one_tile) sa.img.raw = w.d_batch_raw;
+    if (b.scratch) sa.place = x->d_place;
     sa.fp32_accum = x->plain ? 1 : 0;
     sa.lut32 = b.labelled ? w.d_lut32r.get() : w.d_lut32.get();
     sa.lut_min = w.d_lut_min;
@@ -792,7 +797,7 @@
             const int cnt = std::min<int>((int)b.tile_segs, sa.n_seg_pass - t0);
             {
                 Timer t(x, stream, 4);
-                DPQ_HIP(dpq::launch_decode_list(x->img, sa.seg_list + t0, cnt, x->d_relabel,
+                DPQ_HIP(dpq::launch_decode_list(x->img, sa.seg_list + t0, cnt, x->d_relabel, x->d_place,
                                                 reinterpret_cast<uint32_t*>(w.d_batch_raw.get()), stream));
             }
             dpq::ScanArgs tile = sa;
@@ -1016,7 +1021,7 @@
             const int cnt = std::min<int>((int)b.tile_segs, sa.n_seg_pass - t0);
             {
                 Timer t(x, stream, 4);
-                DPQ_HIP(dpq::launch_decode_list(x->img, sa.seg_list + t0, cnt, x->d_relabel,
+                DPQ_HIP(dpq::launch_decode_list(x->img, sa.seg_list + t0, cnt, x->d_relabel, x->d_place,
                                                 reinterpret_cast<uint32_t*>(w.d_batch_raw.get()), stream));
             }
             dpq::ScanArgs tile = sa;
@@ -1147,6 +1152,7 @@
     dpq::ScanArgs sa{};
     sa.img = x->img;
     if (b.one_tile) sa.img.raw = w.d_batch_raw;
+    if (b.scratch) sa.place = x->d_place;
     sa.fp32_accum = x->plain ? 1 : 0;
     sa.lut32 = b.labelled ? w.d_lut32r.get() : w.d_lut32.get();
     sa.lut_min = w.d_lut_min;
@@ -1311,7 +1317,7 @@
     const Tuning tune0 = resolve_tuning(o);
     const bool want_strands = tune0.strands && (tune0.force_strands || per_shard >= dpq::kStrandMinNodes / 4 * 3);
     int rc = dpq::transcode(payload, n_bytes, n_codes, M, o.shard_rank, o.shard_count, o.chunks_per_segment, &soa,
-                            &err, o.num_codes, mi_stride, 0, want_strands ? 1 : 0);
+                            &err, o.num_codes, mi_stride, 0, want_strands ? 1 : 0, tune0.place ? 1 : 0);
     if (rc) return fail(rc, err);
 
     DPQ_HIP(hipSetDevice(o.device));
@@ -1351,6 +1357,10 @@
     }
     if (!rc && x->tune.relabel && soa.relabel.size() == (size_t)M * 256) {
         rc = up(x->d_relabel, soa.relabel.data(), soa.relabel.size());
+    }
+    if (!rc && !soa.place.empty()) {
+        if (soa.relabel.empty() || x->d_relabel) rc = up(x->d_place, soa.place.data(), soa.place.size());
+        else soa.place.clear();
     }
     if (!rc && x->boot && x->tune.strands && soa.n_strips > 0 && soa.n_strips < INT32_MAX) {
         rc = up(x->d_st_ckpt, soa.st_ckpt.data(), soa.st_ckpt.size() * 8);
@@ -1409,7 +1419,7 @@
     inf.node_lo = o.global_offset + soa.node_lo;
     inf.node_hi = o.global_offset + soa.node_hi;
     inf.algorithmic_bytes = soa.algorithmic_bytes;
-    inf.device_bytes = soa.device_bytes();
+    inf.device_bytes = soa.device_bytes() + (x->d_place ? (int64_t)soa.place.size() : 0);
     inf.bootstrap_bytes = x->boot ? soa.bootstrap_bytes() : 0;
     inf.bootstrap_stride = x->boot ? soa.mi_stride : 0;
     inf.batch_decode_mb = batch_decode_possible(x) ? (int32_t)((batch_raw_bytes(x) + (1 << 20) - 1) >> 20) : 0;
@@ -1641,7 +1651,8 @@
     dpq_soa* s = new dpq_soa();
     std::string err;
     int rc = dpq::transcode(payload, n_bytes, n_codes, M, o.shard_rank, o.shard_count, o.chunks_per_segment, &s->soa,
-                            &err, o.num_codes, o.bootstrap > 0 && M % 4 == 0 ? o.bootstrap : 0);
+                            &err, o.num_codes, o.bootstrap > 0 && M % 4 == 0 ? o.bootstrap : 0, 0, -1,
+                            resolve_tuning(o).place ? 1 : 0);
     if (rc) {
         delete s;
         *out = nullptr;
@@ -1681,7 +1692,9 @@
         case 13: *ptr = s.st_pbase.data(); *n_bytes = (int64_t)s.st_pbase.size() * 4; break;
         case 14: *ptr = s.st_delta.data(); *n_bytes = (int64_t)s.st_delta.size(); break;
         case 15: *ptr = s.st_depth.data(); *n_bytes = (int64_t)s.st_depth.size() * 2; break;
-        default: return fail(DPQ_ERR_ARG, "which must be 0..15");
+        case 16: *ptr = s.relabel.data(); *n_bytes = (int64_t)s.relabel.size(); break;
+        case 17: *ptr = s.place.data(); *n_bytes = (int64_t)s.place.size(); break;
+        default: return fail(DPQ_ERR_ARG, "which must be 0..17");
     }
     return DPQ_OK;
     });
@@ -2731,7 +2744,7 @@
         if (const char* e = getenv("DPQ_LOOKUP_GROUPED")) grouped = atoi(e) != 0;
     if (!grouped) return DPQ_OK;
     if (int rc = grow(lw.tile, &lw.tile_n, (size_t)image_bytes)) return rc;
-    DPQ_HIP(dpq::launch_decode_list(x->img, nullptr, x->img.n_segments, nullptr, reinterpret_cast<uint32_t*>(lw.tile.get()),
+    DPQ_HIP(dpq::launch_decode_list(x->img, nullptr, x->img.n_segments, nullptr, nullptr, reinterpret_cast<uint32_t*>(lw.tile.get()),
                                     stream));
     img->raw = lw.tile;
     return DPQ_OK;
@@ -2888,7 +2901,7 @@
         const int64_t nt = std::min(tile, seg1 - t0);
         for (int64_t j = 0; j < nt; ++j) segs[(size_t)j] = (uint32_t)(t0 + j);
         DPQ_HIP(hipMemcpy(lw.tile_segs, segs.data(), (size_t)nt * sizeof(uint32_t), hipMemcpyHostToDevice));
-        DPQ_HIP(dpq::launch_decode_list(x->img, lw.tile_segs, (int)nt, nullptr, reinterpret_cast<uint32_t*>(lw.tile.get()),
+        DPQ_HIP(dpq::launch_decode_list(x->img, lw.tile_segs, (int)nt, nullptr, nullptr, reinterpret_cast<uint32_t*>(lw.tile.get()),
                                         nullptr));
         const int64_t a = std::max(l0, t0 * S), b = std::min(l1, (t0 + nt) * S);
         DPQ_HIP(hipMemcpy(codes_out + (size_t)(a - l0) * M, lw.tile.get() + (size_t)(a - t0 * S) * M, (size_t)(b - a) * M,
@@ -3129,6 +3142,7 @@
     sa.debug_pass = pass_all == 2 ? 0 : (pass_all ? 2 : 1);
     if (!x->plain && w.d_batch_raw && batch_tile_segments(x) >= x->img.n_segments && !getenv("DPQ_DEBUG_FUSED")) {
         sa.img.raw = w.d_batch_raw;
+        sa.place = x->d_place;
         if (x->d_relabel) sa.lut32 = w.d_lut32r;
     }
     hipEvent_t a, b;
diff --git a/deltapq_amd/csrc/dpq_format.cpp b/deltapq_amd/csrc/dpq_format.cpp
--- a/deltapq_amd/csrc/dpq_format.cpp
+++ b/deltapq_amd/csrc/dpq_format.cpp
@@ -4,6 +4,7 @@
 #include <cstdio>
 #include <cstring>
 #include <fstream>
+#include <thread>
 
 namespace dpq {
 
@@ -142,7 +143,7 @@
 
 int transcode(const uint8_t* payload, int64_t n_bytes, int64_t n_codes, int M, int shard_rank, int shard_count,
               int chunks_per_segment, SoA* out, std::string* err, int64_t scan_codes, int multi_index_stride,
-              int multi_index_classes, int strands) {
+              int multi_index_classes, int strands, int place) {
     int rc = check_args(payload, n_bytes, n_codes, M, err);
     if (rc) return rc;
     if (scan_codes < 0 || scan_codes > n_codes) {
@@ -227,6 +228,8 @@
     int grp_n = 0;
     std::vector<uint32_t> mi_ids;
     std::vector<uint8_t> mi_codes;
+    const bool want_place = place != 0 && M % 4 == 0 && n_pad > 0 && n_pad <= kPlaceMaxNodes;
+    std::vector<uint8_t> all_codes(want_place ? (size_t)n_pad * M : 0, 0);
     if (multi_index_stride > 0) {
         mi_ids.reserve((size_t)((o.node_hi - o.node_lo) / multi_index_stride + 1));
         mi_codes.reserve((size_t)((o.node_hi - o.node_lo) / multi_index_stride + 1) * M);
@@ -318,6 +321,7 @@
             o.algorithmic_bytes += r.payload_end - r.payload_begin;
             if (i > 0) o.n_diffs += r.n_diff;
             if (r.depth > o.max_depth) o.max_depth = r.depth;
+            if (want_place) memcpy(&all_codes[(size_t)l * M], cur, (size_t)M);
             if (multi_index_stride > 0 && l % multi_index_stride == 0) {
                 mi_ids.push_back((uint32_t)i);
                 mi_codes.insert(mi_codes.end(), cur, cur + M);
@@ -368,6 +372,12 @@
             for (int a = 0; a < 256; ++a) o.relabel[(size_t)m * 256 + a] = (uint8_t)(colour[a] + 16 * seen[colour[a]]++);
         }
     }
+    if (want_place) {
+        if (!o.relabel.empty())
+            for (size_t e = 0; e < all_codes.size(); ++e) all_codes[e] = o.relabel[(e % (size_t)M) * 256 + all_codes[e]];
+        o.place.resize((size_t)n_pad);
+        place_chunks(all_codes.data(), n_pad / kChunk, M, o.place.data());
+    }
     if (multi_index_stride > 0)
         build_multi_index(mi_ids, mi_codes, M, multi_index_stride,
                           multi_index_classes > 0 ? multi_index_classes : bootstrap_classes_for((int64_t)mi_ids.size()), &o);
@@ -391,6 +401,94 @@
         }
     }
     return DPQ_OK;
+}
+
+static void place_chunk(const uint8_t* lab, int M, uint8_t* out) {
+    constexpr int kSweeps = 3;
+    uint8_t cnt[4][16][256];
+    uint8_t dq[4][16][16];
+    uint8_t mx[4][16];
+    int grp[64];
+    memset(cnt, 0, sizeof cnt);
+    memset(dq, 0, sizeof dq);
+    for (int i = 0; i < 64; ++i) {
+        grp[i] = i / 16;
+        for (int m = 0; m < M; ++m)
+            if (cnt[grp[i]][m][lab[i * M + m]]++ == 0) dq[grp[i]][m][lab[i * M + m] & 15]++;
+    }
+    auto max16 = [](const uint8_t* d) {
+        uint8_t r = 0;
+        for (int q = 0; q < 16; ++q) r = std::max(r, d[q]);
+        return r;
+    };
+    for (int g = 0; g < 4; ++g)
+        for (int m = 0; m < M; ++m) mx[g][m] = max16(dq[g][m]);
+    auto cost_after = [&](int a, int m, uint8_t x, uint8_t y) -> int {
+        const bool rem = cnt[a][m][x] == 1, add = cnt[a][m][y] == 0;
+        if (!rem && !add) return mx[a][m];
+        uint8_t* d = dq[a][m];
+        d[x & 15] -= rem, d[y & 15] += add;
+        const int r = max16(d);
+        d[x & 15] += rem, d[y & 15] -= add;
+        return r;
+    };
+    auto swap_delta = [&](int i, int j) {
+        const int a = grp[i], b = grp[j];
+        int delta = 0;
+        for (int m = 0; m < M; ++m) {
+            const uint8_t x = lab[i * M + m], y = lab[j * M + m];
+            if (x != y) delta += cost_after(a, m, x, y) + cost_after(b, m, y, x) - mx[a][m] - mx[b][m];
+        }
+        return delta;
+    };
+    auto move = [&](int i, int to) {
+        const int from = grp[i];
+        for (int m = 0; m < M; ++m) {
+            const uint8_t x = lab[i * M + m];
+            if (--cnt[from][m][x] == 0) dq[from][m][x & 15]--;
+            if (cnt[to][m][x]++ == 0) dq[to][m][x & 15]++;
+        }
+        grp[i] = to;
+    };
+    for (int sweep = 0; sweep < kSweeps; ++sweep) {
+        bool changed = false;
+        for (int i = 0; i < 64; ++i) {
+            bool hot = false;
+            for (int m = 0; m < M && !hot; ++m) {
+                const uint8_t x = lab[i * M + m];
+                hot = mx[grp[i]][m] > 1 && cnt[grp[i]][m][x] == 1 && dq[grp[i]][m][x & 15] == mx[grp[i]][m];
+            }
+            if (!hot) continue;
+            int best = -1, best_delta = 0;
+            for (int j = 0; j < 64; ++j) {
+                if (grp[j] == grp[i]) continue;
+                const int d = swap_delta(i, j);
+                if (d < best_delta) best_delta = d, best = j;
+            }
+            if (best < 0) continue;
+            const int a = grp[i], b = grp[best];
+            move(i, b);
+            move(best, a);
+            for (int m = 0; m < M; ++m) mx[a][m] = max16(dq[a][m]), mx[b][m] = max16(dq[b][m]);
+            changed = true;
+        }
+        if (!changed) break;
+    }
+    int at[4] = {0, 16, 32, 48};
+    for (int i = 0; i < 64; ++i) out[at[grp[i]]++] = (uint8_t)i;
+}
+
+void place_chunks(const uint8_t* labels, int64_t n_chunks, int M, uint8_t* place) {
+    if (M > 16 || n_chunks <= 0) return;
+    const int nt = (int)std::min<int64_t>(std::min<int64_t>(8, std::max(1u, std::thread::hardware_concurrency())), n_chunks / 2048 + 1);
+    auto work = [&](int t) {
+        for (int64_t c = n_chunks * t / nt; c < n_chunks * (t + 1) / nt; ++c)
+            place_chunk(labels + (size_t)c * kChunk * M, M, place + (size_t)c * kChunk);
+    };
+    std::vector<std::thread> th;
+    for (int t = 1; t < nt; ++t) th.emplace_back(work, t);
+    work(0);
+    for (std::thread& t : th) t.join();
 }
 
 void build_multi_index(const std::vector<uint32_t>& ids, const std::vector<uint8_t>& codes, int M, int stride, int classes,
diff --git a/deltapq_amd/csrc/dpq_format.h b/deltapq_amd/csrc/dpq_format.h
--- a/deltapq_amd/csrc/dpq_format.h
+++ b/deltapq_amd/csrc/dpq_format.h
@@ -70,6 +70,7 @@
     std::vector<uint32_t> mi_code;
     std::vector<uint32_t> mi_id;
     std::vector<uint8_t> relabel;
+    std::vector<uint8_t> place;
     int64_t n_strips = 0;
     std::vector<uint64_t> st_ckpt;
     std::vector<uint32_t> st_mask;
@@ -91,7 +92,9 @@
 int validate(const uint8_t* payload, int64_t n_bytes, int64_t n_codes, int M, dpq_dtc_stats* stats, std::string* err);
 int transcode(const uint8_t* payload, int64_t n_bytes, int64_t n_codes, int M, int shard_rank, int shard_count,
               int chunks_per_segment, SoA* out, std::string* err, int64_t scan_codes = 0, int multi_index_stride = 0,
-              int multi_index_classes = 0, int strands = -1);
+              int multi_index_classes = 0, int strands = -1, int place = 0);
+constexpr int64_t kPlaceMaxNodes = (int64_t)16 << 20;
+void place_chunks(const uint8_t* labels, int64_t n_chunks, int M, uint8_t* place);
 constexpr int64_t kStrandMinNodes = (int64_t)8 << 20;
 void build_multi_index(const std::vector<uint32_t>& ids, const std::vector<uint8_t>& codes, int M, int stride, int classes,
                        SoA* out);
diff --git a/deltapq_amd/csrc/dpq_kernels.h b/deltapq_amd/csrc/dpq_kernels.h
--- a/deltapq_amd/csrc/dpq_kernels.h
+++ b/deltapq_amd/csrc/dpq_kernels.h
@@ -58,6 +58,7 @@
     int32_t debug_pass;
     unsigned long long* wg_times;
     int32_t raw_by_pos;
+    const uint8_t* place;
     int32_t append;
     int32_t fp32_accum;
     uint32_t* cand_count;
@@ -159,7 +160,7 @@
                             const uint8_t* d_relabel, float* d_lut_labels, uint32_t* d_tight_hist,
                             hipStream_t stream);
 hipError_t launch_decode_list(const DeviceImage& img, const uint32_t* seg_list, int n_seg, const uint8_t* relabel,
-                              uint32_t* out_code, hipStream_t stream);
+                              const uint8_t* place, uint32_t* out_code, hipStream_t stream);
 hipError_t launch_decode_segments(const DeviceImage& img, const uint32_t* seg_list, int n_seg, uint32_t* out_id,
                                   uint32_t* out_code, hipStream_t stream);
 hipError_t launch_stream(const ScanArgs& a, int n_slots, hipStream_t stream);
diff --git a/deltapq_amd/csrc/dpq_kernels.hip b/deltapq_amd/csrc/dpq_kernels.hip
--- a/deltapq_amd/csrc/dpq_kernels.hip
+++ b/deltapq_amd/csrc/dpq_kernels.hip
@@ -125,7 +125,7 @@
 template <int M>
 __global__ __launch_bounds__(256) void decode_list_kernel(const DeviceImage img, const uint32_t* __restrict__ seg_list,
                                                            int n_seg, const uint8_t* __restrict__ relabel,
-                                                           uint32_t* __restrict__ out_code) {
+                                                           const uint8_t* __restrict__ place, uint32_t* __restrict__ out_code) {
     constexpr int W = Cfg<M>::W;
     __builtin_amdgcn_s_setprio(DPQ_UNDER_SCAN_PRIO);
     const int lane = threadIdx.x & 63;
@@ -139,6 +139,7 @@
         const int64_t node = (seg * cps + c) * 64 + lane;
         const int64_t out = (j * cps + c) * 64 + lane;
         uint32_t code[W];
+        const int src = place ? (int)place[node] : lane;
         dec.step(img, node, lane, c + 1 < cps, code);
         if (relabel) {
 #pragma unroll
@@ -148,6 +149,10 @@
                 for (int b = 0; b < 4; ++b) r |= (uint32_t)relabel[(4 * w + b) * 256 + ((code[w] >> (8 * b)) & 0xffu)] << (8 * b);
                 code[w] = r;
             }
+        }
+        if (place) {
+#pragma unroll
+            for (int w = 0; w < W; ++w) code[w] = (uint32_t)__builtin_amdgcn_ds_bpermute(src << 2, (int)code[w]);
         }
         if constexpr (W == 2)
             reinterpret_cast<uint2*>(out_code)[out] = make_uint2(code[0], code[1]);
@@ -580,6 +585,7 @@
         uint32_t h_stk[W];
         typename WaveDecoder<M>::Ld ld;
         uint32_t raw[W];
+        uint32_t pl;
     };
     int nlane = lane;
     if constexpr (PLAIN) {
@@ -588,17 +594,21 @@
         const int pos = h < 4 ? h : h < 12 ? h - 4 : h < 16 ? h - 8 : h < 20 ? h - 8 : h < 28 ? h - 12 : h - 16;
         nlane = (lane & 32) + 16 * g + pos;
     }
-    auto node_of = [&](const Chunk& k) { return ((int64_t)k.seg * cps + k.c) * 64 + nlane; };
+    auto node_of = [&](const Chunk& k) {
+        return ((int64_t)k.seg * cps + k.c) * 64 + (PLAIN ? (int)k.pl : nlane);
+    };
     auto stage1 = [&](Chunk& k) {
         if (k.seg < 0) return;
-        const int64_t node = node_of(k);
         if (PLAIN) {
+            const int64_t entry = ((int64_t)k.seg * cps + k.c) * 64 + nlane;
+            k.pl = a.place ? (uint32_t)a.place[entry] : (uint32_t)nlane;
 #pragma unroll
             for (int w = 0; w < W; ++w) {
-                const int64_t at = a.raw_by_pos ? ((int64_t)k.pos * cps + k.c) * 64 + nlane : node;
+                const int64_t at = a.raw_by_pos ? ((int64_t)k.pos * cps + k.c) * 64 + nlane : entry;
                 k.raw[w] = reinterpret_cast<const uint32_t*>(a.img.raw)[(size_t)at * W + w];
             }
         } else {
+            const int64_t node = node_of(k);
             k.in = WaveDecoder<M>::load_in(a.img, node);
             k.carry_lane = 0xffu;
             if (k.c + 1 < cps && lane < C::LEVELS) k.carry_lane = a.img.carry[(size_t)(node >> 6) * C::LEVELS + lane];
@@ -633,8 +643,15 @@
         return n;
     };
     Chunk A, B, Cn;
-    uint32_t fwA = 0, fwB = 0, fwC = 0;
-    auto filter_word = [&](const Chunk& k) -> uint32_t { return k.seg < 0 ? 0u : a.filter[(size_t)node_of(k) >> 5]; };
+    using FW = std::conditional_t<PLAIN, uint64_t, uint32_t>;
+    FW fwA = 0, fwB = 0, fwC = 0;
+    auto filter_word = [&](const Chunk& k) -> FW {
+        if (k.seg < 0) return 0;
+        if constexpr (PLAIN)
+            return reinterpret_cast<const uint64_t*>(a.filter)[(size_t)__builtin_amdgcn_readfirstlane(k.seg * cps + k.c)];
+        else
+            return a.filter[(size_t)node_of(k) >> 5];
+    };
     A.seg = helper ? -1 : next_entry();
     A.pos = entry_pos;
     A.c = 0;
@@ -649,6 +666,7 @@
         if constexpr (PLAIN) {
 #pragma unroll
             for (int w = 0; w < W; ++w) asm volatile("" ::"v"(A.raw[w]), "v"(B.raw[w]));
+            asm volatile("" ::"v"(A.pl), "v"(B.pl));
         } else {
             asm volatile("" ::"v"(A.ld.level), "v"(A.ld.mk), "v"(A.ld.par), "v"(A.carry_lane), "v"(B.in.nb), "v"(B.in.mk),
                          "v"(B.in.par), "v"(B.carry_lane));
@@ -658,7 +676,8 @@
 #pragma unroll
             for (int w = 0; w < W; ++w) asm volatile("" ::"v"(A.h_stk[w]), "v"(B.h_stk[w]));
         }
-        if constexpr (FILT) asm volatile("" ::"v"(fwA), "v"(fwB));
+        if constexpr (FILT && PLAIN) asm volatile("" ::"s"(fwA), "s"(fwB));
+        if constexpr (FILT && !PLAIN) asm volatile("" ::"v"(fwA), "v"(fwB));
         Cn = successor(B);
         stage2(B);
         stage1(Cn);
@@ -778,7 +797,7 @@
             }
             stamp(kStGather);
             bool valid = node < a.img.n_local;
-            if constexpr (FILT) valid = valid && ((fwA >> ((uint32_t)node & 31u)) & 1u) != 0u;
+            if constexpr (FILT) valid = valid && ((fwA >> ((uint32_t)node & (PLAIN ? 63u : 31u))) & 1u) != 0u;
             uint64_t pend = 0;
 #pragma unroll
             for (int h = 0; h < MD; ++h) {
@@ -2796,13 +2815,13 @@
 }
 
 hipError_t launch_decode_list(const DeviceImage& img, const uint32_t* seg_list, int n_seg, const uint8_t* relabel,
-                              uint32_t* out_code, hipStream_t stream) {
+                              const uint8_t* place, uint32_t* out_code, hipStream_t stream) {
     if (n_seg <= 0) return hipSuccess;
     const unsigned grid = (unsigned)((n_seg + 3) / 4);
     if (img.M == 8)
-        hipLaunchKernelGGL(decode_list_kernel<8>, dim3(grid), dim3(256), 0, stream, img, seg_list, n_seg, relabel, out_code);
+        hipLaunchKernelGGL(decode_list_kernel<8>, dim3(grid), dim3(256), 0, stream, img, seg_list, n_seg, relabel, place, out_code);
     else if (img.M == 16)
-        hipLaunchKernelGGL(decode_list_kernel<16>, dim3(grid), dim3(256), 0, stream, img, seg_list, n_seg, relabel, out_code);
+        hipLaunchKernelGGL(decode_list_kernel<16>, dim3(grid), dim3(256), 0, stream, img, seg_list, n_seg, relabel, place, out_code);
     else
         return hipErrorInvalidValue;
     return hipGetLastError();
diff --git a/include/deltapq_amd.h b/include/deltapq_amd.h
--- a/include/deltapq_amd.h
+++ b/include/deltapq_amd.h
@@ -53,6 +53,7 @@
 #define DPQ_OPT_NO_STRANDS 32u
 #define DPQ_OPT_FORCE_STRANDS 64u
 #define DPQ_OPT_NO_STRAND1 128u
+#define DPQ_OPT_NO_PLACE 256u
 
 typedef struct dpq_info {
     int64_t n_codes_total;
```

Result: slower. 6.562 million queries/s (-1.4%).
